# quadram-institute-bioscience/tatajuba

Measured on AMD Instinct MI355X. Metric: reads/s (whole node), 150 bp synthetic FASTQ, homopolymer scan + context histogram, higher is better.
Workload: dtype u8/u64

## Files before the change

### include/tatajuba_amd.h

```cpp
#ifndef TATAJUBA_AMD_H
#define TATAJUBA_AMD_H

#include "tatajuba_hopo.h"

#ifdef __cplusplus
extern "C" {
#endif

#define TJ_META_BASE_SHIFT   0
#define TJ_META_LEN_SHIFT    2
#define TJ_META_COUNT_SHIFT  12
#define TJ_META_MISM_SHIFT   32
#define TJ_META_FLAG_SHIFT   49
#define TJ_META_RAW_CONST    ((1ULL << TJ_META_COUNT_SHIFT) | (0xffeULL << TJ_META_MISM_SHIFT))

typedef struct tjamd_counter tjamd_counter;

typedef struct { uint64_t ctx0, ctx1, meta; } tjamd_record;
typedef struct { uint64_t ctx0, ctx1, meta, pos; } tjamd_located_record;

enum { TJAMD_OK = 0, TJAMD_ERR_NO_DEVICE = 1, TJAMD_ERR_HIP = 2, TJAMD_ERR_ARG = 3, TJAMD_ERR_CAPACITY = 4, TJAMD_ERR_STATE = 5 };

int  tjamd_device_count (void);
const char *tjamd_last_error (void);
const char *tjamd_version (void);
const char *tjamd_source_hash (void);

tjamd_counter *tjamd_counter_create (int device, int kmer_size);
void tjamd_counter_destroy (tjamd_counter *c);
int  tjamd_counter_reset (tjamd_counter *c);
int  tjamd_counter_set_stream (tjamd_counter *c, void *hip_stream);
int  tjamd_counter_device (const tjamd_counter *c);

int  tjamd_scan_device (tjamd_counter *c, const void *d_stream, size_t n_bytes, int min_tract_size);
int  tjamd_scan_host (tjamd_counter *c, const void *h_stream, size_t n_bytes, int min_tract_size);
long tjamd_scan_host_located (tjamd_counter *c, const void *h_stream, size_t n_bytes, int min_tract_size,
                              tjamd_located_record *out, long capacity);

long tjamd_scan_windows (int kmer_size, const char *const *seqs, const int *lens, int n_windows, int min_tract_size,
                         hopo_element *out, int *window_of, long capacity);

long tjamd_read_file_stream (const char *path, unsigned char *out, long capacity, long *n_reads);

long tjamd_read_file_stream_mt (const char *path, unsigned char *out, long capacity, long *n_reads, int n_threads, long window_bytes);

void *tjamd_host_alloc (size_t bytes);
void tjamd_host_free (void *p);
int  tjamd_sync (tjamd_counter *c);

void *tjamd_device_alloc (tjamd_counter *c, size_t bytes);
void tjamd_device_free (tjamd_counter *c, void *p);
int  tjamd_device_download (tjamd_counter *c, void *host, const void *dev, size_t bytes);

int  tjamd_reserve (tjamd_counter *c, size_t stream_bytes, int min_tract_size);

int  tjamd_mark (tjamd_counter *c);
int  tjamd_wait_mark (tjamd_counter *c, int mark);

long tjamd_raw_count (tjamd_counter *c);
long tjamd_download_raw (tjamd_counter *c, tjamd_record *out, long capacity);
long tjamd_undefined_runs (tjamd_counter *c);
int  tjamd_upload_raw (tjamd_counter *c, const hopo_element *elems, long n);

int  tjamd_finalise (tjamd_counter *c, int remove_biased, int min_coverage, int *status);
int  tjamd_finalise_begin (tjamd_counter *c, int remove_biased, int min_coverage);
int  tjamd_counter_set_order_stream (tjamd_counter *c, void *hip_stream);
int  tjamd_finalise_end (tjamd_counter *c, int *status);
long tjamd_kept_count (tjamd_counter *c);
int  tjamd_n_idx (tjamd_counter *c);
int  tjamd_coverage (tjamd_counter *c);
long tjamd_download_kept (tjamd_counter *c, hopo_element *out, long capacity);
long tjamd_download_idx (tjamd_counter *c, int *idx_initial, int *idx_final, long capacity);
const void *tjamd_kept_device_ptr (tjamd_counter *c);

long tjamd_merge_samples (tjamd_counter *c, const void *d_records, const long *counts, int n_samples,
                          void *d_out_keys, void *d_out_counts, long capacity);

long tjamd_gather_histograms (tjamd_counter *dst, tjamd_counter *const *samples, int n_samples, const void **d_records, long *counts);

int tjamd_peer_access_report (char *out, int capacity);

#define TJAMD_COMM_ID_BYTES 128
typedef struct tjamd_comm tjamd_comm;
int  tjamd_comm_unique_id (void *id_bytes);
tjamd_comm *tjamd_comm_create (tjamd_counter *c, const void *id_bytes, int rank, int world);
void tjamd_comm_destroy (tjamd_comm *comm);
int  tjamd_comm_set_stream (tjamd_comm *comm, void *hip_stream);
int  tjamd_comm_rank (const tjamd_comm *comm);
int  tjamd_comm_world (const tjamd_comm *comm);
int  tjamd_comm_count (const tjamd_comm *comm);
int  tjamd_comm_last_exchange (const tjamd_comm *comm, double *ms, long *bytes, long *collectives);
long tjamd_comm_collectives (const tjamd_comm *comm);
long tjamd_allgather_histograms (tjamd_counter *c, tjamd_comm *comm, const void **d_records, long *counts);

long tjamd_tract_ids (tjamd_counter *c, const void *d_keys, long n, int *d_tract_id, int *h_tract_id);

#define TJAMD_N_TRACT_STATS 5
enum { TJAMD_STAT_AVG_LENGTH, TJAMD_STAT_MODAL_FREQ, TJAMD_STAT_PROP_COVERAGE, TJAMD_STAT_COVERAGE_PER_CONTEXT, TJAMD_STAT_ENTROPY };
typedef struct { int first, n_rows, n_present, variable; double reldiff[TJAMD_N_TRACT_STATS]; } tjamd_tract_summary;

long tjamd_tract_stats (tjamd_counter *c, const void *d_keys, const void *d_counts, long n_union, int n_samples,
                        const int *d_tract_id, const int *coverage, const int *d_ref_length,
                        tjamd_tract_summary *d_summary, int *d_var, long capacity, long *n_var);
long tjamd_tract_sample_stats (tjamd_counter *c, const void *d_keys, const void *d_counts, long n_union, int n_samples,
                               const int *coverage, const tjamd_tract_summary *d_summary, long n_tracts, const int *d_list, long n_list,
                               double *d_values, int *d_modal_len, int *d_n_context);

typedef struct { int first, n_rows, n_context, mode, indel, lev_distance; long long integral; } tjamd_union_tract;
typedef struct { int first, n_rows, n_present, variable, selected, lev_distance; double reldiff[TJAMD_N_TRACT_STATS]; } tjamd_union_tract_summary;

long tjamd_union_tracts (tjamd_counter *c, const void *d_keys, const void *d_counts, long n_union, int n_samples,
                         int max_distance_per_flank, int levenshtein_distance,
                         int *d_tract_id, int *d_join_type, tjamd_union_tract *d_tracts, long capacity);
long tjamd_union_tract_stats (tjamd_counter *c, const void *d_keys, const void *d_counts, long n_union, int n_samples,
                              const tjamd_union_tract *d_tracts, long n_tracts, const int *coverage, const int *d_ref_length,
                              tjamd_union_tract_summary *d_summary, int *d_var, long *n_var, int *d_sel, long *n_sel);
long tjamd_union_tract_sample_stats (tjamd_counter *c, const void *d_keys, const void *d_counts, long n_union, int n_samples,
                                     const int *coverage, const tjamd_union_tract_summary *d_summary, long n_tracts,
                                     const int *d_list, long n_list, double *d_values, int *d_modal_len, int *d_n_context, int *d_n_len);

typedef struct { int first, n_elem, n_context, mode; long long integral; } tjamd_group;
long tjamd_group_contexts (tjamd_counter *c, int max_distance_per_flank, int *group_of, tjamd_group *groups, long capacity);

typedef struct { int first, n_elem, n_context, mode, indel, n_len, modal_len, modal_freq; long long integral; } tjamd_context_group;
typedef struct { int length, freq; } tjamd_length_freq;
long tjamd_context_histograms (tjamd_counter *c, int max_distance_per_flank, int levenshtein_distance, int *group_of, int *join_type,
                               tjamd_context_group *groups, tjamd_length_freq *hist, long capacity);

typedef struct tjamd_reference tjamd_reference;
typedef struct { uint64_t ctx0, ctx1; long long flat; int contig, pos, length, base, neg_strand, pad; } tjamd_ref_entry;
tjamd_reference *tjamd_reference_create (tjamd_counter *c, const void *h_stream, size_t n_bytes);
void tjamd_reference_destroy (tjamd_reference *ref);
long tjamd_reference_entries (const tjamd_reference *ref);
long tjamd_reference_contigs (const tjamd_reference *ref);
long tjamd_reference_download (const tjamd_reference *ref, tjamd_ref_entry *out, long capacity);

typedef struct { long long flat; int contig, pos, ref_length, mismatches, neg_strand, n_hits; } tjamd_location;
long tjamd_locate (tjamd_counter *c, const tjamd_reference *ref, const void *d_keys, long n, int max_mismatches, tjamd_location *d_loc);

long tjamd_located_tracts (tjamd_counter *c, const void *d_keys, const void *d_counts, long n_union, int n_samples,
                           const tjamd_union_tract *d_tracts, long n_tracts, const tjamd_location *d_loc,
                           int *d_perm, void *d_out_keys, void *d_out_counts,
                           tjamd_union_tract *d_out_tracts, tjamd_location *d_tract_loc, int *d_ref_length, long capacity);






void tjamd_thread_cleanup (void);

double tjamd_last_scan_ms (tjamd_counter *c);
int    tjamd_counter_uses_log (const tjamd_counter *c);
double tjamd_last_partition_ms (tjamd_counter *c);
double tjamd_last_finalise_ms (tjamd_counter *c);
double tjamd_last_merge_ms (tjamd_counter *c);
double tjamd_last_tract_stats_ms (tjamd_counter *c);
double tjamd_last_union_tracts_ms (tjamd_counter *c);
double tjamd_last_union_tract_stats_ms (tjamd_counter *c);
long   tjamd_last_union_tract_candidates (tjamd_counter *c);
double tjamd_last_reference_ms (tjamd_counter *c);
double tjamd_last_locate_ms (tjamd_counter *c);
double tjamd_last_located_tracts_ms (tjamd_counter *c);
double tjamd_last_tract_variants_ms (tjamd_counter *c);
long   tjamd_last_scan_launches (tjamd_counter *c);
long   tjamd_plan_mismatches (tjamd_counter *c);

long tjamd_synth_stream (uint64_t seed_genome, uint64_t seed_reads, uint64_t variant_seed, long genome_len,
                         long n_reads, int read_len, int read_len_max, unsigned char *out, long capacity, int n_threads);

#ifdef __cplusplus
}
#endif
#endif
```

### tatajuba_amd/capi.py

```python
import ctypes as C
import os

import numpy as np

from .build import build_library, library_path

ELEM_DTYPE = np.dtype([("ctx0", "<u8"), ("ctx1", "<u8"), ("meta", "<u8"), ("read_offset", "<i4"),
                       ("loc_ref_id", "<i4"), ("loc_pos", "<i4"), ("loc_last", "<i4")])
RECORD_DTYPE = np.dtype([("ctx0", "<u8"), ("ctx1", "<u8"), ("meta", "<u8")])
GROUP_DTYPE = np.dtype([("first", "<i4"), ("n_elem", "<i4"), ("n_context", "<i4"), ("mode", "<i4"), ("integral", "<i8")])
CONTEXT_GROUP_DTYPE = np.dtype([("first", "<i4"), ("n_elem", "<i4"), ("n_context", "<i4"), ("mode", "<i4"), ("indel", "<i4"), ("n_len", "<i4"),
                                ("modal_len", "<i4"), ("modal_freq", "<i4"), ("integral", "<i8")])
LENGTH_FREQ_DTYPE = np.dtype([("length", "<i4"), ("freq", "<i4")])
LOCATED_DTYPE = np.dtype([("ctx0", "<u8"), ("ctx1", "<u8"), ("meta", "<u8"), ("pos", "<u8")])
N_TRACT_STATS = 5
TRACT_SUMMARY_DTYPE = np.dtype([("first", "<i4"), ("n_rows", "<i4"), ("n_present", "<i4"), ("variable", "<i4"), ("reldiff", "<f8", (N_TRACT_STATS,))])
assert TRACT_SUMMARY_DTYPE.itemsize == 56
UNION_TRACT_DTYPE = np.dtype([("first", "<i4"), ("n_rows", "<i4"), ("n_context", "<i4"), ("mode", "<i4"), ("indel", "<i4"),
                              ("lev_distance", "<i4"), ("integral", "<i8")])
assert UNION_TRACT_DTYPE.itemsize == 32
UNION_TRACT_SUMMARY_DTYPE = np.dtype([("first", "<i4"), ("n_rows", "<i4"), ("n_present", "<i4"), ("variable", "<i4"), ("selected", "<i4"),
                                      ("lev_distance", "<i4"), ("reldiff", "<f8", (N_TRACT_STATS,))])
assert UNION_TRACT_SUMMARY_DTYPE.itemsize == 64
REF_ENTRY_DTYPE = np.dtype([("ctx0", "<u8"), ("ctx1", "<u8"), ("flat", "<i8"), ("contig", "<i4"), ("pos", "<i4"), ("length", "<i4"),
                            ("base", "<i4"), ("neg_strand", "<i4"), ("pad", "<i4")])
assert REF_ENTRY_DTYPE.itemsize == 48
LOCATION_DTYPE = np.dtype([("flat", "<i8"), ("contig", "<i4"), ("pos", "<i4"), ("ref_length", "<i4"), ("mismatches", "<i4"),
                           ("neg_strand", "<i4"), ("n_hits", "<i4")])
assert LOCATION_DTYPE.itemsize == 32
VARIANT_DTYPE = np.dtype([("flat", "<i8"), ("tract", "<i4"), ("sample", "<i4"), ("contig", "<i4"), ("pos", "<i4"), ("row", "<i4"), ("base", "<i4"),
                          ("ref_length", "<i4"), ("alt_length", "<i4"), ("n_flank", "<i4"), ("pad", "<i4"), ("ref_flank", "<u8"), ("alt_flank", "<u8")])
assert VARIANT_DTYPE.itemsize == 64
FEATURE_DTYPE = np.dtype([("contig", "<i4"), ("start", "<i4"), ("end", "<i4"), ("cls", "<i4"), ("strand", "<i4"), ("line", "<i4"), ("type_off", "<i4"), ("id_off", "<i4")])
assert FEATURE_DTYPE.itemsize == 32
TRACT_FEATURE_DTYPE = np.dtype([("feature", "<i4"), ("max_length", "<i4")])
assert TRACT_FEATURE_DTYPE.itemsize == 8
CDS_DTYPE = np.dtype([("aa_len", "<i4"), ("has_stop", "<i4"), ("n_codons", "<i4"), ("phase", "<i4")])
assert CDS_DTYPE.itemsize == 16
EFFECT_DTYPE = np.dtype([("feature", "<i4"), ("cls", "<i4"), ("cds_pos", "<i4"), ("first_diff", "<i4"), ("ref_aa_len", "<i4"), ("alt_aa_len", "<i4"),
                         ("flags", "<i4"), ("pad", "<i4"), ("ref_aa", "<u8"), ("alt_aa", "<u8")])
assert EFFECT_DTYPE.itemsize == 48
EFFECT_CLASSES = ["NONE", "BOUNDARY", "IDENTICAL", "INFRAME", "FRAMESHIFT"]
SITE_DTYPE = np.dtype([("flat", "<i8"), ("tract", "<i4"), ("contig", "<i4"), ("pos", "<i4"), ("base", "<i4"), ("ref_length", "<i4"), ("min_length", "<i4"),
                       ("n_flank", "<i4"), ("n_alleles", "<i4"), ("first_allele", "<i4"), ("n_called", "<i4"), ("first_record", "<i4"), ("pad", "<i4"),
                       ("ref_flank", "<u8")])
assert SITE_DTYPE.itemsize == 64
ALLELE_DTYPE = np.dtype([("site", "<i4"), ("alt_length", "<i4"), ("n_flank", "<i4"), ("n_samples", "<i4"), ("first_record", "<i4"), ("pad", "<i4"),
                         ("alt_flank", "<u8")])
assert ALLELE_DTYPE.itemsize == 32


class TatajubaAmdError(RuntimeError):
    pass


def _sx(v, bits):
    v = v.astype(np.int64) & ((1 << bits) - 1)
    return np.where(v >= (1 << (bits - 1)), v - (1 << bits), v)


def decode_meta(meta):
    m = np.asarray(meta, dtype=np.uint64)
    sh = lambda s: (m >> np.uint64(s))
    return {"base": _sx(sh(0), 2), "length": _sx(sh(2), 10), "count": _sx(sh(12), 20),
            "mismatches": _sx(sh(32), 12), "multi": _sx(sh(44), 3), "neg_strand": _sx(sh(47), 2),
            "canon_flag": _sx(sh(49), 3)}


class Options(C.Structure):
    _fields_ = [("reference_fasta_filename", C.c_char_p), ("outdir", C.c_char_p),
                ("paired_end", C.c_bool), ("remove_biased", C.c_bool), ("save_vcf", C.c_bool),
                ("gff", C.c_void_p),
                ("max_distance_per_flank", C.c_int), ("kmer_size", C.c_int), ("min_tract_size", C.c_int),
                ("levenshtein_distance", C.c_int), ("min_coverage", C.c_int), ("n_samples", C.c_int),
                ("n_threads", C.c_int)]

    @classmethod
    def defaults(cls, kmer_size=25, min_tract_size=4, min_coverage=5, remove_biased=True, paired_end=False):
        o = cls()
        o.kmer_size, o.min_tract_size, o.min_coverage = kmer_size, min_tract_size, min_coverage
        o.remove_biased, o.paired_end = remove_biased, paired_end
        o.max_distance_per_flank, o.levenshtein_distance, o.n_samples, o.n_threads = 1, 2, 1, 1
        return o


class _HopoCounterStruct(C.Structure):
    _fields_ = [("elem", C.c_void_p), ("name", C.c_char_p),
                ("ref_start", C.c_int), ("n_elem", C.c_int), ("n_alloc", C.c_int), ("kmer_size", C.c_int),
                ("coverage", C.c_int),
                ("idx_initial", C.POINTER(C.c_int)), ("idx_final", C.POINTER(C.c_int)), ("n_idx", C.c_int),
                ("opt", Options), ("ref_counter", C.c_int)]


assert C.sizeof(Options) == 64 and C.sizeof(_HopoCounterStruct) == 136

_LIB = None

EXPORTS = [
    "new_hopo_counter", "del_hopo_counter", "new_or_append_hopo_counter_from_file", "update_hopo_counter_from_seq",
    "update_hopo_counter_from_seq_all_monomers",
    "finalise_hopo_counter", "compare_hopo_element_decreasing", "compare_hopo_context",
    "generate_name_from_flanking_contexts", "generate_tract_as_string", "print_tatajuba_options",
    "distance_between_single_context_kmer", "distance_between_context_kmer_pair", "distance_between_context_kmer_pair_with_edit_shift",
    "leftmost_hopo_name_and_length_from_string", "hopo_counter_histogram_integral",
    "dna_in_2_bits", "bit_2_dna",
    "tjamd_device_count", "tjamd_source_hash", "tjamd_last_error", "tjamd_version", "tjamd_counter_create", "tjamd_counter_destroy",
    "tjamd_counter_reset", "tjamd_counter_set_stream", "tjamd_counter_set_order_stream", "tjamd_counter_device", "tjamd_scan_device", "tjamd_scan_host",
    "tjamd_scan_host_located", "tjamd_read_file_stream_mt", "tjamd_host_alloc", "tjamd_host_free", "tjamd_device_alloc", "tjamd_device_free", "tjamd_device_download", "tjamd_sync", "tjamd_mark", "tjamd_wait_mark", "tjamd_reserve", "tjamd_raw_count",
    "tjamd_download_raw", "tjamd_undefined_runs", "tjamd_upload_raw", "tjamd_finalise", "tjamd_finalise_begin", "tjamd_finalise_end", "tjamd_kept_count",
    "tjamd_n_idx", "tjamd_coverage", "tjamd_download_kept", "tjamd_download_idx", "tjamd_kept_device_ptr",
    "tjamd_merge_samples", "tjamd_gather_histograms", "tjamd_peer_access_report", "tjamd_comm_unique_id", "tjamd_comm_create", "tjamd_comm_destroy",
    "tjamd_comm_set_stream", "tjamd_comm_rank", "tjamd_comm_world", "tjamd_comm_collectives", "tjamd_comm_count", "tjamd_comm_last_exchange", "tjamd_last_merge_ms", "tjamd_allgather_histograms", "tjamd_tract_ids", "tjamd_tract_stats", "tjamd_tract_sample_stats", "tjamd_last_tract_stats_ms", "tjamd_union_tracts", "tjamd_union_tract_stats", "tjamd_union_tract_sample_stats", "tjamd_last_union_tracts_ms", "tjamd_last_union_tract_stats_ms", "tjamd_last_union_tract_candidates",
    "tjamd_reference_create", "tjamd_reference_destroy", "tjamd_reference_entries", "tjamd_reference_contigs",
    "tjamd_reference_download", "tjamd_last_reference_ms", "tjamd_locate", "tjamd_last_locate_ms", "tjamd_located_tracts", "tjamd_last_located_tracts_ms",
    "tjamd_last_tract_variants_ms",
    "tjamd_group_contexts", "tjamd_context_histograms", "tjamd_scan_windows", "tjamd_thread_cleanup", "tjamd_last_scan_ms", "tjamd_last_partition_ms", "tjamd_counter_uses_log", "tjamd_last_finalise_ms", "tjamd_last_scan_launches", "tjamd_plan_mismatches",
    "tjamd_synth_stream", "tjamd_read_file_stream",
    "new_genomic_context_list", "del_genomic_context_list", "del_context_histogram",
    "distance_between_context_histogram_and_hopo_context", "indel_distance_between_context_histogram_and_hopo_context",
]

VARIANT_EXPORTS = ["tjamd_tract_variants", "tjamd_read_file_names"]
FEATURE_EXPORTS = ["tjamd_gff3_read", "tjamd_annotation_create", "tjamd_annotation_destroy", "tjamd_annotation_features", "tjamd_annotation_download",
                   "tjamd_tract_features", "tjamd_last_annotation_ms", "tjamd_last_tract_features_ms"]
LOCATE_EXPORTS = ["tjamd_flank_edit_distance", "tjamd_reference_add_seeds", "tjamd_reference_has_seeds", "tjamd_locate_gapped",
                  "tjamd_last_seed_order_ms", "tjamd_last_locate_gapped_ms"]
EFFECT_EXPORTS = ["tjamd_translate", "tjamd_gff3_read_phase", "tjamd_coding_create", "tjamd_coding_destroy", "tjamd_coding_features", "tjamd_coding_download",
                  "tjamd_variant_effects", "tjamd_last_coding_ms", "tjamd_last_variant_effects_ms"]
SITE_EXPORTS = ["tjamd_merge_variants", "tjamd_site_ref_alt", "tjamd_last_merge_variants_ms"]
MAX_SHIFT = 3


def _share_hip_runtime_with_torch():
    if os.environ.get("TATAJUBA_AMD_HIP_RUNTIME", "") == "system":
        return
    import importlib.util
    import sys
    if "torch" in sys.modules:
        return
    try:
        spec = importlib.util.find_spec("torch")
    except (ImportError, ValueError):
        spec = None
    if spec is None or not spec.submodule_search_locations:
        return
    cand = os.path.join(list(spec.submodule_search_locations)[0], "lib", "libamdhip64.so")
    if os.path.exists(cand):
        try:
            C.CDLL(cand, mode=C.RTLD_GLOBAL)
        except OSError:
            pass


def lib():
    global _LIB
    if _LIB is not None:
        return _LIB
    path = library_path()
    if not os.path.exists(path):
        build_library()
    _share_hip_runtime_with_torch()
    L = C.CDLL(path)
    P = C.POINTER(_HopoCounterStruct)
    L.new_hopo_counter.restype = P; L.new_hopo_counter.argtypes = [C.c_int]
    L.del_hopo_counter.restype = None; L.del_hopo_counter.argtypes = [P]
    L.new_or_append_hopo_counter_from_file.restype = P
    L.new_or_append_hopo_counter_from_file.argtypes = [P, C.c_char_p, Options]
    L.update_hopo_counter_from_seq.restype = None
    L.update_hopo_counter_from_seq.argtypes = [P, C.c_char_p, C.c_int, C.c_int]
    L.update_hopo_counter_from_seq_all_monomers.restype = None
    L.update_hopo_counter_from_seq_all_monomers.argtypes = [P, C.c_char_p, C.c_int]
    L.finalise_hopo_counter.restype = None; L.finalise_hopo_counter.argtypes = [P]
    L.generate_name_from_flanking_contexts.restype = C.c_void_p
    L.generate_name_from_flanking_contexts.argtypes = [C.POINTER(C.c_uint64), C.c_int8, C.c_int, C.c_bool]
    L.generate_tract_as_string.restype = C.c_void_p
    L.generate_tract_as_string.argtypes = [C.POINTER(C.c_uint64), C.c_int8, C.c_int, C.c_int, C.c_bool]
    L.compare_hopo_element_decreasing.restype = C.c_int
    L.compare_hopo_element_decreasing.argtypes = [C.c_void_p, C.c_void_p]

    L.tjamd_device_count.restype = C.c_int
    L.tjamd_last_error.restype = C.c_char_p
    L.tjamd_version.restype = C.c_char_p
    L.tjamd_counter_create.restype = C.c_void_p; L.tjamd_counter_create.argtypes = [C.c_int, C.c_int]
    L.tjamd_counter_destroy.restype = None; L.tjamd_counter_destroy.argtypes = [C.c_void_p]
    L.tjamd_counter_reset.argtypes = [C.c_void_p]
    L.tjamd_counter_set_stream.argtypes = [C.c_void_p, C.c_void_p]
    L.tjamd_counter_device.argtypes = [C.c_void_p]
    L.tjamd_scan_device.argtypes = [C.c_void_p, C.c_void_p, C.c_size_t, C.c_int]
    L.tjamd_scan_host.argtypes = [C.c_void_p, C.c_void_p, C.c_size_t, C.c_int]
    L.tjamd_scan_host_located.restype = C.c_long
    L.tjamd_scan_host_located.argtypes = [C.c_void_p, C.c_void_p, C.c_size_t, C.c_int, C.c_void_p, C.c_long]
    L.tjamd_host_alloc.restype = C.c_void_p; L.tjamd_host_alloc.argtypes = [C.c_size_t]
    L.tjamd_host_free.restype = None; L.tjamd_host_free.argtypes = [C.c_void_p]
    L.tjamd_sync.argtypes = [C.c_void_p]
    L.tjamd_raw_count.restype = C.c_long; L.tjamd_raw_count.argtypes = [C.c_void_p]
    L.tjamd_download_raw.restype = C.c_long; L.tjamd_download_raw.argtypes = [C.c_void_p, C.c_void_p, C.c_long]
    L.tjamd_undefined_runs.restype = C.c_long; L.tjamd_undefined_runs.argtypes = [C.c_void_p]
    L.tjamd_upload_raw.argtypes = [C.c_void_p, C.c_void_p, C.c_long]
    L.tjamd_finalise.argtypes = [C.c_void_p, C.c_int, C.c_int, C.POINTER(C.c_int)]
    L.tjamd_finalise_begin.argtypes = [C.c_void_p, C.c_int, C.c_int]
    L.tjamd_finalise_end.argtypes = [C.c_void_p, C.POINTER(C.c_int)]
    L.tjamd_kept_count.restype = C.c_long; L.tjamd_kept_count.argtypes = [C.c_void_p]
    L.tjamd_n_idx.argtypes = [C.c_void_p]
    L.tjamd_coverage.argtypes = [C.c_void_p]
    L.tjamd_download_kept.restype = C.c_long; L.tjamd_download_kept.argtypes = [C.c_void_p, C.c_void_p, C.c_long]
    L.tjamd_download_idx.restype = C.c_long
    L.tjamd_download_idx.argtypes = [C.c_void_p, C.c_void_p, C.c_void_p, C.c_long]
    L.tjamd_kept_device_ptr.restype = C.c_void_p; L.tjamd_kept_device_ptr.argtypes = [C.c_void_p]
    L.tjamd_merge_samples.restype = C.c_long
    L.tjamd_merge_samples.argtypes = [C.c_void_p, C.c_void_p, C.POINTER(C.c_long), C.c_int, C.c_void_p, C.c_void_p, C.c_long]
    L.tjamd_gather_histograms.restype = C.c_long
    L.tjamd_gather_histograms.argtypes = [C.c_void_p, C.POINTER(C.c_void_p), C.c_int, C.POINTER(C.c_void_p), C.POINTER(C.c_long)]
    L.tjamd_tract_ids.restype = C.c_long; L.tjamd_tract_ids.argtypes = [C.c_void_p, C.c_void_p, C.c_long, C.c_void_p, C.c_void_p]
    L.tjamd_tract_stats.restype = C.c_long
    L.tjamd_tract_stats.argtypes = [C.c_void_p, C.c_void_p, C.c_void_p, C.c_long, C.c_int, C.c_void_p, C.POINTER(C.c_int), C.c_void_p,
                                    C.c_void_p, C.c_void_p, C.c_long, C.POINTER(C.c_long)]
    L.tjamd_tract_sample_stats.restype = C.c_long
    L.tjamd_tract_sample_stats.argtypes = [C.c_void_p, C.c_void_p, C.c_void_p, C.c_long, C.c_int, C.POINTER(C.c_int), C.c_void_p, C.c_long,
                                           C.c_void_p, C.c_long, C.c_void_p, C.c_void_p, C.c_void_p]
    L.tjamd_last_tract_stats_ms.restype = C.c_double; L.tjamd_last_tract_stats_ms.argtypes = [C.c_void_p]
    L.tjamd_union_tracts.restype = C.c_long
    L.tjamd_union_tracts.argtypes = [C.c_void_p, C.c_void_p, C.c_void_p, C.c_long, C.c_int, C.c_int, C.c_int, C.c_void_p, C.c_void_p, C.c_void_p, C.c_long]
    L.tjamd_union_tract_stats.restype = C.c_long
    L.tjamd_union_tract_stats.argtypes = [C.c_void_p, C.c_void_p, C.c_void_p, C.c_long, C.c_int, C.c_void_p, C.c_long, C.POINTER(C.c_int), C.c_void_p,
                                          C.c_void_p, C.c_void_p, C.POINTER(C.c_long), C.c_void_p, C.POINTER(C.c_long)]
    L.tjamd_union_tract_sample_stats.restype = C.c_long
    L.tjamd_union_tract_sample_stats.argtypes = [C.c_void_p, C.c_void_p, C.c_void_p, C.c_long, C.c_int, C.POINTER(C.c_int), C.c_void_p, C.c_long,
                                                 C.c_void_p, C.c_long, C.c_void_p, C.c_void_p, C.c_void_p, C.c_void_p]
    L.tjamd_last_union_tracts_ms.restype = C.c_double; L.tjamd_last_union_tracts_ms.argtypes = [C.c_void_p]
    L.tjamd_last_union_tract_stats_ms.restype = C.c_double; L.tjamd_last_union_tract_stats_ms.argtypes = [C.c_void_p]
    L.tjamd_last_union_tract_candidates.restype = C.c_long; L.tjamd_last_union_tract_candidates.argtypes = [C.c_void_p]
    L.tjamd_reference_create.restype = C.c_void_p; L.tjamd_reference_create.argtypes = [C.c_void_p, C.c_void_p, C.c_size_t]
    L.tjamd_reference_destroy.restype = None; L.tjamd_reference_destroy.argtypes = [C.c_void_p]
    L.tjamd_reference_entries.restype = C.c_long; L.tjamd_reference_entries.argtypes = [C.c_void_p]
    L.tjamd_reference_contigs.restype = C.c_long; L.tjamd_reference_contigs.argtypes = [C.c_void_p]
    L.tjamd_reference_download.restype = C.c_long; L.tjamd_reference_download.argtypes = [C.c_void_p, C.c_void_p, C.c_long]
    L.tjamd_locate.restype = C.c_long; L.tjamd_locate.argtypes = [C.c_void_p, C.c_void_p, C.c_void_p, C.c_long, C.c_int, C.c_void_p]
    L.tjamd_located_tracts.restype = C.c_long
    L.tjamd_located_tracts.argtypes = [C.c_void_p, C.c_void_p, C.c_void_p, C.c_long, C.c_int, C.c_void_p, C.c_long, C.c_void_p,
                                       C.c_void_p, C.c_void_p, C.c_void_p, C.c_void_p, C.c_void_p, C.c_void_p, C.c_long]
    L.tjamd_last_reference_ms.restype = C.c_double; L.tjamd_last_reference_ms.argtypes = [C.c_void_p]
    L.tjamd_last_locate_ms.restype = C.c_double; L.tjamd_last_locate_ms.argtypes = [C.c_void_p]
    L.tjamd_last_located_tracts_ms.restype = C.c_double; L.tjamd_last_located_tracts_ms.argtypes = [C.c_void_p]
    L.tjamd_flank_edit_distance.restype = C.c_int; L.tjamd_flank_edit_distance.argtypes = [C.c_uint64, C.c_uint64, C.c_int, C.c_int, C.c_int]
    L.tjamd_reference_add_seeds.restype = C.c_long; L.tjamd_reference_add_seeds.argtypes = [C.c_void_p, C.c_void_p]
    L.tjamd_reference_has_seeds.restype = C.c_int; L.tjamd_reference_has_seeds.argtypes = [C.c_void_p]
    L.tjamd_locate_gapped.restype = C.c_long
    L.tjamd_locate_gapped.argtypes = [C.c_void_p, C.c_void_p, C.c_void_p, C.c_long, C.c_int, C.c_int, C.c_void_p, C.c_void_p]
    L.tjamd_last_seed_order_ms.restype = C.c_double; L.tjamd_last_seed_order_ms.argtypes = [C.c_void_p]
    L.tjamd_last_locate_gapped_ms.restype = C.c_double; L.tjamd_last_locate_gapped_ms.argtypes = [C.c_void_p]
    L.tjamd_tract_variants.restype = C.c_long
    L.tjamd_tract_variants.argtypes = [C.c_void_p, C.c_void_p, C.c_void_p, C.c_void_p, C.c_long, C.c_int, C.c_void_p, C.c_long, C.c_void_p,
                                       C.c_void_p, C.c_long, C.c_void_p, C.c_long, C.c_void_p]
    L.tjamd_last_tract_variants_ms.restype = C.c_double; L.tjamd_last_tract_variants_ms.argtypes = [C.c_void_p]
    L.tjamd_read_file_names.restype = C.c_long
    L.tjamd_read_file_names.argtypes = [C.c_char_p, C.c_void_p, C.c_long, C.POINTER(C.c_long)]
    L.tjamd_gff3_read.restype = C.c_long
    L.tjamd_gff3_read.argtypes = [C.c_char_p, C.c_char_p, C.c_long, C.c_void_p, C.c_long, C.c_void_p, C.c_long, C.POINTER(C.c_long), C.POINTER(C.c_long)]
    L.tjamd_annotation_create.restype = C.c_void_p; L.tjamd_annotation_create.argtypes = [C.c_void_p, C.c_void_p, C.c_void_p, C.c_long]
    L.tjamd_annotation_destroy.restype = None; L.tjamd_annotation_destroy.argtypes = [C.c_void_p]
    L.tjamd_annotation_features.restype = C.c_long; L.tjamd_annotation_features.argtypes = [C.c_void_p]
    L.tjamd_annotation_download.restype = C.c_long; L.tjamd_annotation_download.argtypes = [C.c_void_p, C.c_void_p, C.c_void_p, C.c_long]
    L.tjamd_tract_features.restype = C.c_long
    L.tjamd_tract_features.argtypes = [C.c_void_p, C.c_void_p, C.c_void_p, C.c_void_p, C.c_long, C.c_int, C.c_void_p, C.c_long, C.c_void_p, C.c_void_p]
    L.tjamd_last_annotation_ms.restype = C.c_double; L.tjamd_last_annotation_ms.argtypes = [C.c_void_p]
    L.tjamd_last_tract_features_ms.restype = C.c_double; L.tjamd_last_tract_features_ms.argtypes = [C.c_void_p]
    L.tjamd_translate.restype = C.c_long; L.tjamd_translate.argtypes = [C.c_char_p, C.c_long, C.c_int, C.c_void_p, C.c_long]
    L.tjamd_gff3_read_phase.restype = C.c_long; L.tjamd_gff3_read_phase.argtypes = [C.c_char_p, C.c_char_p, C.c_long, C.c_void_p, C.c_long]
    L.tjamd_coding_create.restype = C.c_void_p; L.tjamd_coding_create.argtypes = [C.c_void_p, C.c_void_p, C.c_size_t, C.c_void_p, C.c_long, C.c_void_p]
    L.tjamd_coding_destroy.restype = None; L.tjamd_coding_destroy.argtypes = [C.c_void_p]
    L.tjamd_coding_features.restype = C.c_long; L.tjamd_coding_features.argtypes = [C.c_void_p]
    L.tjamd_coding_download.restype = C.c_long; L.tjamd_coding_download.argtypes = [C.c_void_p, C.c_void_p, C.c_long]
    L.tjamd_variant_effects.restype = C.c_long
    L.tjamd_variant_effects.argtypes = [C.c_void_p, C.c_void_p, C.c_void_p, C.c_long, C.c_void_p, C.c_long, C.c_void_p]
    L.tjamd_last_coding_ms.restype = C.c_double; L.tjamd_last_coding_ms.argtypes = [C.c_void_p]
    L.tjamd_last_variant_effects_ms.restype = C.c_double; L.tjamd_last_variant_effects_ms.argtypes = [C.c_void_p]
    L.tjamd_merge_variants.restype = C.c_long
    L.tjamd_merge_variants.argtypes = [C.c_void_p, C.c_int, C.c_void_p, C.c_long, C.c_int, C.c_long, C.c_void_p, C.c_long, C.c_void_p, C.c_long,
                                       C.c_void_p, C.c_void_p, C.c_void_p, C.c_void_p]
    L.tjamd_site_ref_alt.restype = C.c_int; L.tjamd_site_ref_alt.argtypes = [C.c_void_p, C.c_void_p, C.c_int, C.c_void_p, C.c_int]
    L.tjamd_last_merge_variants_ms.restype = C.c_double; L.tjamd_last_merge_variants_ms.argtypes = [C.c_void_p]
    L.tjamd_group_contexts.restype = C.c_long
    L.tjamd_group_contexts.argtypes = [C.c_void_p, C.c_int, C.c_void_p, C.c_void_p, C.c_long]
    L.new_genomic_context_list.restype = C.POINTER(GenomicContextListStruct); L.new_genomic_context_list.argtypes = [P]
    L.del_genomic_context_list.restype = None; L.del_genomic_context_list.argtypes = [C.POINTER(GenomicContextListStruct)]
    L.tjamd_comm_unique_id.argtypes = [C.c_void_p]
    L.tjamd_comm_create.restype = C.c_void_p; L.tjamd_comm_create.argtypes = [C.c_void_p, C.c_void_p, C.c_int, C.c_int]
    L.tjamd_comm_destroy.restype = None; L.tjamd_comm_destroy.argtypes = [C.c_void_p]
    L.tjamd_comm_rank.argtypes = [C.c_void_p]; L.tjamd_comm_world.argtypes = [C.c_void_p]
    L.tjamd_comm_set_stream.argtypes = [C.c_void_p, C.c_void_p]
    L.tjamd_comm_collectives.restype = C.c_long; L.tjamd_comm_collectives.argtypes = [C.c_void_p]
    L.tjamd_allgather_histograms.restype = C.c_long
    L.tjamd_allgather_histograms.argtypes = [C.c_void_p, C.c_void_p, C.POINTER(C.c_void_p), C.POINTER(C.c_long)]
    L.tjamd_peer_access_report.argtypes = [C.c_char_p, C.c_int]
    L.tjamd_context_histograms.restype = C.c_long
    L.tjamd_context_histograms.argtypes = [C.c_void_p, C.c_int, C.c_int, C.c_void_p, C.c_void_p, C.c_void_p, C.c_void_p, C.c_long]
    L.tjamd_device_alloc.restype = C.c_void_p; L.tjamd_device_alloc.argtypes = [C.c_void_p, C.c_size_t]
    L.tjamd_device_free.restype = None; L.tjamd_device_free.argtypes = [C.c_void_p, C.c_void_p]
    L.tjamd_device_download.argtypes = [C.c_void_p, C.c_void_p, C.c_void_p, C.c_size_t]
    L.tjamd_scan_windows.restype = C.c_long
    L.tjamd_scan_windows.argtypes = [C.c_int, C.POINTER(C.c_char_p), C.POINTER(C.c_int), C.c_int, C.c_int, C.c_void_p, C.c_void_p, C.c_long]
    U64P = C.POINTER(C.c_uint64)
    L.distance_between_single_context_kmer.argtypes = [U64P, U64P, C.c_int]
    L.distance_between_context_kmer_pair.argtypes = [U64P, U64P]
    L.distance_between_context_kmer_pair_with_edit_shift.argtypes = [U64P, U64P, C.POINTER(C.c_int)]
    L.leftmost_hopo_name_and_length_from_string.restype = C.c_void_p
    L.leftmost_hopo_name_and_length_from_string.argtypes = [C.c_char_p, C.c_size_t, C.c_int, C.c_int, C.POINTER(C.c_int)]
    L.hopo_counter_histogram_integral.argtypes = [P, C.c_int]
    L.tjamd_last_scan_ms.restype = C.c_double; L.tjamd_last_scan_ms.argtypes = [C.c_void_p]
    L.tjamd_last_finalise_ms.restype = C.c_double; L.tjamd_last_finalise_ms.argtypes = [C.c_void_p]
    L.tjamd_last_partition_ms.restype = C.c_double; L.tjamd_last_partition_ms.argtypes = [C.c_void_p]
    L.tjamd_last_scan_launches.restype = C.c_long; L.tjamd_last_scan_launches.argtypes = [C.c_void_p]
    L.tjamd_synth_stream.restype = C.c_long
    L.tjamd_synth_stream.argtypes = [C.c_uint64, C.c_uint64, C.c_uint64, C.c_long, C.c_long, C.c_int, C.c_int,
                                     C.c_void_p, C.c_long, C.c_int]
    L.tjamd_read_file_stream.restype = C.c_long
    L.tjamd_read_file_stream.argtypes = [C.c_char_p, C.c_void_p, C.c_long, C.POINTER(C.c_long)]
    _LIB = L
    return L


def _err():
    return (lib().tjamd_last_error() or b"").decode(errors="replace")


def device_count():
    return lib().tjamd_device_count()


def synth_stream(n_reads, read_len, genome_len, seed_genome=0x7A7A0001, seed_reads=0x7A7A1000, variant_seed=0,
                 read_len_max=0, n_threads=8, out=None):
    need = -lib().tjamd_synth_stream(seed_genome, seed_reads, variant_seed, genome_len, n_reads, read_len, read_len_max,
                                     None, 0, n_threads)
    if need <= 0:
        raise TatajubaAmdError("bad synthetic-stream parameters")
    if out is None:
        out = np.empty(need, dtype=np.uint8)
    assert out.dtype == np.uint8 and out.size >= need and out.flags["C_CONTIGUOUS"]
    got = lib().tjamd_synth_stream(seed_genome, seed_reads, variant_seed, genome_len, n_reads, read_len, read_len_max,
                                   out.ctypes.data, out.size, n_threads)
    if got != need:
        raise TatajubaAmdError("synthetic stream generation failed")
    return out[:need]


def read_file_stream_mt(path, n_threads=4, window_bytes=0):
    L = lib()
    L.tjamd_read_file_stream_mt.restype = C.c_long
    L.tjamd_read_file_stream_mt.argtypes = [C.c_char_p, C.c_void_p, C.c_long, C.POINTER(C.c_long), C.c_int, C.c_long]
    n = C.c_long(0)
    need = L.tjamd_read_file_stream_mt(os.fsencode(path), None, 0, C.byref(n), n_threads, window_bytes)
    if need < 0:
        raise FileNotFoundError(path)
    out = np.empty(max(need, 1), dtype=np.uint8)
    got = L.tjamd_read_file_stream_mt(os.fsencode(path), out.ctypes.data, need, C.byref(n), n_threads, window_bytes)
    assert got == need
    return out[:need], n.value


def read_file_stream(path):
    n = C.c_long(0)
    need = lib().tjamd_read_file_stream(os.fsencode(path), None, 0, C.byref(n))
    if need < 0:
        raise FileNotFoundError(path)
    out = np.empty(max(need, 1), dtype=np.uint8)
    got = lib().tjamd_read_file_stream(os.fsencode(path), out.ctypes.data, need, C.byref(n))
    assert got == need
    return out[:need], n.value


def read_gff3(path, names):
    blob = b"".join((n if isinstance(n, bytes) else str(n).encode()) + b"\n" for n in names)
    nb, sk = C.c_long(0), C.c_long(0)
    n = lib().tjamd_gff3_read(os.fsencode(path), blob, len(names), None, 0, None, 0, C.byref(nb), C.byref(sk))
    if n < 0:
        raise FileNotFoundError(path)
    out = np.zeros(n, dtype=FEATURE_DTYPE)
    strings = np.zeros(max(nb.value, 1), dtype=np.uint8)
    got = lib().tjamd_gff3_read(os.fsencode(path), blob, len(names), out.ctypes.data, n, strings.ctypes.data, nb.value, C.byref(nb), C.byref(sk))
    assert got == n
    read_gff3.last_skipped = sk.value
    return out, strings[: nb.value].tobytes()


def read_gff3_phase(path, names):
    blob = b"".join((n if isinstance(n, bytes) else str(n).encode()) + b"\n" for n in names)
    n = lib().tjamd_gff3_read_phase(os.fsencode(path), blob, len(names), None, 0)
    if n < 0:
        raise FileNotFoundError(path)
    out = np.zeros(n, dtype=np.int8)
    got = lib().tjamd_gff3_read_phase(os.fsencode(path), blob, len(names), out.ctypes.data if n else None, n)
    assert got == n
    return out


def translate(dna, reverse=False):
    b = dna if isinstance(dna, bytes) else str(dna).encode()
    out = np.zeros(max(len(b) // 3, 1), dtype=np.uint8)
    n = lib().tjamd_translate(b, len(b), 1 if reverse else 0, out.ctypes.data, len(b) // 3)
    if n < 0:
        raise TatajubaAmdError(_err())
    return out[:n].tobytes().decode()


def site_ref_alt(site, allele, k):
    sb = np.asarray(site, SITE_DTYPE).reshape(1).tobytes()
    ab = None if allele is None else np.asarray(allele, ALLELE_DTYPE).reshape(1).tobytes()
    n = lib().tjamd_site_ref_alt(sb, ab, k, None, 0)
    if n < 0:
        raise TatajubaAmdError("tjamd_site_ref_alt: a site or allele that has no text")
    out = C.create_string_buffer(n + 1)
    assert lib().tjamd_site_ref_alt(sb, ab, k, out, n + 1) == n
    return out.value.decode()


def gff3_string(strings, off):
    return strings[off: strings.index(b"\0", off)].decode(errors="replace")


class EmpfreqElement(C.Structure):
    _fields_ = [("freq", C.c_int), ("idx", C.c_int)]


class EmpfreqStruct(C.Structure):
    _fields_ = [("i", C.POINTER(EmpfreqElement)), ("n", C.c_int), ("min", C.c_int), ("max", C.c_int)]


class ContextHistogramStruct(C.Structure):
    _fields_ = [("context", C.POINTER(C.c_uint64)),
                ("base", C.c_int32, 2), ("multi", C.c_int32, 3), ("indel", C.c_int32, 2), ("neg_strand", C.c_int32, 1), ("mismatches", C.c_int32, 12),
                ("name", C.c_char_p), ("n_context", C.c_int), ("integral", C.c_int), ("location", C.c_int), ("loc2d", C.c_int * 3),
                ("coverage", C.c_int), ("n_tracts", C.c_int), ("mode_context_count", C.c_int), ("mode_context_length", C.c_int),
                ("mode_context_id", C.c_int), ("tmp_count", C.POINTER(C.c_int)), ("tmp_length", C.POINTER(C.c_int)), ("index", C.c_int),
                ("h", C.POINTER(EmpfreqStruct)), ("tract_id", C.c_int), ("ref_counter", C.c_int)]


class GenomicContextListStruct(C.Structure):
    _fields_ = [("hist", C.POINTER(C.POINTER(ContextHistogramStruct))), ("name", C.c_char_p), ("opt", Options),
                ("n_hist", C.c_int), ("coverage", C.c_int), ("ref_start", C.c_int)]


class Comm:

    ID_BYTES = 128

    @staticmethod
    def unique_id():
        buf = C.create_string_buffer(Comm.ID_BYTES)
        if lib().tjamd_comm_unique_id(buf) != 0:
            raise TatajubaAmdError(_err())
        return buf.raw

    def __init__(self, counter, ident, rank, world):
        self.world = world
        self._id = C.create_string_buffer(bytes(ident), Comm.ID_BYTES)
        self._h = lib().tjamd_comm_create(counter._h, self._id, rank, world)
        if not self._h:
            raise TatajubaAmdError(_err())

    def set_stream(self, hip_stream):
        if lib().tjamd_comm_set_stream(self._h, C.c_void_p(hip_stream)) != 0:
            raise TatajubaAmdError(_err())

# ... 212 lines not shown
        self._chk(lib().tjamd_finalise(self._h, int(bool(remove_biased)), int(min_coverage), C.byref(st)))
        return st.value

    def finalise_begin(self, remove_biased, min_coverage):
        self._chk(lib().tjamd_finalise_begin(self._h, int(bool(remove_biased)), int(min_coverage)))

    def finalise_end(self):
        st = C.c_int(-1)
        self._chk(lib().tjamd_finalise_end(self._h, C.byref(st)))
        return st.value

    @property
    def n_kept(self):
        return lib().tjamd_kept_count(self._h)

    @property
    def n_idx(self):
        return lib().tjamd_n_idx(self._h)

    @property
    def coverage(self):
        return lib().tjamd_coverage(self._h)

    @property
    def kept_device_ptr(self):
        return lib().tjamd_kept_device_ptr(self._h)

    def download_kept(self):
        n = self.n_kept
        out = np.zeros(n, dtype=ELEM_DTYPE)
        self._chkn(lib().tjamd_download_kept(self._h, out.ctypes.data, n))
        return out

    def download_idx(self):
        n = self.n_idx
        a, b = np.zeros(n, np.int32), np.zeros(n, np.int32)
        self._chkn(lib().tjamd_download_idx(self._h, a.ctypes.data, b.ctypes.data, n))
        return a, b

    def group_contexts(self, max_distance_per_flank):
        n = self.n_kept
        gof = np.zeros(max(n, 1), dtype=np.int32)
        grp = np.zeros(max(n, 1), dtype=GROUP_DTYPE)
        ng = self._chkn(lib().tjamd_group_contexts(self._h, max_distance_per_flank, gof.ctypes.data, grp.ctypes.data, n))
        return gof[:n], grp[:ng]

    def context_histograms(self, max_distance_per_flank, levenshtein_distance):
        n = self.n_kept
        gof, jt = np.zeros(max(n, 1), np.int32), np.zeros(max(n, 1), np.int32)
        grp = np.zeros(max(n, 1), dtype=CONTEXT_GROUP_DTYPE)
        hist = np.zeros(max(n, 1), dtype=LENGTH_FREQ_DTYPE)
        ng = self._chkn(lib().tjamd_context_histograms(self._h, max_distance_per_flank, levenshtein_distance, gof.ctypes.data, jt.ctypes.data,
                                                       grp.ctypes.data, hist.ctypes.data, n))
        return {"group_of": gof[:n], "join_type": jt[:n], "groups": grp[:ng], "hist": hist[:n]}

    def last_scan_launches(self):
        return int(lib().tjamd_last_scan_launches(self._h))

    def plan_mismatches(self):
        lib().tjamd_plan_mismatches.restype = C.c_long
        lib().tjamd_plan_mismatches.argtypes = [C.c_void_p]
        return int(lib().tjamd_plan_mismatches(self._h))

    def last_scan_ms(self):
        return lib().tjamd_last_scan_ms(self._h)

    def last_partition_ms(self):
        return lib().tjamd_last_partition_ms(self._h)

    def bucket_counts(self):
        import numpy as np
        f = lib().tjamd_debug_bucket_counts
        f.restype = C.c_long
        f.argtypes = [C.c_void_p, C.c_void_p, C.c_int]
        b = np.zeros(256, np.uint32)
        if f(self._h, b.ctypes.data, 256) < 0:
            raise TatajubaAmdError(_err())
        return b

    def last_merge_ms(self):
        lib().tjamd_last_merge_ms.restype = C.c_double
        lib().tjamd_last_merge_ms.argtypes = [C.c_void_p]
        return lib().tjamd_last_merge_ms(self._h)

    def last_tract_stats_ms(self):
        return lib().tjamd_last_tract_stats_ms(self._h)

    def last_union_tracts_ms(self):
        return lib().tjamd_last_union_tracts_ms(self._h)

    def last_union_tract_stats_ms(self):
        return lib().tjamd_last_union_tract_stats_ms(self._h)

    def last_union_tract_candidates(self):
        return int(lib().tjamd_last_union_tract_candidates(self._h))

    def last_reference_ms(self):
        return lib().tjamd_last_reference_ms(self._h)

    def last_locate_ms(self):
        return lib().tjamd_last_locate_ms(self._h)

    def last_located_tracts_ms(self):
        return lib().tjamd_last_located_tracts_ms(self._h)

    def locate_gapped(self, ref, d_keys, n, max_edits, max_shift, d_loc, d_how=None):
        got = lib().tjamd_locate_gapped(self._h, ref._h, d_keys, n, max_edits, max_shift, d_loc, d_how)
        if got < 0:
            raise TatajubaAmdError(_err())
        return int(got)

    def last_seed_order_ms(self):
        return lib().tjamd_last_seed_order_ms(self._h)

    def last_locate_gapped_ms(self):
        return lib().tjamd_last_locate_gapped_ms(self._h)

    def last_tract_variants_ms(self):
        return lib().tjamd_last_tract_variants_ms(self._h)

    def last_annotation_ms(self):
        return lib().tjamd_last_annotation_ms(self._h)

    def last_tract_features_ms(self):
        return lib().tjamd_last_tract_features_ms(self._h)

    def variant_effects(self, coding, d_variants, n, d_out, d_tract_feat=None, n_tracts=0):
        return self._chkn(lib().tjamd_variant_effects(self._h, coding._h, d_variants, n, d_tract_feat, n_tracts, d_out))

    def last_coding_ms(self):
        return lib().tjamd_last_coding_ms(self._h)

    def last_variant_effects_ms(self):
        return lib().tjamd_last_variant_effects_ms(self._h)

    def merge_variants(self, kmer_size, d_records, n_records, n_samples, n_tracts, d_sites, site_capacity, d_alleles, allele_capacity,
                       d_genotype=None, d_allele_of=None, d_unique=None):
        n_alleles = C.c_long(-1)
        n_sites = self._chkn(lib().tjamd_merge_variants(self._h, kmer_size, d_records, n_records, n_samples, n_tracts, d_sites, site_capacity,
                                                        d_alleles, allele_capacity, d_genotype, d_allele_of, d_unique, C.byref(n_alleles)))
        return n_sites, n_alleles.value

    def last_merge_variants_ms(self):
        return lib().tjamd_last_merge_variants_ms(self._h)

    def uses_log(self):
        lib().tjamd_counter_uses_log.restype = C.c_int
        lib().tjamd_counter_uses_log.argtypes = [C.c_void_p]
        return bool(lib().tjamd_counter_uses_log(self._h))

    def last_finalise_ms(self):
        return lib().tjamd_last_finalise_ms(self._h)


class HopoCounter:

    def __init__(self, ptr):
        self._p = ptr

    @classmethod
    def new(cls, kmer_size):
        return cls(lib().new_hopo_counter(kmer_size))

    @classmethod
    def new_or_append_from_file(cls, hc, filename, opt):
        p = lib().new_or_append_hopo_counter_from_file(hc._p if hc is not None else None, os.fsencode(filename), opt)
        if hc is not None:
            return hc
        return cls(p)

    def update_from_seq(self, seq, min_tract_size):
        if isinstance(seq, str):
            seq = seq.encode("latin-1")
        lib().update_hopo_counter_from_seq(self._p, seq, len(seq), min_tract_size)

    def update_from_seq_all_monomers(self, seq):
        if isinstance(seq, str):
            seq = seq.encode("latin-1")
        lib().update_hopo_counter_from_seq_all_monomers(self._p, seq, len(seq))

    def finalise(self):
        lib().finalise_hopo_counter(self._p)

    def delete(self):
        if self._p:
            lib().del_hopo_counter(self._p)
            self._p = None

    __del__ = delete

    @property
    def c(self):
        return self._p.contents

    def elems(self, n=None):
        n = self.c.n_elem if n is None else n
        if n == 0:
            return np.zeros(0, dtype=ELEM_DTYPE)
        buf = (C.c_char * (n * 40)).from_address(self.c.elem)
        return np.frombuffer(buf, dtype=ELEM_DTYPE).copy()

    def idx(self):
        n = self.c.n_idx
        if n == 0 or not self.c.idx_initial:
            return np.zeros(0, np.int32), np.zeros(0, np.int32)
        return (np.ctypeslib.as_array(self.c.idx_initial, (n,)).copy(),
                np.ctypeslib.as_array(self.c.idx_final, (n,)).copy())
```

### tatajuba_amd/csrc/hopo_device.hip

```cpp

#include <hip/hip_runtime.h>
#include <rccl/rccl.h>
#include <dlfcn.h>
#include <mutex>
#include <string>
#include <new>
#include <stdint.h>
#include <stdio.h>
#include <stdlib.h>
#include <string.h>
#include <stdarg.h>
#include <limits.h>
#include <float.h>
#include <algorithm>
#include <vector>
#include <memory>

#include "../../include/tatajuba_amd.h"
#include "../../include/tatajuba_variants.h"
#include "../../include/tatajuba_features.h"
#include "../../include/tatajuba_effects.h"
#include "../../include/tatajuba_sites.h"
#include "../../include/tatajuba_locate.h"

// ... 567 lines not shown
  for (u64 i = blockIdx.x * (u64) blockDim.x + threadIdx.x; i < n_fix; i += (u64) gridDim.x * blockDim.x) {
    u64 c0, c1; u32 base, flag;
    if (stale_context (seq, n_bytes, fix[i].pos, k, mprime, c0, c1, base, flag)) {
      u64 idx = atomicAdd (&ctr->n_rec, 1ull);
      if (idx < cap) store_record<4> (out, idx, c0, c1, make_meta (base, fix[i].len, flag), (u64) fix[i].pos);
      else ctr->overflow = 1u;
    }
    else atomicAdd (&ctr->n_undefined, 1ull);
  }
}


template <int W> __device__ __forceinline__ void pack_raw (u64 c0, u64 c1, u32 base, u32 len10, u32 flag, int k, u64 *w);
#define R1_FLAG_SHIFT 59
#define R1_KEY_MASK   (~(3ull << R1_FLAG_SHIFT))
__device__ __forceinline__ u64 pack_rec1 (u32 c0, u32 c1, u32 base, u32 len10, u32 flag)
{
  const u32 lo = c1 | (len10 << 24), hi = c0 | ((len10 >> 8) << 24) | (base << 26) | (flag << 27);
  return ((u64) hi << 32) | lo;
}
template <> __device__ __forceinline__ void pack_raw<1> (u64 c0, u64 c1, u32 base, u32 len10, u32 flag, int k, u64 *w)
{ w[0] = pack_rec1 ((u32) c0, (u32) c1, base, len10, flag); }
template <> __device__ __forceinline__ void pack_raw<2> (u64 c0, u64 c1, u32 base, u32 len10, u32 flag, int k, u64 *w)
{ w[0] = 1ull | ((u64) base << 1) | ((u64) (len10 & 31u) << 2) | (c0 << 7); w[1] = c1 | ((u64) (len10 >> 5) << 56) | ((u64) flag << 61); }
template <> __device__ __forceinline__ void pack_raw<4> (u64 c0, u64 c1, u32 base, u32 len10, u32 flag, int k, u64 *w)
{ w[0] = c0; w[1] = c1; w[2] = (u64) base | ((u64) len10 << 2) | ((u64) flag << 12); w[3] = 0; }
template <int W> __device__ __forceinline__ void pack_null (u64 *w) { pack_raw<W> (0, 0, 0, 0, 3u, 2, w); }

template <int W> __device__ __forceinline__ void unpack_raw (const u64 *w, int k, u64 &c0, u64 &c1, u32 &base, u32 &len10, u32 &flag);
template <> __device__ __forceinline__ void unpack_raw<1> (const u64 *w, int k, u64 &c0, u64 &c1, u32 &base, u32 &len10, u32 &flag)
{
  const u32 lo = (u32) w[0], hi = (u32) (w[0] >> 32);
  c1 = lo & 0xFFFFFFu; c0 = hi & 0xFFFFFFu; len10 = (lo >> 24) | (((hi >> 24) & 3u) << 8); base = (hi >> 26) & 1u; flag = (hi >> 27) & 3u;
}
template <> __device__ __forceinline__ void unpack_raw<2> (const u64 *w, int k, u64 &c0, u64 &c1, u32 &base, u32 &len10, u32 &flag)
{
  const u64 m56 = (1ull << 56) - 1ull;
  c0 = (w[0] >> 7) & m56; c1 = w[1] & m56;
  base = (u32) (w[0] >> 1) & 1u; len10 = ((u32) (w[0] >> 2) & 31u) | (((u32) (w[1] >> 56) & 31u) << 5); flag = (u32) (w[1] >> 61) & 3u;
}
template <> __device__ __forceinline__ void unpack_raw<4> (const u64 *w, int k, u64 &c0, u64 &c1, u32 &base, u32 &len10, u32 &flag)
{ c0 = w[0]; c1 = w[1]; base = (u32) (w[2] & 3ull); len10 = (u32) ((w[2] >> 2) & 0x3FFull); flag = (u32) ((w[2] >> 12) & 3ull); }

__device__ __forceinline__ u64 hash_key (u64 c0, u64 c1, u32 base, u32 len10)
{
  u32 a = (u32) c0 ^ __builtin_amdgcn_alignbit ((u32) (c0 >> 32), (u32) (c0 >> 32), 25) ^ __builtin_amdgcn_alignbit ((u32) c1, (u32) c1, 19)
          ^ __builtin_amdgcn_alignbit ((u32) (c1 >> 32), (u32) (c1 >> 32), 11) ^ ((base | (len10 << 2)) * 0x9E3779B1u);
  u32 h = a * 0x85EBCA6Bu;
  h ^= h >> 15; h *= 0xC2B2AE35u; h ^= h >> 16;
  const u32 tag = (a ^ (a >> 13)) * 0x27D4EB2Fu;
  return ((u64) tag << 32) | h;
}

__device__ __forceinline__ u32 bucket_of_key (u64 c0, u64 c1, u32 base, u32 len10)
{
  u32 h = __builtin_amdgcn_udot4 ((u32) c0, 0x6D2B4F0Bu, base | (len10 << 2), false);
  h = __builtin_amdgcn_udot4 ((u32) (c0 >> 32), 0x1D59A735u, h, false);
  h = __builtin_amdgcn_udot4 ((u32) c1, 0xC5A34D17u, h, false);
  h = __builtin_amdgcn_udot4 ((u32) (c1 >> 32), 0x3B7F9165u, h, false);
  return (h ^ (h >> 8)) & 255u;
}

__device__ __forceinline__ u32 bucket_of_rec1 (u32 lo, u32 hi)
{
  u32 h = __builtin_amdgcn_udot4 (lo, 0x6D2B4F0Bu, 0u, false);
  h = __builtin_amdgcn_udot4 (hi & 0x07FFFFFFu, 0xC5A34D17u, h, false);
  return (h ^ (h >> 8)) & 255u;
}

#define TJ_P        256
#define TJ_PBITS    8
#define TJ_STAGE_WORDS 2048
#define TJ_CH0      1536
#define TJ_EMPTY    0xFFFFFFFFu
#define TJ_CSTRIDE  64

struct Buckets
{
  u64 *pool;
  u32 *table;
  u32 *cursors;
  u32 *pool_next;
  u32 pool_chunks, maxj, ch_shift;
};

#define TJ_NOCHUNK  0xFFFFFFFEu
#define TJ_SPIN_MAX (1u << 20)

__device__ __forceinline__ u32 chunk_of_pos (const Buckets &B, u32 pos) { return (pos / TJ_CH0) >> B.ch_shift; }

__device__ __forceinline__ void bucket_claim_ahead (const Buckets &B, u32 b, u32 p0, u32 n, DevCounters *ctr)
{
  const u32 j = chunk_of_pos (B, p0 + n - 1);
  if (((j * TJ_CH0) << B.ch_shift) < p0) return;
  if (j + 1 >= B.maxj) { ctr->overflow = 1u; return; }
  const u32 mine = atomicAdd (B.pool_next, 1u);
  if (mine >= B.pool_chunks) ctr->overflow = 1u;
  __hip_atomic_store (B.table + (u64) b * B.maxj + j + 1, mine < B.pool_chunks ? mine : TJ_NOCHUNK, __ATOMIC_RELAXED, __HIP_MEMORY_SCOPE_AGENT);
}

__device__ __forceinline__ void bucket_claim_ahead_range (const Buckets &B, u32 b, u32 p0, u32 n, DevCounters *ctr)
{
  const u32 ch = (u32) TJ_CH0 << B.ch_shift;
  for (u32 j = (p0 + ch - 1u) / ch; (u64) j * ch < (u64) p0 + n; j++) {
    if (j + 1 >= B.maxj) { ctr->overflow = 1u; return; }
    const u32 mine = atomicAdd (B.pool_next, 1u);
    if (mine >= B.pool_chunks) ctr->overflow = 1u;
    __hip_atomic_store (B.table + (u64) b * B.maxj + j + 1, mine < B.pool_chunks ? mine : TJ_NOCHUNK, __ATOMIC_RELAXED, __HIP_MEMORY_SCOPE_AGENT);
  }
}

__device__ __forceinline__ u32 bucket_chunk_id (const Buckets &B, u32 b, u32 j, bool wait, DevCounters *ctr)
{
  if (j >= B.maxj) return TJ_NOCHUNK;
  u32 *e = B.table + (u64) b * B.maxj + j;
  u32 ch = __hip_atomic_load (e, __ATOMIC_RELAXED, __HIP_MEMORY_SCOPE_AGENT);
  if (wait) {
    for (u32 spins = 0; ch == TJ_EMPTY && spins < TJ_SPIN_MAX; spins++) {
      __builtin_amdgcn_s_sleep (4);
      ch = __hip_atomic_load (e, __ATOMIC_RELAXED, __HIP_MEMORY_SCOPE_AGENT);
    }
    if (ch == TJ_EMPTY && ctr) ctr->overflow = 2u;
  }
  return ch >= TJ_NOCHUNK ? TJ_NOCHUNK : ch;
}

__device__ __forceinline__ u64 bucket_slot (const Buckets &B, u32 b, u32 pos, bool wait, DevCounters *ctr)
{
  const u32 j = chunk_of_pos (B, pos);
  const u32 ch = bucket_chunk_id (B, b, j, wait, ctr);
  if (ch == TJ_NOCHUNK) return ~0ull;
  return (((u64) ch * TJ_CH0) << B.ch_shift) + (pos - ((j * TJ_CH0) << B.ch_shift));
}

template <int W>
__device__ __forceinline__ void bucket_insert_slow (u64 c0, u64 c1, u32 base, u32 len10, u32 flag, int k, const Buckets &B, DevCounters *ctr)
{
  u64 w[W];
  pack_raw<W> (c0, c1, base, len10, flag, k, w);
  const u32 b = (W == 1) ? bucket_of_rec1 ((u32) w[0], (u32) (w[0] >> 32)) : bucket_of_key (c0, c1, base, len10);
  const u32 pos = atomicAdd (&B.cursors[b * TJ_CSTRIDE], 1u);
  bucket_claim_ahead (B, b, pos, 1u, ctr);
  const u64 at = bucket_slot (B, b, pos, true, ctr);
  if (at != ~0ull) { u64 *q = B.pool + at * W; for (int j = 0; j < W; j++) q[j] = w[j]; }
}


template <int W, int BIG = 0>
struct StageLds
{
  static constexpr int WS = (W == 4) ? 3 : W;
  static constexpr int WORDS = BIG == 2 ? 8192 : BIG ? TJ_STAGE_WORDS * 2 : (W == 1) ? TJ_STAGE_WORDS : 2688;
  static constexpr int S = WORDS / WS;
  static constexpr int SPARE = BIG ? 64 : 0;
  u64 rec[WORDS + SPARE * WS];
  alignas (16) u64 gbase[TJ_P];
  u64 gbase2[TJ_P];
  alignas (16) u32 hist[TJ_P + SPARE];
  alignas (16) u32 offs[TJ_P + SPARE];
  u32 split[BIG == 2 ? 1 : TJ_P];
  u32 wsum[TJ_P / 64];
  u32 n;
  unsigned char bin[S + SPARE];
};

typedef StageLds<1, true> StageLdsFast1;
static_assert (offsetof (StageLdsFast1, gbase2) == offsetof (StageLdsFast1, gbase) + sizeof (u64) * TJ_P, "gbase and gbase2 back to back");

template <int W, int BLOCK, int BIG = 0>
struct StageSink
{
  static constexpr bool K32 = (W == 1);
  static constexpr int S = StageLds<W, BIG>::S;
  static constexpr int WS = StageLds<W, BIG>::WS;
  static constexpr int R = (S + BLOCK - 1) / BLOCK;
  static constexpr int PS = (BIG && S > BLOCK && (S - BLOCK) % BLOCK == 0) ? S - BLOCK : 0;
  StageLds<W, BIG> &L;
  Buckets B; DevCounters *ctr; int k;
  u32 bound;
  u32 cur_j, cur_chunk;

  __device__ __forceinline__ void start ()
  {
    if (threadIdx.x == 0) L.n = 0;
    if (BIG && threadIdx.x < TJ_P) L.hist[threadIdx.x] = 0;
    bound = 0; cur_j = TJ_EMPTY; cur_chunk = TJ_NOCHUNK;
    lds_barrier ();
  }

  __device__ __forceinline__ void tick () {}

  __device__ __forceinline__ void put (bool have, u64 c0, u64 c1, u32 base, u32 len10, u32 flag, u64 pos, u32 round_max)
  {
    if (bound + round_max > (u32) S) bound = partition ();
    bound += round_max;
    if (have) {
      const u32 at = atomicAdd (&L.n, 1u);
      u64 w[W];
      pack_raw<W> (c0, c1, base, len10, flag, k, w);
#pragma unroll
      for (int j = 0; j < WS; j++) L.rec[at * WS + j] = w[j];
      L.bin[at] = (unsigned char) (W == 1 ? bucket_of_rec1 ((u32) w[0], (u32) (w[0] >> 32)) : bucket_of_key (c0, c1, base, len10));
    }
  }

  __device__ __forceinline__ void put1 (bool have, u32 lo, u32 hi, u32 round_max)
  {
    if (bound + round_max > (u32) S) bound = partition ();
    bound += round_max;
    if (have) {
      const u32 at = atomicAdd (&L.n, 1u);
      L.rec[at * WS] = ((u64) hi << 32) | lo;
      L.bin[at] = (unsigned char) bucket_of_rec1 (lo, hi);
    }
  }

  __device__ __forceinline__ void reserve1 (u32 round_max)
  {
    if (bound + round_max > (u32) S) bound = partition ();
    bound += round_max;
  }
  __device__ __forceinline__ u32 count_addr () const { return (u32) (size_t) (lptr_t) &L.n; }
  __device__ __forceinline__ void store1 (u32 at, u32 lo, u32 hi)
  {
    L.rec[at * WS] = ((u64) hi << 32) | lo;
    L.bin[at] = (unsigned char) bucket_of_rec1 (lo, hi);
  }
  __device__ __forceinline__ void store1v (u32 at, u32 lo, u32 hi, u32 h0, u32 h1, u32 m27)
  {
    L.rec[at * WS] = ((u64) hi << 32) | lo;
    u32 h = __builtin_amdgcn_udot4 (lo, h0, 0u, false);
    h = __builtin_amdgcn_udot4 (hi & m27, h1, h, false);
    L.bin[at] = (unsigned char) (h ^ (h >> 8));
  }
  __device__ __forceinline__ void store_fields (u32 at, u64 c0, u64 c1, u32 base, u32 len10, u32 flag)
  {
    u64 w[W];
    pack_raw<W> (c0, c1, base, len10, flag, k, w);
#pragma unroll
    for (int j = 0; j < WS; j++) L.rec[at * WS + j] = w[j];
    L.bin[at] = (unsigned char) (W == 1 ? bucket_of_rec1 ((u32) w[0], (u32) (w[0] >> 32)) : bucket_of_key (c0, c1, base, len10));
  }

  __device__ __forceinline__ u32 partition_big (const bool final_pass = false)
  {
    lds_barrier ();
    const u32 n = (u32) __builtin_amdgcn_readfirstlane ((int) L.n);
    if constexpr (PS > 0) {
      if (n >= (u32) PS || final_pass) return final_pass ? partition_pass<false> (n) : partition_pass<true> (n);
      lds_barrier ();
      return n;
    }
    else return partition_pass<false> (n);
  }

  template <bool FULL>
  __device__ __forceinline__ u32 partition_pass (const u32 n)
  {
    static_assert (!BIG || BLOCK == 2 * TJ_P, "two threads per bucket");
    constexpr int RR = FULL ? PS / BLOCK : R;
    constexpr int H = (RR < 4) ? RR : 4;
    const int tid = threadIdx.x, lane = tid & 63;
    const int wave = __builtin_amdgcn_readfirstlane (tid >> 6);
    u64 w[RR][WS], wrem[WS];
    u32 rk[RR], bb[RR], brem = 0;
#pragma unroll
    for (int r = 0; r < RR; r++)
      if (FULL || (u32) r * BLOCK < n) {
        const u32 i = (u32) tid + (u32) r * BLOCK;
        bb[r] = L.bin[i];
#pragma unroll
        for (int j = 0; j < WS; j++) w[r][j] = L.rec[i * WS + j];
      }
    if constexpr (FULL) {
      brem = L.bin[(u32) PS + (u32) tid];
#pragma unroll
      for (int j = 0; j < WS; j++) wrem[j] = L.rec[((u32) PS + (u32) tid) * WS + j];
    }
#pragma unroll
    for (int r = 0; r < RR; r++)
      if (FULL || (u32) r * BLOCK < n) {
        const u32 i = (u32) tid + (u32) r * BLOCK;
        if constexpr (!FULL) bb[r] = (i < n) ? bb[r] : (u32) (TJ_P + lane);
        rk[r] = atomicAdd (&L.hist[bb[r]], 1u);
      }
    lds_barrier ();
    if (tid == 0) L.n = FULL ? n - (u32) PS : 0u;
    u32 cnt = 0, p0 = 0, off = 0;
    if (wave < TJ_P / 64) {
      const uint4 h4 = *reinterpret_cast<const uint4 *> (&L.hist[4 * lane]);
      const u32 tot = h4.x + h4.y + h4.z + h4.w;
      const u32 e0 = wave_inclusive_scan (tot) - tot;
      if ((lane >> 4) == wave) *reinterpret_cast<uint4 *> (&L.offs[4 * lane]) = make_uint4 (e0, e0 + h4.x, e0 + h4.x + h4.y, e0 + h4.x + h4.y + h4.z);
      cnt = L.hist[tid];
      off = L.offs[tid];
      if (cnt) p0 = atomicAdd (&B.cursors[tid * TJ_CSTRIDE], cnt);
    }
    else if (!FULL && wave == TJ_P / 64) L.offs[tid] = (u32) S + (u32) lane;
    lds_barrier ();
    if (tid < TJ_P) L.hist[tid] = 0;
    {
      u32 dst[RR];
#pragma unroll
      for (int r = 0; r < RR; r++) if (FULL || (u32) r * BLOCK < n) dst[r] = L.offs[bb[r]];
#pragma unroll
      for (int r = 0; r < RR; r++)
        if (FULL || (u32) r * BLOCK < n) {
// ... 1594 lines not shown
}


__device__ __forceinline__ u32 key_digit (u64 c0, u64 c1, u64 meta, int pass, int k)
{
  const int o = 8 * pass;
  const u32 v12 = (u32) ((((meta >> TJ_META_LEN_SHIFT) & 0x3FFull) ^ 0x200ull) << 2) | (u32) ((meta >> TJ_META_FLAG_SHIFT) & 3ull);
  const u64 base = meta & 1ull;
  u32 d = 0;
  int lo;
  lo = o;                      if (lo < 12)                       d |= (u32) (v12 >> lo);
  lo = o - 12;                 if (lo < 2 * k && lo > -8)         d |= (u32) (lo >= 0 ? (c1 >> lo) : (c1 << -lo));
  lo = o - 12 - 2 * k;         if (lo < 2 * k && lo > -8)         d |= (u32) (lo >= 0 ? (c0 >> lo) : (c0 << -lo));
  lo = o - 12 - 4 * k;         if (lo < 1 && lo > -8)             d |= (u32) (base << -lo);
  return (~d) & 0xFFu;
}

__host__ int key_passes (int k) { return (13 + 4 * k + 7) / 8; }

#define RS_ITEMS      1024
#define RS_WAVE_ITEMS 256

__device__ __forceinline__ u64 match_digit (u32 d, bool active)
{
  u64 peers = __ballot (active);
#pragma unroll
  for (int b = 0; b < 8; b++) {
    u64 bal = __ballot ((d >> b) & 1u);
    peers &= ((d >> b) & 1u) ? bal : ~bal;
  }
  return active ? peers : 0ull;
}

__global__ __launch_bounds__ (256)
void radix_count_kernel (const u64 *__restrict__ in, long n, int pass, int k, u32 *__restrict__ hist, int nblk)
{
  __shared__ u32 h[256];
  const int tid = threadIdx.x, lane = tid & 63;
  const u64 lt = (1ull << lane) - 1ull;
  h[tid] = 0;
  __syncthreads ();
  const long base = (long) blockIdx.x * RS_ITEMS;
  for (int i = tid; i < RS_ITEMS; i += 256) {
    long r = base + i;
    bool active = r < n;
    u32 d = 0;
    if (active) { const u64 *p = in + 3 * r; d = key_digit (p[0], p[1], p[2], pass, k); }
    u64 peers = match_digit (d, active);
    if (active && (peers & lt) == 0ull) atomicAdd (&h[d], (u32) __popcll (peers));
  }
  __syncthreads ();
  hist[(long) tid * nblk + blockIdx.x] = h[tid];
}

__global__ __launch_bounds__ (256)
void radix_scatter_kernel (const u64 *__restrict__ in, u64 *__restrict__ out, long n, int pass, int k,
                           const u32 *__restrict__ offs, int nblk)
{
  __shared__ u32 wcnt[4][256];
  const int tid = threadIdx.x, wave = tid >> 6, lane = tid & 63;
  for (int i = tid; i < 1024; i += 256) (&wcnt[0][0])[i] = 0;
  __syncthreads ();
  const long wbase = (long) blockIdx.x * RS_ITEMS + (long) wave * RS_WAVE_ITEMS;
  const u64 lt = (1ull << lane) - 1ull;

  for (int r = 0; r < RS_WAVE_ITEMS / 64; r++) {
    long idx = wbase + r * 64 + lane;
    bool active = idx < n;
    u32 d = 0;
    if (active) { const u64 *p = in + 3 * idx; d = key_digit (p[0], p[1], p[2], pass, k); }
    u64 peers = match_digit (d, active);
    if (active && (peers & lt) == 0ull) atomicAdd (&wcnt[wave][d], (u32) __popcll (peers));
  }
  __syncthreads ();
  {
    u32 run = offs[(long) tid * nblk + blockIdx.x];
    for (int w = 0; w < 4; w++) { u32 c = wcnt[w][tid]; wcnt[w][tid] = run; run += c; }
  }
  __syncthreads ();
  for (int r = 0; r < RS_WAVE_ITEMS / 64; r++) {
    long idx = wbase + r * 64 + lane;
    bool active = idx < n;
    u32 d = 0;
    u64 a = 0, b = 0, m = 0;
    if (active) { const u64 *p = in + 3 * idx; a = p[0]; b = p[1]; m = p[2]; d = key_digit (a, b, m, pass, k); }
    u64 peers = match_digit (d, active);
    int leader = active ? (__ffsll ((long long) peers) - 1) : 0;
    u32 old = 0;
    if (active && lane == leader) old = atomicAdd (&wcnt[wave][d], (u32) __popcll (peers));
    old = __shfl (old, leader);
    if (active) {
      u64 *q = out + 3 * ((u64) old + (u64) __popcll (peers & lt));
      q[0] = a; q[1] = b; q[2] = m;
    }
  }
}


#define BS_RANK_MAX  256

__device__ __forceinline__ u32 bin_of_record (u64 c0, u64 c1, u64 meta, int k, int nbits)
{
  const int kb = nbits - 1;
  const u64 v = (2 * k >= kb) ? (c0 >> (2 * k - kb)) : ((c0 << (kb - 2 * k)) | (c1 >> (4 * k - kb)));
  const u32 x = ((u32) (meta & 1ull) << kb) | (u32) v;
  return ((1u << nbits) - 1u) - x;
}

__device__ __forceinline__ bool record_before (u64 a0, u64 a1, u64 am, u32 ai, u64 b0, u64 b1, u64 bm, u32 bi)
{
  const u32 ab = (u32) am & 1u, bb = (u32) bm & 1u;
  if (ab != bb) return ab > bb;
  if (a0 != b0) return a0 > b0;
  if (a1 != b1) return a1 > b1;
  const u32 al = ((u32) (am >> TJ_META_LEN_SHIFT) & 0x3FFu) ^ 0x200u, bl = ((u32) (bm >> TJ_META_LEN_SHIFT) & 0x3FFu) ^ 0x200u;
  if (al != bl) return al > bl;
  return ai < bi;
}

__device__ __forceinline__ u32 bin_reserve (u32 *__restrict__ cursors, u32 bin, bool active, int grouped)
{
  if (!grouped) return active ? atomicAdd (&cursors[bin], 1u) : 0u;
  const int lane = threadIdx.x & 63;
  u64 todo = __ballot (active);
  u32 pos = 0;
  while (todo) {
    const int leader = __ffsll ((long long) todo) - 1;
    const u32 lb = (u32) __builtin_amdgcn_readlane ((int) bin, leader);
    const u64 grp = __ballot (active && bin == lb) & todo;
    u32 base = 0;
    if (lane == leader) base = atomicAdd (&cursors[lb], (u32) __popcll (grp));
    base = (u32) __builtin_amdgcn_readlane ((int) base, leader);
    if ((grp >> lane) & 1ull) pos = base + (u32) __popcll (grp & ((1ull << lane) - 1ull));
    todo &= ~grp;
  }
  return pos;
}

__global__ __launch_bounds__ (256)
void bin_count_kernel (const u64 *__restrict__ in, long n, int k, int nbits, u32 *__restrict__ bins, uint4 *__restrict__ cov, long cov_vec, int grouped,
                       const FinPlan *__restrict__ plan = nullptr)
{
  if (plan) { if (!plan->ok) return; n = plan->n1; nbits = plan->nbits; cov_vec = plan->t / 2; }
  for (long i = (long) blockIdx.x * 256 + threadIdx.x; i < cov_vec; i += (long) gridDim.x * 256) cov[i] = make_uint4 (0, 0, 0, 0);
  for (long i0 = (long) blockIdx.x * 256; i0 < n; i0 += (long) gridDim.x * 256) {
    const long i = i0 + threadIdx.x;
    u32 bin = 0;
    if (i < n) { const u64 *p = in + 3 * i; bin = bin_of_record (p[0], p[1], p[2], k, nbits); }
    (void) bin_reserve (bins, bin, i < n, grouped);
  }
}

#define BS_MAXBINS (1 << BS_MAXBITS)
#define WGS_CHUNK  16384

#define WGS_PAD(i) ((i) + ((i) >> 5))
struct WgScanLds { u32 a[WGS_CHUNK + WGS_CHUNK / 32 + 1]; u32 wsum[16]; u32 vmax; };

__device__ __forceinline__ u32 wg_exclusive_scan (const u32 *__restrict__ in, int n_all, u32 *__restrict__ out, u32 *__restrict__ out2, WgScanLds &L, u32 &vmax)
{
  const int tid = threadIdx.x, lane = tid & 63, wave = tid >> 6;
  if (tid == 0) L.vmax = 0;
  u32 carry = 0;
  for (int base = 0; base < n_all; base += WGS_CHUNK) {
    const int n = min (WGS_CHUNK, n_all - base);
    const int per = (n + 1023) / 1024;
    for (int i = tid; i < n; i += 1024) L.a[WGS_PAD (i)] = in[base + i];
    __syncthreads ();
    u32 sum = 0, mx = 0;
    for (int j = 0; j < per; j++) { const int b = tid * per + j; if (b < n) { const u32 v = L.a[WGS_PAD (b)]; sum += v; mx = max (mx, v); } }
    const u32 incl = wave_inclusive_scan (sum);
    if (lane == 63) L.wsum[wave] = incl;
    for (int o = 32; o > 0; o >>= 1) mx = max (mx, (u32) __shfl_down ((int) mx, o));
    if (lane == 0 && mx) atomicMax (&L.vmax, mx);
    __syncthreads ();
    u32 run = carry + incl - sum, total = 0;
    for (int w = 0; w < 16; w++) { const u32 x = L.wsum[w]; if (w < wave) run += x; total += x; }
    for (int j = 0; j < per; j++) { const int b = tid * per + j; if (b < n) { const u32 v = L.a[WGS_PAD (b)]; L.a[WGS_PAD (b)] = run; run += v; } }
    __syncthreads ();
    for (int i = tid; i < n; i += 1024) { const u32 v = L.a[WGS_PAD (i)]; out[base + i] = v; if (out2) out2[base + i] = v; }
    carry += total;
    __syncthreads ();
  }
  vmax = L.vmax;
  return carry;
}

__global__ __launch_bounds__ (1024)
void bin_scan_kernel (u32 *__restrict__ bins, int nbins, u32 *__restrict__ binstart, u32 rank_max, FinCounts *fin, const FinPlan *__restrict__ plan = nullptr)
{
  __shared__ WgScanLds L;
  u32 vmax;
  if (plan) { if (!plan->ok) return; nbins = plan->nbins; }
  const u32 total = wg_exclusive_scan (bins, nbins, binstart, bins, L, vmax);
  if (threadIdx.x == 0) { binstart[nbins] = total; fin->sort_fallback = vmax > rank_max ? 1u : 0u; }
}

__global__ __launch_bounds__ (256)
void bin_scatter_kernel (const u64 *__restrict__ in, u64 *__restrict__ out, long n, int k, int nbits, u32 *__restrict__ cursors,
                         const FinPlan *__restrict__ plan = nullptr, uint4 *__restrict__ cov = nullptr)
{
  if (plan) { if (!plan->ok) return; n = plan->n1; nbits = plan->nbits; }
  if (cov) for (long i = (long) blockIdx.x * 256 + threadIdx.x; i < plan->t / 2; i += (long) gridDim.x * 256) cov[i] = make_uint4 (0, 0, 0, 0);
  for (long i = (long) blockIdx.x * 256 + threadIdx.x; i < n; i += (long) gridDim.x * 256) {
    const u64 *p = in + 3 * i;
    const u64 a = p[0], b = p[1], m = p[2];
    u64 *q = out + 3 * (u64) atomicAdd (&cursors[bin_of_record (a, b, m, k, nbits)], 1u);
    q[0] = a; q[1] = b; q[2] = m;
  }
}


#define SC_ITEMS 4096

__device__ __forceinline__ u32 block_exclusive_scan_256 (u32 v, u32 *s_tmp, u32 &total)
{
  const int tid = threadIdx.x, lane = tid & 63, wave = tid >> 6;
  u32 x = v;
#pragma unroll
  for (int o = 1; o < 64; o <<= 1) { u32 y = __shfl_up (x, o); if (lane >= o) x += y; }
  if (lane == 63) s_tmp[wave] = x;
  __syncthreads ();
  u32 wbase = 0;
  for (int w = 0; w < wave; w++) wbase += s_tmp[w];
  total = s_tmp[0] + s_tmp[1] + s_tmp[2] + s_tmp[3];
  __syncthreads ();
  return wbase + x - v;
}

__global__ __launch_bounds__ (256)
void scan_reduce_kernel (const u32 *__restrict__ in, long n, u32 *__restrict__ bsum)
{
  __shared__ u32 s_tmp[4];
  const long base = (long) blockIdx.x * SC_ITEMS + (long) threadIdx.x * 16;
  u32 s = 0;
  for (int i = 0; i < 16; i++) if (base + i < n) s += in[base + i];
  u32 total;
  block_exclusive_scan_256 (s, s_tmp, total);
  if (threadIdx.x == 0) bsum[blockIdx.x] = total;
}

__global__ __launch_bounds__ (256)
void scan_apply_kernel (const u32 *__restrict__ in, u32 *__restrict__ out, long n, const u32 *__restrict__ boff, u32 *total_out)
{
  __shared__ u32 s_tmp[4];
  const long base = (long) blockIdx.x * SC_ITEMS + (long) threadIdx.x * 16;
  u32 v[16], s = 0;
  for (int i = 0; i < 16; i++) { v[i] = (base + i < n) ? in[base + i] : 0u; s += v[i]; }
  u32 total;
  u32 ex = block_exclusive_scan_256 (s, s_tmp, total) + (boff ? boff[blockIdx.x] : 0u);
  for (int i = 0; i < 16; i++) { if (base + i < n) out[base + i] = ex; ex += v[i]; }
  if (total_out && base <= n - 1 && n - 1 < base + 16) *total_out = ex;
}


__device__ __forceinline__ bool same_key (const u64 *a, const u64 *b)
{
  const u64 km = (3ull << TJ_META_BASE_SHIFT) | (0x3FFull << TJ_META_LEN_SHIFT);
  return a[0] == b[0] && a[1] == b[1] && ((a[2] ^ b[2]) & km) == 0ull;
}

__device__ __forceinline__ bool same_context (const u64 *a, const u64 *b)
{
  return a[0] == b[0] && a[1] == b[1] && ((a[2] ^ b[2]) & 3ull) == 0ull;
}

__device__ __forceinline__ int meta_count (u64 meta)
{
  int c = (int) ((meta >> TJ_META_COUNT_SHIFT) & 0xFFFFFull);
  return (c & 0x80000) ? c - 0x100000 : c;
}

__device__ __forceinline__ int meta_len (u64 meta)
{
  int l = (int) ((meta >> TJ_META_LEN_SHIFT) & 0x3FFull);
  return (l & 0x200) ? l - 0x400 : l;
}

__device__ __forceinline__ bool same_context_rows (const u64 *rec, long i, long j) { return same_context (rec + 3 * i, rec + 3 * j); }

__global__ void seg_heads_kernel (const u64 *__restrict__ rec, long n, u32 *__restrict__ flags, int context_only)
{
  for (long i = blockIdx.x * (long) blockDim.x + threadIdx.x; i < n; i += (long) gridDim.x * blockDim.x) {
    bool head = (i == 0);
    if (!head) head = context_only ? !same_context (rec + 3 * i, rec + 3 * (i - 1)) : !same_key (rec + 3 * i, rec + 3 * (i - 1));
    flags[i] = head ? 1u : 0u;
  }
}

__global__ void seg_headpos_kernel (const u32 *__restrict__ flags, const u32 *__restrict__ segid, long n, u32 *__restrict__ headpos)
{
  for (long i = blockIdx.x * (long) blockDim.x + threadIdx.x; i < n; i += (long) gridDim.x * blockDim.x)
    if (flags[i]) headpos[segid[i]] = (u32) i;
}

__global__ void ctx_decide_kernel (const u64 *__restrict__ kept, long n1, const u32 *__restrict__ ctxpos, const u32 *n_ctx_p,
                                   int min_coverage, u32 *__restrict__ keep)
{
  const u32 n_ctx = *n_ctx_p;
  for (u32 j = blockIdx.x * blockDim.x + threadIdx.x; j < n_ctx; j += gridDim.x * blockDim.x) {
    const long s = ctxpos[j], e = (j + 1 < n_ctx) ? (long) ctxpos[j + 1] : n1;
    int depth = 0;
    for (long i = s; i < e; i++) depth += meta_count (kept[3 * i + 2]);
    keep[j] = depth >= min_coverage;
  }
}

__global__ void ctx_write_kernel (long n1, const u32 *__restrict__ ctxpos, const u32 *n_ctx_p, const u32 *__restrict__ keep,
                                  const u32 *__restrict__ outpos, int *__restrict__ idx_initial, int *__restrict__ idx_final)
{
  const u32 n_ctx = *n_ctx_p;
  for (u32 j = blockIdx.x * blockDim.x + threadIdx.x; j < n_ctx; j += gridDim.x * blockDim.x)
    if (keep[j]) {
      idx_initial[outpos[j]] = (int) ctxpos[j];
      idx_final[outpos[j]] = (j + 1 < n_ctx) ? (int) ctxpos[j + 1] : (int) n1;
    }
}

__device__ __forceinline__ u64 cov_word (u32 key31, int w) { return ((u64) (key31 + 1u) << 32) | (u64) (u32) w; }

__device__ __forceinline__ void cov_direct_add (u32 key31, int w, u64 *__restrict__ tab)
{
  atomicAdd ((unsigned long long *) &tab[key31], (unsigned long long) (long long) w + (1ull << 33));
}

__device__ __forceinline__ void cov_add_from (u32 key31, u32 slot, int w, u64 *__restrict__ tab, int log2t)
{
  const u32 tmask = (1u << log2t) - 1u;
  for (u32 probe = 0; probe <= tmask; probe++) {
    const u64 old = atomicCAS ((unsigned long long *) &tab[slot], 0ull, (unsigned long long) cov_word (key31, w));
    if (old == 0ull) break;
    if ((u32) (old >> 32) == key31 + 1u) { atomicAdd (reinterpret_cast<u32 *> (&tab[slot]), (u32) w); break; }
    slot = (slot + 1u) & tmask;
  }
}

__device__ __forceinline__ void cov_add (u32 key31, int w, u64 *__restrict__ tab, int log2t)
{
  cov_add_from (key31, (key31 * 2654435761u) >> (32 - log2t), w, tab, log2t);
}

__device__ __forceinline__ void cov_add2 (u32 ka, u32 kb, int w, u64 *__restrict__ tab, int log2t)
// ... 78 lines not shown
  else if constexpr (J == 16) { const auto r = __builtin_amdgcn_permlane16_swap (v, v, false, false); return (lane & 16) ? r[0] : r[1]; }
  else { const auto r = __builtin_amdgcn_permlane32_swap (v, v, false, false); return (lane & 32) ? r[0] : r[1]; }
}

__global__ __launch_bounds__ (64 * BSI_WAVES)
void bin_sort_index_kernel (const u64 *__restrict__ in, u64 *__restrict__ out, const u32 *__restrict__ binstart, int nbins, const FinCounts *fin,
                            int min_coverage, u64 *__restrict__ cov_tab, int log2t,
                            u32 *__restrict__ binctx, u32 *__restrict__ tstart, u32 *__restrict__ tend, const FinPlan *__restrict__ plan = nullptr,
                            int cov_direct = 0)
{
  __shared__ alignas (16) u32 hd[BSI_WAVES][BS_RANK_MAX];
  __shared__ u32 sz[BSI_WAVES][BS_RANK_MAX];
  const int lane = threadIdx.x & 63, wave = threadIdx.x >> 6;
  const int bin0 = (int) blockIdx.x * BSI_WAVES + wave;
  u32 st0 = 0, en0 = 0;
  if (bin0 < nbins) { st0 = binstart[bin0]; en0 = binstart[bin0 + 1]; }
  if (plan) { if (!plan->ok) return; nbins = plan->nbins; log2t = plan->log2t; cov_direct = (int) plan->cov_direct; }
  if (fin->sort_fallback) return;
  u32 *H = hd[wave], *E = sz[wave];
  for (int bin = bin0; bin < nbins; bin += gridDim.x * BSI_WAVES) {
    const u32 st = (bin == bin0) ? st0 : binstart[bin], s = ((bin == bin0) ? en0 : binstart[bin + 1]) - st;
    if (s == 0) { if (lane == 0) binctx[bin] = 0; continue; }
    const u64 *R = in + 3 * (u64) st;
    u32 nkeep = 0;
    if (s <= 64u) {
      const bool valid = (u32) lane < s;
      u64 a0 = 0, a1 = 0, am = 0;
      if (valid) { a0 = R[3 * lane]; a1 = R[3 * lane + 1]; am = R[3 * lane + 2]; }
      const int w = meta_count (am);
      u64 cas_a = 0, cas_b = 0;
      if (!cov_direct && valid) cov_add2_issue ((u32) (a0 & 0x7FFFFFFFull), (u32) (a1 & 0x7FFFFFFFull), w, cov_tab, log2t, cas_a, cas_b);
      u32 kh = valid ? 2u | ((u32) am & 1u) : 0u;
      u32 kl = ((((u32) (am >> TJ_META_LEN_SHIFT) & 0x3FFu) ^ 0x200u) << 6) | (63u - (u32) lane);
      u32 x0 = (u32) a0, x1 = (u32) (a0 >> 32), y0 = (u32) a1, y1 = (u32) (a1 >> 32), m0 = (u32) am, m1 = (u32) (am >> 32);
      auto step = [&] (auto jc, int kk) {
        constexpr int J = decltype (jc)::value;
        const u32 ox0 = lane_xor<J> (x0, lane), ox1 = lane_xor<J> (x1, lane), oy0 = lane_xor<J> (y0, lane), oy1 = lane_xor<J> (y1, lane);
        const u32 om0 = lane_xor<J> (m0, lane), om1 = lane_xor<J> (m1, lane), okh = lane_xor<J> (kh, lane), okl = lane_xor<J> (kl, lane);
        const u64 mx = ((u64) x1 << 32) | x0, my = ((u64) y1 << 32) | y0, ox = ((u64) ox1 << 32) | ox0, oy = ((u64) oy1 << 32) | oy0;
        const bool mine_first = (kh > okh) | ((kh == okh) & ((mx > ox) | ((mx == ox) & ((my > oy) | ((my == oy) & (kl > okl))))));
        const bool want_first = ((lane & kk) == 0) == ((lane & J) == 0);
        const bool take = mine_first != want_first;
        x0 = take ? ox0 : x0; x1 = take ? ox1 : x1; y0 = take ? oy0 : y0; y1 = take ? oy1 : y1;
        m0 = take ? om0 : m0; m1 = take ? om1 : m1; kh = take ? okh : kh; kl = take ? okl : kl;
      };
#pragma unroll
      for (int kk = 2; kk <= 64; kk <<= 1) {
        if (kk >= 64) step (std::integral_constant<int, 32> (), kk);
        if (kk >= 32) step (std::integral_constant<int, 16> (), kk);
        if (kk >= 16) step (std::integral_constant<int, 8> (), kk);
        if (kk >= 8) step (std::integral_constant<int, 4> (), kk);
        if (kk >= 4) step (std::integral_constant<int, 2> (), kk);
        step (std::integral_constant<int, 1> (), kk);
      }
      const bool have = kh >= 2u;
      const u64 b0 = ((u64) x1 << 32) | x0, b1 = ((u64) y1 << 32) | y0, bm = ((u64) m1 << 32) | m0;
      if (have) { u64 *q = out + 3 * ((u64) st + (u32) lane); q[0] = b0; q[1] = b1; q[2] = bm; }
      const u32 px0 = (u32) __builtin_amdgcn_update_dpp (0, (int) x0, 0x138, 0xF, 0xF, false), px1 = (u32) __builtin_amdgcn_update_dpp (0, (int) x1, 0x138, 0xF, 0xF, false);
      const u32 py0 = (u32) __builtin_amdgcn_update_dpp (0, (int) y0, 0x138, 0xF, 0xF, false), py1 = (u32) __builtin_amdgcn_update_dpp (0, (int) y1, 0x138, 0xF, 0xF, false);
      const u32 pkh = (u32) __builtin_amdgcn_update_dpp (0, (int) kh, 0x138, 0xF, 0xF, false);
      const bool head = have & ((lane == 0) | (px0 != x0) | (px1 != x1) | (py0 != y0) | (py1 != y1) | (pkh != kh));
      const u64 heads = __ballot (head);
      const int cnt = have ? meta_count (bm) : 0;
      const u32 incl = wave_inclusive_scan ((u32) cnt);
      const u64 above = (lane == 63) ? 0ull : (heads >> (lane + 1));
      const u32 next_head = above ? (u32) lane + (u32) __ffsll ((long long) above) : s;
      const u32 last_incl = (u32) __builtin_amdgcn_ds_bpermute ((int) ((next_head - 1u) << 2), (int) incl);
      const int depth = (int) (last_incl - (incl - (u32) cnt));
      const bool keep = head & (depth >= min_coverage);
      const u64 keeps = __ballot (keep);
      if (keep) {
        const u32 o = (u32) __popcll (keeps & ((1ull << lane) - 1ull));
        tstart[st + o] = st + (u32) lane;
        tend[st + o] = st + next_head;
      }
      nkeep = (u32) __popcll (keeps);
      if (cov_direct) {
        if (head) { cov_direct_add ((u32) (b0 & 0x7FFFFFFFull), depth, cov_tab); cov_direct_add ((u32) (b1 & 0x7FFFFFFFull), depth, cov_tab); }
      }
      else if (valid) {
        asm volatile ("" : "+v"(cas_a), "+v"(cas_b));
        cov_add2_finish ((u32) (a0 & 0x7FFFFFFFull), (u32) (a1 & 0x7FFFFFFFull), w, cov_tab, log2t, cas_a, cas_b);
      }
      if (lane == 0) binctx[bin] = nkeep;
      asm volatile ("s_waitcnt lgkmcnt(0)" ::: "memory");
      __builtin_amdgcn_wave_barrier ();
      continue;
    }
    for (u32 t0 = 0; t0 < s; t0 += 64) {
      const u32 t = t0 + lane;
      bool keep = false;
      if (t < s) {
        const u64 a0 = R[3 * t], a1 = R[3 * t + 1], am = R[3 * t + 2];
        u32 rank = 0, ctx_before = 0, ctx_size = 0;
        int depth = 0;
        const u32 abase = (u32) am & 1u, alen = ((u32) (am >> TJ_META_LEN_SHIFT) & 0x3FFu) ^ 0x200u;
        for (u32 j0 = 0; j0 < s; j0 += 4) {
          u64 b0[4], b1[4], bm[4];
#pragma unroll
          for (int i = 0; i < 4; i++) {
            const u32 jj = (j0 + (u32) i < s) ? j0 + (u32) i : s - 1u;
            b0[i] = R[3 * jj]; b1[i] = R[3 * jj + 1]; bm[i] = R[3 * jj + 2];
          }
#pragma unroll
          for (int i = 0; i < 4; i++) {
            const u32 j = j0 + (u32) i;
            const bool live = j < s;
            const u32 bbase = (u32) bm[i] & 1u, blen = ((u32) (bm[i] >> TJ_META_LEN_SHIFT) & 0x3FFu) ^ 0x200u;
            const bool e0 = b0[i] == a0, e1 = b1[i] == a1, eb = bbase == abase;
            const bool before = live & ((bbase > abase) | (eb & ((b0[i] > a0) | (e0 & ((b1[i] > a1) | (e1 & ((blen > alen) | ((blen == alen) & (j < t)))))))));
            const bool same = live & e0 & e1 & (((u32) (bm[i] ^ am) & 3u) == 0u);
            rank += before ? 1u : 0u;
            ctx_size += same ? 1u : 0u;
            depth += same ? meta_count (bm[i]) : 0;
            ctx_before += (same & before) ? 1u : 0u;
          }
        }
        u64 *q = out + 3 * ((u64) st + rank);
        q[0] = a0; q[1] = a1; q[2] = am;
        keep = (ctx_before == 0u) && depth >= min_coverage;
        H[t] = rank | (keep ? 0x80000000u : 0u);
        E[t] = ctx_size;
        if (ctx_before == 0u) {
          if (cov_direct) { cov_direct_add ((u32) (a0 & 0x7FFFFFFFull), depth, cov_tab); cov_direct_add ((u32) (a1 & 0x7FFFFFFFull), depth, cov_tab); }
          else cov_add2 ((u32) (a0 & 0x7FFFFFFFull), (u32) (a1 & 0x7FFFFFFFull), depth, cov_tab, log2t);
        }
      }
      nkeep += (u32) __popcll (__ballot (keep));
    }
    asm volatile ("s_waitcnt lgkmcnt(0)" ::: "memory");
    __builtin_amdgcn_wave_barrier ();
    for (u32 t = lane; t < s; t += 64) {
      const u32 h = H[t];
      if (h & 0x80000000u) {
        const u32 rank = h & 0x7FFFFFFFu;
        u32 o = 0;
        for (u32 j = 0; j < s; j += 4) {
          const uint4 g = *reinterpret_cast<const uint4 *> (&H[j]);
          o += ((g.x & 0x80000000u) && (g.x & 0x7FFFFFFFu) < rank) ? 1u : 0u;
          o += (j + 1u < s && (g.y & 0x80000000u) && (g.y & 0x7FFFFFFFu) < rank) ? 1u : 0u;
          o += (j + 2u < s && (g.z & 0x80000000u) && (g.z & 0x7FFFFFFFu) < rank) ? 1u : 0u;
          o += (j + 3u < s && (g.w & 0x80000000u) && (g.w & 0x7FFFFFFFu) < rank) ? 1u : 0u;
        }
        tstart[st + o] = st + rank;
        tend[st + o] = st + rank + E[t];
      }
    }
    if (lane == 0) binctx[bin] = nkeep;
    asm volatile ("s_waitcnt lgkmcnt(0)" ::: "memory");
    __builtin_amdgcn_wave_barrier ();
  }
}

__global__ __launch_bounds__ (1024)
void bin_ctx_scan_kernel (const u32 *__restrict__ binctx, int nbins, u32 *__restrict__ binout, FinCounts *fin, const FinPlan *__restrict__ plan = nullptr)
{
  __shared__ WgScanLds L;
  u32 vmax;
  if (plan) { if (!plan->ok) return; nbins = plan->nbins; }
  const u32 total = wg_exclusive_scan (binctx, nbins, binout, nullptr, L, vmax);
  if (threadIdx.x == 0 && !fin->sort_fallback) { fin->n_idx = total; fin->coverage = INT_MIN; }
}

__global__ __launch_bounds__ (256)
void bin_ctx_write_kernel (const u32 *__restrict__ binstart, const u32 *__restrict__ binctx, const u32 *__restrict__ binout, int nbins,
                           const u32 *__restrict__ tstart, const u32 *__restrict__ tend, int *__restrict__ idx_initial, int *__restrict__ idx_final,
                           const u64 *__restrict__ cov_tab, long t, FinCounts *fin, const FinPlan *__restrict__ plan = nullptr)
{
  __shared__ int s_best[4];
  if (plan) { if (!plan->ok) return; nbins = plan->nbins; t = plan->t; }
  if (fin->sort_fallback) return;
  const int lane = threadIdx.x & 63, wave = threadIdx.x >> 6;
  for (int bin = blockIdx.x * 4 + wave; bin < nbins; bin += gridDim.x * 4) {
    const u32 cnt = binctx[bin], st = binstart[bin], o0 = binout[bin];
    for (u32 o = lane; o < cnt; o += 64) { idx_initial[o0 + o] = (int) tstart[st + o]; idx_final[o0 + o] = (int) tend[st + o]; }
  }
  cov_max_part (cov_tab, t, &fin->coverage, s_best);
}

#define MG_RANK_MAX 256
#define TJ_META_SAMPLE_SHIFT 52

__global__ __launch_bounds__ (256)
void merge_scatter_kernel (const u64 *__restrict__ in, u64 *__restrict__ out, long n, int k, int nbits, u32 *__restrict__ cursors,
                           const long *__restrict__ starts, int n_samples)
{
  for (long i0 = (long) blockIdx.x * 256; i0 < n; i0 += (long) gridDim.x * 256) {
    const long i = i0 + threadIdx.x;
    const bool active = i < n;
    u64 a = 0, b = 0, m = 0;
    int lo = 0;
    if (active) {
      int hi = n_samples;
      while (hi - lo > 1) { const int mid = (lo + hi) >> 1; if (starts[mid] <= i) lo = mid; else hi = mid; }
      const u64 *p = in + 3 * i;
      a = p[0]; b = p[1]; m = p[2];
    }
    const u32 pos = bin_reserve (cursors, active ? bin_of_record (a, b, m, k, nbits) : 0u, active, 1);
    if (active) {
      u64 *q = out + 3 * (u64) pos;
      q[0] = a; q[1] = b; q[2] = (m & ((1ull << TJ_META_SAMPLE_SHIFT) - 1ull)) | ((u64) lo << TJ_META_SAMPLE_SHIFT);
    }
  }
}

__device__ __forceinline__ bool merge_same_key (u64 a0, u64 a1, u64 am, u64 b0, u64 b1, u64 bm)
{
  const u64 km = (3ull << TJ_META_BASE_SHIFT) | (0x3FFull << TJ_META_LEN_SHIFT);
  return a0 == b0 && a1 == b1 && ((am ^ bm) & km) == 0ull;
}

__global__ __launch_bounds__ (64)
void bin_merge_kernel (const u64 *__restrict__ rec, const u32 *__restrict__ binstart, int nbins, const FinCounts *fin,
                       u32 *__restrict__ binctx, u32 *__restrict__ tpos, u32 *__restrict__ ttot)
{
  __shared__ u64 R[3 * MG_RANK_MAX];
  __shared__ alignas (16) u32 H[MG_RANK_MAX];
  if (fin->sort_fallback) return;
  const int lane = threadIdx.x;
  for (int bin = blockIdx.x; bin < nbins; bin += gridDim.x) {
    const u32 st = binstart[bin], s = binstart[bin + 1] - st;
    if (s == 0) { if (lane == 0) binctx[bin] = 0; continue; }
    for (u32 t = lane; t < s; t += 64) {
      const u64 *p = rec + 3 * (u64) (st + t);
      const u64 v0 = p[0], v1 = p[1], v2 = p[2];
      R[3 * t] = v0; R[3 * t + 1] = v1;
      R[3 * t + 2] = (v2 & ~(0x3FFull << TJ_META_LEN_SHIFT)) | ((((v2 >> TJ_META_LEN_SHIFT) & 0x3FFull) ^ 0x200ull) << TJ_META_LEN_SHIFT);
    }
    asm volatile ("s_waitcnt vmcnt(0) lgkmcnt(0)" ::: "memory");
    __builtin_amdgcn_wave_barrier ();
    const u64 lmask = 0x3FFull << TJ_META_LEN_SHIFT;
    u32 nrep = 0;
    for (u32 t0 = 0; t0 < s; t0 += 64) {
      const u32 t = t0 + lane;
      bool rep = false;
      if (t < s) {
        const u64 a0 = R[3 * t], a1 = R[3 * t + 1], al = R[3 * t + 2] & lmask;
        rep = true;
        u32 tot = 0, r = 0, fl = 0;
        for (u32 j0 = 0; j0 < s; j0 += 4) {
          u64 b0[4], b1[4], bm[4];
#pragma unroll
          for (int i = 0; i < 4; i++) {
            const u32 jj = (j0 + (u32) i < s) ? j0 + (u32) i : s - 1u;
            b0[i] = R[3 * jj]; b1[i] = R[3 * jj + 1]; bm[i] = R[3 * jj + 2];
          }
#pragma unroll
          for (int i = 0; i < 4; i++) {
            const u32 j = j0 + (u32) i;
            const bool live = j < s;
            const u64 bl = bm[i] & lmask;
            const bool same = live & (b0[i] == a0) & (b1[i] == a1) & (bl == al);
            const bool before = live & ((b0[i] > a0) | ((b0[i] == a0) & ((b1[i] > a1) | ((b1[i] == a1) & (bl > al)))));
            r += before ? 1u : 0u;
            rep = rep & !(same & (j < t));
            tot += same ? (u32) meta_count (bm[i]) : 0u;
            fl |= same ? (u32) (bm[i] >> TJ_META_FLAG_SHIFT) & 7u : 0u;
          }
        }
        H[t] = r | (rep ? 0x80000000u : 0u);
        ttot[st + t] = rep ? ((tot & 0xFFFFFu) | (fl << 28)) : 0xFFFFFFFFu;
      }
      nrep += (u32) __popcll (__ballot (rep));
    }
    asm volatile ("s_waitcnt lgkmcnt(0)" ::: "memory");
    __builtin_amdgcn_wave_barrier ();
    for (u32 t = lane; t < s; t += 64) {
      const u32 r = H[t] & 0x7FFFFFFFu;
      u32 d = 0;
      for (u32 j = 0; j < s; j += 4) {
        const uint4 h = *reinterpret_cast<const uint4 *> (&H[j]);
        d += ((h.x & 0x80000000u) && (h.x & 0x7FFFFFFFu) < r) ? 1u : 0u;
        d += (j + 1u < s && (h.y & 0x80000000u) && (h.y & 0x7FFFFFFFu) < r) ? 1u : 0u;
        d += (j + 2u < s && (h.z & 0x80000000u) && (h.z & 0x7FFFFFFFu) < r) ? 1u : 0u;
        d += (j + 3u < s && (h.w & 0x80000000u) && (h.w & 0x7FFFFFFFu) < r) ? 1u : 0u;
      }
      tpos[st + t] = d;
    }
    if (lane == 0) binctx[bin] = nrep;
    asm volatile ("s_waitcnt lgkmcnt(0)" ::: "memory");
    __builtin_amdgcn_wave_barrier ();
  }
}

__global__ __launch_bounds__ (256)
void bin_merge_write_kernel (const u64 *__restrict__ rec, const u32 *__restrict__ binstart, const u32 *__restrict__ binout, int nbins, const FinCounts *fin,
                             const u32 *__restrict__ tpos, const u32 *__restrict__ ttot, int n_samples,
                             u64 *__restrict__ keys, int *__restrict__ counts, long cap)
{
  if (fin->sort_fallback) return;
  const int lane = threadIdx.x & 63, wave = threadIdx.x >> 6;
  for (int bin = blockIdx.x * 4 + wave; bin < nbins; bin += gridDim.x * 4) {
    const u32 st = binstart[bin], s = binstart[bin + 1] - st, o0 = binout[bin];
    for (u32 t0 = 0; t0 < s; t0 += 64) {
      const u32 t = t0 + lane;
      if (t < s) {
        const long u = (long) o0 + tpos[st + t];
        if (u < cap) {
          const u64 a0 = rec[3 * (u64) (st + t)], a1 = rec[3 * (u64) (st + t) + 1], am = rec[3 * (u64) (st + t) + 2];
          const u32 tot = ttot[st + t];
          if (tot != 0xFFFFFFFFu) {
            for (int q = 0; q < n_samples; q++) counts[u * n_samples + q] = 0;
            u64 m = am & ((1ull << TJ_META_SAMPLE_SHIFT) - 1ull);
            m = (m & ~(0xFFFFFull << TJ_META_COUNT_SHIFT)) | (((u64) tot & 0xFFFFFull) << TJ_META_COUNT_SHIFT);
            m = (m & ~(7ull << TJ_META_FLAG_SHIFT)) | ((u64) ((tot >> 28) & 7u) << TJ_META_FLAG_SHIFT);
            keys[3 * u] = a0; keys[3 * u + 1] = a1; keys[3 * u + 2] = m;
          }
        }
      }
      __builtin_amdgcn_wave_barrier ();
      asm volatile ("s_waitcnt vmcnt(0)" ::: "memory");
      if (t < s) {
        const long u = (long) o0 + tpos[st + t];
        if (u < cap) {
          const u64 am = rec[3 * (u64) (st + t) + 2];
          counts[u * n_samples + (int) (am >> TJ_META_SAMPLE_SHIFT)] = meta_count (am);
        }
      }
    }
  }
}

__global__ void set_int_kernel (int *p, int v) { *p = v; }


__global__ void merge_tag_kernel (const u64 *__restrict__ in, u64 *__restrict__ out, long n, const long *__restrict__ starts, int n_samples)
{
  for (long i = blockIdx.x * (long) blockDim.x + threadIdx.x; i < n; i += (long) gridDim.x * blockDim.x) {
    int lo = 0, hi = n_samples;
    while (hi - lo > 1) { const int mid = (lo + hi) >> 1; if (starts[mid] <= i) lo = mid; else hi = mid; }
    out[3 * i] = in[3 * i]; out[3 * i + 1] = in[3 * i + 1];
    out[3 * i + 2] = (in[3 * i + 2] & ((1ull << TJ_META_SAMPLE_SHIFT) - 1ull)) | ((u64) lo << TJ_META_SAMPLE_SHIFT);
  }
}

__global__ void merge_write_kernel (const u64 *__restrict__ rec, long n, const u32 *__restrict__ flags, const u32 *__restrict__ segid,
                                    int n_samples, u64 *__restrict__ keys, int *__restrict__ counts, u32 *__restrict__ totals, u32 *__restrict__ orflags, long cap)
{
  for (long i = blockIdx.x * (long) blockDim.x + threadIdx.x; i < n; i += (long) gridDim.x * blockDim.x) {
    const u32 seg = segid[i] + flags[i] - 1u;
    if ((long) seg >= cap) continue;
    const u64 meta = rec[3 * i + 2];
    const int sample = (int) (meta >> TJ_META_SAMPLE_SHIFT);
    const int cnt = meta_count (meta);
    counts[(long) seg * n_samples + sample] = cnt;
    atomicAdd (&totals[seg], (u32) cnt);
    atomicOr (&orflags[seg], (u32) (meta >> TJ_META_FLAG_SHIFT) & 7u);
    if (flags[i]) { keys[3 * (long) seg] = rec[3 * i]; keys[3 * (long) seg + 1] = rec[3 * i + 1]; keys[3 * (long) seg + 2] = meta; }
  }
}

__global__ void merge_totals_kernel (u64 *__restrict__ keys, const u32 *__restrict__ totals, const u32 *__restrict__ orflags, const u32 *n_seg_p, long cap)
{
  const long n_seg = min ((long) *n_seg_p, cap);
  for (long j = blockIdx.x * (long) blockDim.x + threadIdx.x; j < n_seg; j += (long) gridDim.x * blockDim.x) {
    u64 m = keys[3 * j + 2] & ((1ull << TJ_META_SAMPLE_SHIFT) - 1ull);
    m = (m & ~(0xFFFFFull << TJ_META_COUNT_SHIFT)) | (((u64) totals[j] & 0xFFFFFull) << TJ_META_COUNT_SHIFT);
    m = (m & ~(7ull << TJ_META_FLAG_SHIFT)) | ((u64) (orflags[j] & 7u) << TJ_META_FLAG_SHIFT);
    keys[3 * j + 2] = m;
  }
}



struct DevBuf
{
  void *p = nullptr;
  size_t cap = 0;
};

#define TJ_SCAN_PIECE_TARGET (1ull << 30)

struct DevState { alignas (256) DevCounters ctr; alignas (256) FinCounts fin; alignas (256) u32 cursors[TJ_P + 1]; alignas (256) FinPlan plan;
                  alignas (256) DevCounters snap_ctr; alignas (256) u32 snap_cursors[TJ_P + 1]; alignas (256) u32 pad[4]; };

struct StageTimer
{
  hipEvent_t e0 = nullptr, e1 = nullptr;
  bool timed = false;
  hipError_t create () { const hipError_t e = hipEventCreate (&e0); return e != hipSuccess ? e : hipEventCreate (&e1); }
  void destroy () { if (e0) (void) hipEventDestroy (e0); if (e1) (void) hipEventDestroy (e1); }
  hipError_t begin (hipStream_t stream) { return hipEventRecord (e0, stream); }
  hipError_t end (hipStream_t stream) { return hipEventRecord (e1, stream); }
  bool elapsed (int device, float &ms) const
  { return timed && hipSetDevice (device) == hipSuccess && hipEventSynchronize (e1) == hipSuccess && hipEventElapsedTime (&ms, e0, e1) == hipSuccess; }
  double ms (int device) const { float f = 0.f; return elapsed (device, f) ? (double) f : -1.0; }
};
enum { T_SCAN, T_FIN, T_MERGE, T_TRACT, T_UNION, T_UNION_STATS, T_REF, T_LOCATE, T_LOCATED_TRACTS, T_VARIANTS, T_ANNOTATION, T_TRACT_FEATURES, T_SEED_ORDER, T_LOCATE_GAPPED, T_CODING, T_VARIANT_EFFECTS, T_MERGE_VARIANTS, TJ_N_TIMERS };

struct tjamd_counter
{
  int device = 0, k = 0, W = 4, n_cu = 256;
  hipStream_t own_stream = nullptr, stream = nullptr;
  DevCounters *d_ctr = nullptr, *h_ctr = nullptr;
  DevCounters *d_lctr = nullptr;
  u32 *d_cursors = nullptr, *h_cursors = nullptr;
  DevBuf pool, table, stage, fix, loc, prefix, rawlist, slow;
  DevBuf log, logmeta;
  int log_mode = 1;
  bool log_next_clean[2] = {false, false};
  hipEvent_t ev_p1 = nullptr;
#define TJ_PIECE_EVENTS 64
  hipEvent_t ev_pa[TJ_PIECE_EVENTS] = {}, ev_pb[TJ_PIECE_EVENTS] = {};
  int n_piece_ev = 0;
  StageTimer timer[TJ_N_TIMERS];
  DevBuf ts_cov, ts_aux;
  long union_cand = -1;
  DevBuf ut_tot, ut_lev, ut_fb, ut_slots;
  DevBuf lc_work;
  bool part_timed = false;
  int fast_mode = 1;
  u32 pool_chunks = 0, maxj = 0;
  int ch_shift = -1;
  u64 bucket_bound = 0;
  u64 chunk_bound = 0;
  long n_raw_known = 0;
  u64 raw_bound = 0;
  long n_undefined = 0;
  double slack = 1.0;
  DevBuf alt, hist, flags, segid, headpos, keep, outpos, scan_tmp, kept, idx_i, idx_f, cov, bins, binstart, binctx, ovf, grp_jt, grp_hist, fine;
  u32 bin_rank_max = BS_RANK_MAX;
  FinCounts *d_fin = nullptr, *h_fin = nullptr;
  struct DevState *d_state = nullptr, *h_state = nullptr;
  void *h_kept = nullptr; size_t h_kept_cap = 0;
  bool bins_zeroed = false;
  bool fine_dirty = false;
  bool bins_counted = false;
  long n_kept = 0; int n_idx = 0, coverage = 0, status = -1;
  hipEvent_t ev_done = nullptr;
  hipEvent_t ev_agg = nullptr;
  hipStream_t order_stream = nullptr;
  int fin_pending = 0;
  int fin_rb = 0, fin_mc = 0; bool fin_speculative = false, fin_plan_ahead = false; u64 fin_kept_cap = 0;
  hipEvent_t marks[8] = {nullptr, nullptr, nullptr, nullptr, nullptr, nullptr, nullptr, nullptr};
  unsigned mark_seq = 0;
  long last_scan_launches = 0;
  unsigned scan_seq = 0;
  size_t piece_target = TJ_SCAN_PIECE_TARGET;
  int scan_grid_cap = 0;
  bool buckets_clean = false;
  long plan_mismatches = 0;
  bool ctr_clean = false;
};

static int ensure (DevBuf &b, size_t bytes, hipStream_t stream, size_t keep_bytes = 0)
{
  if (bytes <= b.cap) return TJAMD_OK;
  size_t want = std::max (bytes, b.cap + b.cap / 2);
  void *np = nullptr;
  hipError_t e = hipMalloc (&np, want);
  if (e != hipSuccess && want > bytes) { want = bytes; e = hipMalloc (&np, want); }
  if (e != hipSuccess) return set_err (TJAMD_ERR_HIP, "hipMalloc of %zu bytes failed: %s", want, hipGetErrorString (e));
  if (b.p) {
    if (keep_bytes) HIPCHK (hipMemcpyAsync (np, b.p, keep_bytes, hipMemcpyDeviceToDevice, stream));
    HIPCHK (hipStreamSynchronize (stream));
    HIPCHK (hipFree (b.p));
  }
  b.p = np; b.cap = want;
  return TJAMD_OK;
}

static void release (DevBuf &b) { if (b.p) (void) hipFree (b.p); b.p = nullptr; b.cap = 0; }

struct Stage
{
  tjamd_counter *c; StageTimer *t;
  Stage (tjamd_counter *c_, int slot) : c (c_), t (c_ && tjamd_device_count () > 0 ? &c_->timer[slot] : nullptr) { if (t) t->timed = false; }
  void begin () { (void) t->begin (c->stream); }
  void end () { (void) t->end (c->stream); }
  void done () { t->timed = true; }
};

struct ScratchCut
{
  struct Piece { void *at; size_t offset; void (*put) (void *at, char *p); } piece[16];
  int n = 0; size_t used = 0;
  template <class T> void take (T *&p, size_t count)
  {
    p = nullptr;
    if (n < 16) piece[n] = Piece {&p, used, [] (void *at, char *q) { *(T **) at = (T *) q; }};
    n++; used += (count * sizeof (T) + 255) & ~(size_t) 255;
  }
  int commit (tjamd_counter *c)
  {
    if (n > 16) return set_err (TJAMD_ERR_STATE, "a scratch cut of %d pieces (16 at most)", n);
    const int rc = ensure (c->lc_work, used, c->stream);
    for (int i = 0; i < n && !rc; i++) piece[i].put (piece[i].at, (char *) c->lc_work.p + piece[i].offset);
    return rc;
  }
};

static int read_back (tjamd_counter *c, const char *fn, const void *d, void *h, size_t words)
{
  hipError_t e = hipGetLastError ();
  if (e == hipSuccess && words) e = hipMemcpyAsync (h, d, words * 4, hipMemcpyDeviceToHost, c->stream);
  if (e == hipSuccess) e = hipStreamSynchronize (c->stream);
  return e == hipSuccess ? TJAMD_OK : set_err (TJAMD_ERR_HIP, "%s: failed: %s", fn, hipGetErrorString (e));
}

extern "C" tjamd_counter *tjamd_counter_create (int device, int kmer_size)
{
  int n = tjamd_device_count ();
  if (n <= 0) { set_err (TJAMD_ERR_NO_DEVICE, "no HIP device visible: the homopolymer-tract engine needs an MI355X (no CPU fallback)"); return NULL; }
  if (device < 0 || device >= n) { set_err (TJAMD_ERR_ARG, "device %d out of range [0,%d)", device, n); return NULL; }
  if (kmer_size < 2 || kmer_size > 32) { set_err (TJAMD_ERR_ARG, "kmer_size %d outside [2,32] (reference clamp: src/main.c:184-185)", kmer_size); return NULL; }
  HIPCHK_NULL (hipSetDevice (device));
  tjamd_counter *c = new tjamd_counter ();
  c->device = device; c->k = kmer_size;
  c->W = (kmer_size <= 12) ? 1 : (kmer_size <= 28) ? 2 : 4;
  hipDeviceProp_t prop;
  HIPCHK_NULL (hipGetDeviceProperties (&prop, device));
  c->n_cu = prop.multiProcessorCount > 0 ? prop.multiProcessorCount : 256;
  const char *bm = getenv ("TATAJUBA_AMD_BIN_MAX");
  if (bm && atoi (bm) >= 1 && atoi (bm) <= BS_RANK_MAX) c->bin_rank_max = (u32) atoi (bm);
  const char *pc = getenv ("TATAJUBA_AMD_SCAN_PIECE");
  if (pc && atol (pc) >= 4096) c->piece_target = (size_t) atol (pc);
  const char *sk = getenv ("TATAJUBA_AMD_SINK");
  if (sk && !strcmp (sk, "fused")) c->log_mode = 0;
  if (sk && !strcmp (sk, "log")) c->log_mode = 2;
  const char *fm = getenv ("TATAJUBA_AMD_FAST");
  if (fm && atoi (fm) >= 0 && atoi (fm) <= 2) c->fast_mode = atoi (fm);
  const char *sg = getenv ("TATAJUBA_AMD_SCAN_GRID");
  if (sg && atoi (sg) >= 1) c->scan_grid_cap = atoi (sg);
  const char *sl = getenv ("TATAJUBA_AMD_BUCKET_SLACK");
  if (sl && atof (sl) >= 1.0) c->slack = atof (sl);
  HIPCHK_NULL (hipStreamCreateWithFlags (&c->own_stream, hipStreamNonBlocking));
  c->stream = c->own_stream;
  HIPCHK_NULL (hipMalloc ((void **) &c->d_state, sizeof (DevState)));
  HIPCHK_NULL (hipMalloc ((void **) &c->d_lctr, sizeof (DevCounters)));
  HIPCHK_NULL (hipHostMalloc ((void **) &c->h_state, sizeof (DevState), hipHostMallocDefault));
  c->d_ctr = &c->d_state->ctr; c->d_fin = &c->d_state->fin;
  HIPCHK_NULL (hipMalloc ((void **) &c->d_cursors, (size_t) (TJ_P + 1) * TJ_CSTRIDE * 4));
  HIPCHK_NULL (hipMemsetAsync (c->d_cursors, 0, (size_t) (TJ_P + 1) * TJ_CSTRIDE * 4, c->stream));
  c->h_ctr = &c->h_state->ctr; c->h_fin = &c->h_state->fin; c->h_cursors = c->h_state->cursors;
  memset (c->h_state, 0, sizeof (DevState));
  HIPCHK_NULL (hipMemsetAsync (c->d_state, 0, sizeof (DevState), c->stream));
  HIPCHK_NULL (hipMemsetAsync (c->d_lctr, 0, sizeof (DevCounters), c->stream));
  for (StageTimer &t : c->timer) HIPCHK_NULL (t.create ());
  HIPCHK_NULL (hipEventCreate (&c->ev_p1));
  HIPCHK_NULL (hipEventCreateWithFlags (&c->ev_done, hipEventDisableTiming));
  HIPCHK_NULL (hipEventCreateWithFlags (&c->ev_agg, hipEventDisableTiming));
  HIPCHK_NULL (hipStreamSynchronize (c->stream));
  return c;
}

extern "C" void tjamd_counter_destroy (tjamd_counter *c)
{
  if (!c) return;
  (void) hipSetDevice (c->device);
  (void) hipStreamSynchronize (c->stream);
  DevBuf *all[] = {&c->log, &c->logmeta, &c->pool, &c->table, &c->stage, &c->fix, &c->loc, &c->prefix, &c->rawlist, &c->slow, &c->alt, &c->hist, &c->flags, &c->segid, &c->headpos,
                   &c->keep, &c->outpos, &c->scan_tmp, &c->kept, &c->idx_i, &c->idx_f, &c->cov, &c->bins, &c->binstart, &c->binctx, &c->ovf, &c->grp_jt, &c->grp_hist, &c->fine,
                   &c->ts_cov, &c->ts_aux, &c->ut_tot, &c->ut_lev, &c->ut_fb, &c->ut_slots, &c->lc_work};
  for (DevBuf *b : all) release (*b);
  for (hipEvent_t ev : c->marks) if (ev) (void) hipEventDestroy (ev);
  if (c->d_state) (void) hipFree (c->d_state);
  if (c->d_lctr) (void) hipFree (c->d_lctr);
  if (c->d_cursors) (void) hipFree (c->d_cursors);
  if (c->h_state) (void) hipHostFree (c->h_state);
  if (c->h_kept) (void) hipHostFree (c->h_kept);
  for (StageTimer &t : c->timer) t.destroy ();
  if (c->ev_p1) (void) hipEventDestroy (c->ev_p1);
  for (int i = 0; i < TJ_PIECE_EVENTS; i++) { if (c->ev_pa[i]) (void) hipEventDestroy (c->ev_pa[i]); if (c->ev_pb[i]) (void) hipEventDestroy (c->ev_pb[i]); }
  if (c->ev_done) (void) hipEventDestroy (c->ev_done);
  if (c->ev_agg) (void) hipEventDestroy (c->ev_agg);
  if (c->own_stream) (void) hipStreamDestroy (c->own_stream);
  delete c;
}

extern "C" int tjamd_counter_device (const tjamd_counter *c) { return c ? c->device : -1; }

extern "C" int tjamd_counter_set_stream (tjamd_counter *c, void *hip_stream)
{
  if (!c) return set_err (TJAMD_ERR_ARG, "null counter");
  HIPCHK (hipSetDevice (c->device));
  HIPCHK (hipStreamSynchronize (c->stream));
  c->stream = hip_stream ? (hipStream_t) hip_stream : c->own_stream;
  return TJAMD_OK;
}

extern "C" int tjamd_counter_set_order_stream (tjamd_counter *c, void *hip_stream)
{
  if (!c) return set_err (TJAMD_ERR_ARG, "null counter");
  HIPCHK (hipSetDevice (c->device));
  HIPCHK (hipStreamSynchronize (c->stream));
  if (c->order_stream) HIPCHK (hipStreamSynchronize (c->order_stream));
  c->order_stream = (hipStream_t) hip_stream;
  return TJAMD_OK;
}

static Buckets make_buckets (const tjamd_counter *c)
{
  Buckets B;
  B.pool = (u64 *) c->pool.p; B.table = (u32 *) c->table.p; B.cursors = c->d_cursors; B.pool_next = c->d_cursors + TJ_P * TJ_CSTRIDE;
  B.pool_chunks = c->pool_chunks; B.maxj = c->maxj; B.ch_shift = (u32) std::max (c->ch_shift, 0);
  return B;
}

static int clear_buckets (tjamd_counter *c, bool snapshot = false)
{
  if (!c->buckets_clean || snapshot) {
    const bool fused = snapshot && c->fine_dirty && c->bins.p != nullptr;
    hipLaunchKernelGGL (clear_buckets_kernel, dim3 (TJ_P), dim3 (256), 0, c->stream, c->d_cursors, c->d_ctr,
                        (u32 *) (c->maxj ? c->table.p : nullptr), c->maxj, c->ch_shift, c->d_fin, (u32 *) c->bins.p, c->bins.p ? BS_MAXBINS : 0,
                        snapshot ? &c->d_state->snap_ctr : (DevCounters *) nullptr, snapshot ? c->d_state->snap_cursors : (u32 *) nullptr,
                        snapshot ? &c->d_state->plan : (FinPlan *) nullptr, fused ? (u32 *) c->fine.p : (u32 *) nullptr, fine_bin_bits (c->k));
    HIPCHK (hipGetLastError ());
    c->buckets_clean = true;
    c->ctr_clean = true;
    c->bins_zeroed = c->bins.p != nullptr && !fused;
    if (fused) { c->fine_dirty = false; c->bins_counted = true; }
  }
  c->n_raw_known = 0; c->raw_bound = 0; c->bucket_bound = 0; c->chunk_bound = TJ_P; c->ch_shift = -1;
  return TJAMD_OK;
}

extern "C" int tjamd_counter_reset (tjamd_counter *c)
{
  if (!c) return set_err (TJAMD_ERR_ARG, "null counter");
  HIPCHK (hipSetDevice (c->device));
  if (!(c->ctr_clean && c->fin_pending == 0 && c->n_undefined == 0)) HIPCHK (hipMemsetAsync (c->d_ctr, 0, sizeof (DevCounters), c->stream));
  int rc = clear_buckets (c);
  c->ctr_clean = true;
  if (rc) return rc;
  c->n_undefined = 0;
  c->n_kept = 0; c->n_idx = 0; c->coverage = 0; c->status = -1;
  return TJAMD_OK;
}

extern "C" void *tjamd_host_alloc (size_t bytes)
{
  void *p = nullptr;
  if (hipHostMalloc (&p, bytes, hipHostMallocPortable) != hipSuccess) { set_err (TJAMD_ERR_HIP, "hipHostMalloc of %zu bytes failed", bytes); return NULL; }
  return p;
}

extern "C" void tjamd_host_free (void *p) { if (p) (void) hipHostFree (p); }

extern "C" void *tjamd_device_alloc (tjamd_counter *c, size_t bytes)
{
  void *p = nullptr;
  if (!c || hipSetDevice (c->device) != hipSuccess || hipMalloc (&p, bytes ? bytes : 1) != hipSuccess) { set_err (TJAMD_ERR_HIP, "hipMalloc of %zu bytes failed", bytes); return NULL; }
  return p;
}
extern "C" void tjamd_device_free (tjamd_counter *c, void *p) { if (c && p && hipSetDevice (c->device) == hipSuccess) (void) hipFree (p); }
extern "C" int tjamd_device_download (tjamd_counter *c, void *host, const void *dev, size_t bytes)
{
  if (!c || (bytes && (!host || !dev))) return set_err (TJAMD_ERR_ARG, "bad arguments");
  HIPCHK (hipSetDevice (c->device));
  HIPCHK (hipStreamSynchronize (c->stream));
  if (bytes) HIPCHK (hipMemcpy (host, dev, bytes, hipMemcpyDeviceToHost));
  return TJAMD_OK;
}

extern "C" int tjamd_sync (tjamd_counter *c)
{
  if (!c) return set_err (TJAMD_ERR_ARG, "null counter");
  HIPCHK (hipSetDevice (c->device));
  HIPCHK (hipStreamSynchronize (c->stream));
  return TJAMD_OK;
}

extern "C" int tjamd_mark (tjamd_counter *c)
{
  if (!c) return -set_err (TJAMD_ERR_ARG, "null counter");
  if (hipSetDevice (c->device) != hipSuccess) return -set_err (TJAMD_ERR_HIP, "hipSetDevice failed");
  const int slot = (int) (c->mark_seq++ & 7u);
  if (!c->marks[slot] && hipEventCreateWithFlags (&c->marks[slot], hipEventDisableTiming) != hipSuccess) return -set_err (TJAMD_ERR_HIP, "hipEventCreate failed");
  if (hipEventRecord (c->marks[slot], c->stream) != hipSuccess) return -set_err (TJAMD_ERR_HIP, "hipEventRecord failed");
  return slot;
}

extern "C" int tjamd_wait_mark (tjamd_counter *c, int mark)
{
  if (!c || mark < 0 || mark > 7 || !c->marks[mark]) return set_err (TJAMD_ERR_ARG, "bad mark");
  HIPCHK (hipSetDevice (c->device));
  HIPCHK (hipEventSynchronize (c->marks[mark]));
  return TJAMD_OK;
}

__global__ void pack_cursors_kernel (const u32 *__restrict__ cursors, u32 *__restrict__ packed)
{
  if (threadIdx.x <= TJ_P) packed[threadIdx.x] = cursors[threadIdx.x * TJ_CSTRIDE];
}

static int queue_counter_copies (tjamd_counter *c)
{
  hipLaunchKernelGGL (pack_cursors_kernel, dim3 (1), dim3 (320), 0, c->stream, (const u32 *) c->d_cursors, c->d_state->cursors);
  HIPCHK (hipGetLastError ());
  HIPCHK (hipMemcpyAsync (c->h_state, c->d_state, sizeof (DevState), hipMemcpyDeviceToHost, c->stream));
  return TJAMD_OK;
}

static int apply_counter_copies (tjamd_counter *c, bool from_snapshot = false)
{
  long total = 0;
  u64 mx = 0;
  struct View { const DevCounters *h_ctr; const u32 *h_cursors; } v = {c->h_ctr, c->h_cursors};
  if (from_snapshot) { v.h_ctr = &c->h_state->snap_ctr; v.h_cursors = c->h_state->snap_cursors; }
  for (int b = 0; b < TJ_P; b++) { total += v.h_cursors[b]; mx = std::max<u64> (mx, v.h_cursors[b]); }
  if (v.h_ctr->overflow == 2u)
    return set_err (TJAMD_ERR_HIP, "a chunk of raw record storage was claimed but its id was never published (waited %u polls): "
                    "the claiming workgroup did not make progress -- please report; scanning again usually succeeds", (unsigned) TJ_SPIN_MAX);
  if (v.h_ctr->overflow)
    return set_err (TJAMD_ERR_CAPACITY, "raw record storage exhausted (%u of %u chunks handed out, fullest bucket %llu records): "
                    "raise TATAJUBA_AMD_BUCKET_SLACK (now %.1f) and scan again", v.h_cursors[TJ_P], c->pool_chunks, (unsigned long long) mx, c->slack);
  if (v.h_ctr->fix_overflow) return set_err (TJAMD_ERR_CAPACITY, "too many non-ACGTU tract candidates in one batch (%llu)",
                                             (unsigned long long) std::max (v.h_ctr->lc[0].n_fix, v.h_ctr->lc[1].n_fix));
  c->n_raw_known = total - (long) v.h_ctr->n_null;
  c->raw_bound = (u64) c->n_raw_known;
  c->bucket_bound = mx;
  c->chunk_bound = v.h_cursors[TJ_P];
  c->n_undefined = (long) v.h_ctr->n_undefined;
  return TJAMD_OK;
}

static int sync_counters (tjamd_counter *c)
{
  int rc = queue_counter_copies (c);
  if (rc) return rc;
  HIPCHK (hipStreamSynchronize (c->stream));
  return apply_counter_copies (c);
}

static void choose_chunk_size (tjamd_counter *c, u64 records)
{
  if (c->ch_shift >= 0) return;
  const u64 units = records / (16384ull * TJ_CH0);
  int sft = 3;
  static_assert ((TJ_CH0 << 3) > (int) TJ_LOGB, "a run of one log block crosses at most one chunk boundary");
  while ((1ull << sft) < units) sft++;
  c->ch_shift = sft;
}

static int ensure_table (tjamd_counter *c, u64 need_maxj)
{
  if (need_maxj > c->maxj) {
    const u32 nmaxj = (u32) std::max<u64> (need_maxj, (u64) c->maxj + c->maxj / 2);
    void *np = nullptr;
// ... 277 lines not shown
extern "C" long tjamd_undefined_runs (tjamd_counter *c)
{
  if (tjamd_raw_count (c) < 0) return -1;
  return c->n_undefined;
}

extern "C" long tjamd_download_raw (tjamd_counter *c, tjamd_record *out, long capacity)
{
  long n = tjamd_raw_count (c);
  if (n < 0) return n;
  if (n > capacity) return -set_err (TJAMD_ERR_CAPACITY, "%ld raw records, caller capacity %ld", n, capacity);
  if (n == 0) return 0;
  int rc = ensure (c->prefix, 64, c->stream);
  if (!rc) rc = ensure (c->rawlist, (size_t) n * 24, c->stream);
  if (rc) return -rc;
  if (hipMemsetAsync (c->prefix.p, 0, 8, c->stream) != hipSuccess) return -set_err (TJAMD_ERR_HIP, "memset failed");
  const Buckets BK = make_buckets (c);
  switch (c->W) {
    case 1: hipLaunchKernelGGL (unpack_buckets_kernel<1>, dim3 (TJ_P), dim3 (256), 0, c->stream, BK, c->k, (u64 *) c->rawlist.p, (u64) n, (u64 *) c->prefix.p); break;
    case 2: hipLaunchKernelGGL (unpack_buckets_kernel<2>, dim3 (TJ_P), dim3 (256), 0, c->stream, BK, c->k, (u64 *) c->rawlist.p, (u64) n, (u64 *) c->prefix.p); break;
    default: hipLaunchKernelGGL (unpack_buckets_kernel<4>, dim3 (TJ_P), dim3 (256), 0, c->stream, BK, c->k, (u64 *) c->rawlist.p, (u64) n, (u64 *) c->prefix.p); break;
  }
  u64 n_out = 0;
  if (hipGetLastError () != hipSuccess || hipStreamSynchronize (c->stream) != hipSuccess ||
      hipMemcpy (&n_out, c->prefix.p, 8, hipMemcpyDeviceToHost) != hipSuccess ||
      hipMemcpy (out, c->rawlist.p, (size_t) n * 24, hipMemcpyDeviceToHost) != hipSuccess) return -set_err (TJAMD_ERR_HIP, "raw download failed");
  if ((long) n_out != n) return -set_err (TJAMD_ERR_STATE, "raw download found %llu records, cursors say %ld", (unsigned long long) n_out, n);
  return n;
}

extern "C" int tjamd_upload_raw (tjamd_counter *c, const hopo_element *elems, long n)
{
  if (!c || (n && !elems) || n < 0) return set_err (TJAMD_ERR_ARG, "bad arguments");
  if (n == 0) return TJAMD_OK;
  HIPCHK (hipSetDevice (c->device));
  int rc = sync_counters (c);
  if (!rc) rc = ensure_buckets (c, (u64) n, 0);
  c->raw_bound += (u64) n;
  if (!rc) rc = ensure (c->stage, (size_t) n * 40, c->stream);
  if (rc) return rc;
  HIPCHK (hipMemcpyAsync (c->stage.p, elems, (size_t) n * 40, hipMemcpyHostToDevice, c->stream));
  const unsigned grid = (unsigned) std::min<long> ((n + 255) / 256, 2048);
  const Buckets BK = make_buckets (c);
  switch (c->W) {
    case 1: hipLaunchKernelGGL (bin_elems_kernel<1>, dim3 (grid), dim3 (256), 0, c->stream, (const u64 *) c->stage.p, n, c->k, BK, c->d_ctr); break;
    case 2: hipLaunchKernelGGL (bin_elems_kernel<2>, dim3 (grid), dim3 (256), 0, c->stream, (const u64 *) c->stage.p, n, c->k, BK, c->d_ctr); break;
    default: hipLaunchKernelGGL (bin_elems_kernel<4>, dim3 (grid), dim3 (256), 0, c->stream, (const u64 *) c->stage.p, n, c->k, BK, c->d_ctr); break;
  }
  HIPCHK (hipGetLastError ());
  c->status = -1;
  return sync_counters (c);
}


static int exclusive_scan (tjamd_counter *c, const u32 *in, u32 *out, long n, u32 *total_out, u32 *tmp, size_t tmp_words)
{
  if (n <= 0) return TJAMD_OK;
  long nblk = (n + SC_ITEMS - 1) / SC_ITEMS;
  if (nblk == 1) {
    hipLaunchKernelGGL (scan_apply_kernel, dim3 (1), dim3 (256), 0, c->stream, in, out, n, (const u32 *) nullptr, total_out);
    HIPCHK (hipGetLastError ());
    return TJAMD_OK;
  }
  if ((size_t) nblk > tmp_words) return set_err (TJAMD_ERR_STATE, "scan scratch too small");
  hipLaunchKernelGGL (scan_reduce_kernel, dim3 ((unsigned) nblk), dim3 (256), 0, c->stream, in, n, tmp);
  HIPCHK (hipGetLastError ());
  int rc = exclusive_scan (c, tmp, tmp, nblk, nullptr, tmp + nblk, tmp_words - (size_t) nblk);
  if (rc) return rc;
  hipLaunchKernelGGL (scan_apply_kernel, dim3 ((unsigned) nblk), dim3 (256), 0, c->stream, in, out, n, (const u32 *) tmp, total_out);
  HIPCHK (hipGetLastError ());
  return TJAMD_OK;
}

static size_t scan_tmp_words (long n)
{
  size_t w = 8;
  while (n > SC_ITEMS) { n = (n + SC_ITEMS - 1) / SC_ITEMS; w += (size_t) n; }
  return w;
}

static int radix_sort_records (tjamd_counter *c, u64 *&a, u64 *&b, long n)
{
  const int passes = key_passes (c->k);
  const int nblk = (int) ((n + RS_ITEMS - 1) / RS_ITEMS);
  const long nh = 256l * nblk;
  int rc = ensure (c->hist, (size_t) nh * 4, c->stream);
  if (!rc) rc = ensure (c->scan_tmp, std::max (scan_tmp_words (nh), scan_tmp_words (n)) * 4, c->stream);
  if (rc) return rc;
  for (int p = 0; p < passes; p++) {
    hipLaunchKernelGGL (radix_count_kernel, dim3 (nblk), dim3 (256), 0, c->stream, (const u64 *) a, n, p, c->k, (u32 *) c->hist.p, nblk);
    HIPCHK (hipGetLastError ());
    rc = exclusive_scan (c, (const u32 *) c->hist.p, (u32 *) c->hist.p, nh, nullptr, (u32 *) c->scan_tmp.p, c->scan_tmp.cap / 4);
    if (rc) return rc;
    hipLaunchKernelGGL (radix_scatter_kernel, dim3 (nblk), dim3 (256), 0, c->stream, (const u64 *) a, b, n, p, c->k, (const u32 *) c->hist.p, nblk);
    HIPCHK (hipGetLastError ());
    std::swap (a, b);
  }
  return TJAMD_OK;
}

static unsigned grid_for (long n) { return (unsigned) std::max<long> (1, std::min<long> ((n + 255) / 256, 4096)); }



static int finalise_radix (tjamd_counter *c, long n1, int min_coverage)
{
  int rc = ensure (c->alt, (size_t) n1 * 24, c->stream);
  if (!rc) rc = ensure (c->flags, (size_t) n1 * 4, c->stream);
  if (!rc) rc = ensure (c->segid, (size_t) n1 * 4, c->stream);
  if (!rc) rc = ensure (c->headpos, (size_t) n1 * 4, c->stream);
  if (!rc) rc = ensure (c->keep, (size_t) n1 * 4, c->stream);
  if (!rc) rc = ensure (c->outpos, (size_t) n1 * 4, c->stream);
  if (!rc) rc = ensure (c->scan_tmp, scan_tmp_words (n1) * 4, c->stream);
  if (rc) return rc;
  u64 *a = (u64 *) c->kept.p, *b = (u64 *) c->alt.p;
  rc = radix_sort_records (c, a, b, n1);
  if (rc) return rc;
  if (a != (u64 *) c->kept.p) std::swap (c->kept, c->alt);

  const u64 *kept = (const u64 *) c->kept.p;
  u32 *flags = (u32 *) c->flags.p, *segid = (u32 *) c->segid.p, *headpos = (u32 *) c->headpos.p;
  u32 *keep = (u32 *) c->keep.p, *outpos = (u32 *) c->outpos.p;
  hipLaunchKernelGGL (seg_heads_kernel, dim3 (grid_for (n1)), dim3 (256), 0, c->stream, kept, n1, flags, 1);
  HIPCHK (hipGetLastError ());
  rc = exclusive_scan (c, flags, segid, n1, &c->d_fin->n_ctx, (u32 *) c->scan_tmp.p, c->scan_tmp.cap / 4);
  if (rc) return rc;
  hipLaunchKernelGGL (seg_headpos_kernel, dim3 (grid_for (n1)), dim3 (256), 0, c->stream, (const u32 *) flags, (const u32 *) segid, n1, headpos);
  HIPCHK (hipGetLastError ());
  hipLaunchKernelGGL (ctx_decide_kernel, dim3 (grid_for (n1)), dim3 (256), 0, c->stream, kept, n1, (const u32 *) headpos,
                      (const u32 *) &c->d_fin->n_ctx, min_coverage, keep);
  HIPCHK (hipGetLastError ());
  HIPCHK (hipMemcpyAsync (c->h_fin, c->d_fin, sizeof (FinCounts), hipMemcpyDeviceToHost, c->stream));
  HIPCHK (hipStreamSynchronize (c->stream));
  const long n_ctx = c->h_fin->n_ctx;
  rc = exclusive_scan (c, keep, outpos, n_ctx, &c->d_fin->n_idx, (u32 *) c->scan_tmp.p, c->scan_tmp.cap / 4);
  if (!rc) rc = ensure (c->idx_i, (size_t) n_ctx * 4, c->stream);
  if (!rc) rc = ensure (c->idx_f, (size_t) n_ctx * 4, c->stream);
  if (rc) return rc;
  hipLaunchKernelGGL (ctx_write_kernel, dim3 (grid_for (n_ctx)), dim3 (256), 0, c->stream, n1, (const u32 *) headpos, (const u32 *) &c->d_fin->n_ctx,
                      (const u32 *) keep, (const u32 *) outpos, (int *) c->idx_i.p, (int *) c->idx_f.p);
  HIPCHK (hipGetLastError ());

  const int log2t = cov_table_bits (n1);
  const long t = 1l << log2t;
  rc = ensure (c->cov, (size_t) t * 8, c->stream);
  if (rc) return rc;
  u64 *ctab = (u64 *) c->cov.p;
  HIPCHK (hipMemsetAsync (c->cov.p, 0, (size_t) t * 8, c->stream));
  hipLaunchKernelGGL (set_int_kernel, dim3 (1), dim3 (1), 0, c->stream, &c->d_fin->coverage, INT_MIN);
  hipLaunchKernelGGL (cov_insert_kernel, dim3 (grid_for (2 * n1)), dim3 (256), 0, c->stream, kept, n1, ctab, log2t);
  HIPCHK (hipGetLastError ());
  hipLaunchKernelGGL (cov_max_kernel, dim3 (std::min<unsigned> (grid_for (t), 256u)), dim3 (256), 0, c->stream, (const u64 *) ctab, t, &c->d_fin->coverage);
  HIPCHK (hipGetLastError ());
  HIPCHK (c->timer[T_FIN].end (c->stream));
  c->timer[T_FIN].timed = true;
  HIPCHK (hipMemcpyAsync (c->h_fin, c->d_fin, sizeof (FinCounts), hipMemcpyDeviceToHost, c->stream));
  HIPCHK (hipStreamSynchronize (c->stream));
  return TJAMD_OK;
}

static int finalise_binned (tjamd_counter *c, long n1, int min_coverage, long cap = 0, bool wait = true)
{
  const bool planned = n1 == 0;
  const bool aside = planned && !wait && c->order_stream != nullptr && c->order_stream != c->stream;
  const hipStream_t st = aside ? c->order_stream : c->stream;
  const FinPlan *plan = planned ? &c->d_state->plan : nullptr;
  if (planned) n1 = cap;
  const int nbits = bin_bits_for (n1, c->k);
  const int nbins = planned ? BS_MAXBINS : 1 << nbits;
  int cov_direct = 0;
  const int log2t = planned ? cov_table_bits (n1) : cov_plan_bits (n1, c->k, &cov_direct);
  const long t = 1l << log2t;
  const bool fused = planned && c->bins_counted;
  c->bins_counted = false;
  int rc = ensure (c->alt, (size_t) n1 * 24, c->stream);
  if (!rc && !c->bins.p) { rc = ensure (c->bins, (size_t) (BS_MAXBINS + 1) * 4, c->stream); c->bins_zeroed = false; }
  if (!rc) rc = ensure (c->binstart, (size_t) (nbins + 1) * 4, c->stream);
  if (!rc) rc = ensure (c->binctx, (size_t) nbins * 8, c->stream);
  if (!rc) rc = ensure (c->headpos, (size_t) n1 * 4, c->stream);
  if (!rc) rc = ensure (c->outpos, (size_t) n1 * 4, c->stream);
  if (!rc) rc = ensure (c->idx_i, (size_t) n1 * 4, c->stream);
  if (!rc) rc = ensure (c->idx_f, (size_t) n1 * 4, c->stream);
  if (!rc) rc = ensure (c->cov, (size_t) t * 8, c->stream);
  if (rc) return rc;
  u32 *bins = (u32 *) c->bins.p, *binstart = (u32 *) c->binstart.p, *binctx = (u32 *) c->binctx.p, *binout = binctx + nbins;
  u32 *tstart = (u32 *) c->headpos.p, *tend = (u32 *) c->outpos.p;
  u64 *ctab = (u64 *) c->cov.p;
  if (!fused && !c->bins_zeroed) HIPCHK (hipMemsetAsync (bins, 0, (size_t) BS_MAXBINS * 4, c->stream));
  c->bins_zeroed = false;
  if (aside) { HIPCHK (hipEventRecord (c->ev_agg, c->stream)); HIPCHK (hipStreamWaitEvent (st, c->ev_agg, 0)); }
  const unsigned g1 = planned ? std::min<unsigned> (grid_for (n1), 2048u) : grid_for (n1);
  if (!fused) hipLaunchKernelGGL (bin_count_kernel, dim3 (g1), dim3 (256), 0, st, (const u64 *) c->kept.p, n1, c->k, nbits, bins,
                                  (uint4 *) c->cov.p, (long) (t / 2), 0, plan);
  hipLaunchKernelGGL (bin_scan_kernel, dim3 (1), dim3 (1024), 0, st, bins, nbins, binstart, c->bin_rank_max, c->d_fin, plan);
  hipLaunchKernelGGL (bin_scatter_kernel, dim3 (g1), dim3 (256), 0, st, (const u64 *) c->kept.p, (u64 *) c->alt.p, n1, c->k, nbits, bins, plan,
                      fused ? (uint4 *) c->cov.p : (uint4 *) nullptr);
  hipLaunchKernelGGL (bin_sort_index_kernel, dim3 ((unsigned) std::min (nbins / BSI_WAVES + 1, 16384)), dim3 (64 * BSI_WAVES), 0, st,
                      (const u64 *) c->alt.p, (u64 *) c->kept.p, (const u32 *) binstart, nbins, (const FinCounts *) c->d_fin, min_coverage,
                      ctab, log2t, binctx, tstart, tend, plan, cov_direct);
  hipLaunchKernelGGL (bin_ctx_scan_kernel, dim3 (1), dim3 (1024), 0, st, (const u32 *) binctx, nbins, binout, c->d_fin, plan);
  hipLaunchKernelGGL (bin_ctx_write_kernel, dim3 (256), dim3 (256), 0, st, (const u32 *) binstart, (const u32 *) binctx, (const u32 *) binout, nbins,
                      (const u32 *) tstart, (const u32 *) tend, (int *) c->idx_i.p, (int *) c->idx_f.p, (const u64 *) ctab, t, c->d_fin, plan);
  HIPCHK (hipGetLastError ());
  HIPCHK (c->timer[T_FIN].end (st));
  c->timer[T_FIN].timed = true;
  if (planned) HIPCHK (hipMemcpyAsync (c->h_state, c->d_state, sizeof (DevState), hipMemcpyDeviceToHost, st));
  else HIPCHK (hipMemcpyAsync (c->h_fin, c->d_fin, sizeof (FinCounts), hipMemcpyDeviceToHost, c->stream));
  if (wait) HIPCHK (hipStreamSynchronize (c->stream));
  else HIPCHK (hipEventRecord (c->ev_done, st));
  return TJAMD_OK;
}

static int finalise_impl (tjamd_counter *c, int remove_biased, int min_coverage, int *status, int phase);

extern "C" int tjamd_finalise (tjamd_counter *c, int remove_biased, int min_coverage, int *status)
{
  int rc = finalise_impl (c, remove_biased, min_coverage, status, 0);
  return rc;
}
extern "C" int tjamd_finalise_begin (tjamd_counter *c, int remove_biased, int min_coverage)
{
  const int rc = finalise_impl (c, remove_biased, min_coverage, nullptr, 1);
  if (!rc && c->fin_pending == 0) c->fin_pending = 3;
  return rc;
}
extern "C" int tjamd_finalise_end (tjamd_counter *c, int *status)
{
  if (!c) return set_err (TJAMD_ERR_ARG, "null counter");
  if (!c->fin_pending) return set_err (TJAMD_ERR_STATE, "tjamd_finalise_end without tjamd_finalise_begin");
  if (c->fin_pending == 3) { c->fin_pending = 0; if (status) *status = c->status; return TJAMD_OK; }
  return finalise_impl (c, c->fin_rb, c->fin_mc, status, 2);
}

static int finalise_impl (tjamd_counter *c, int remove_biased, int min_coverage, int *status, int phase)
{
  if (!c) return set_err (TJAMD_ERR_ARG, "null counter");
  HIPCHK (hipSetDevice (c->device));
  bool speculative = c->fin_speculative, plan_ahead = c->fin_plan_ahead;
  u64 kept_cap = c->fin_kept_cap;
  int rc = TJAMD_OK;
  if (phase == 2) goto second_half;
  c->fin_pending = 0;
  {
  c->n_kept = 0; c->n_idx = 0; c->coverage = 0; c->timer[T_FIN].timed = false;
  speculative = (c->raw_bound / 2 + 1) * 24 <= (8ull << 30);
  kept_cap = c->raw_bound / 2 + 1;
  if (!speculative) {
    rc = sync_counters (c);
    if (rc) return rc;
    if (c->n_raw_known == 0) { c->status = 1; if (status) *status = 1; return TJAMD_OK; }
    if (c->n_raw_known >= (1l << 31)) return set_err (TJAMD_ERR_CAPACITY, "%ld raw records exceed the reference's int n_elem", c->n_raw_known);
    kept_cap = (u64) c->n_raw_known / 2 + 1;
  }

  rc = ensure (c->kept, (size_t) kept_cap * 24, c->stream);
  if (!rc) rc = ensure (c->ovf, c->pool.cap, c->stream);
  if (rc) return rc;
  HIPCHK (c->timer[T_FIN].begin (c->stream));
  const Buckets BK = make_buckets (c);
  long plan_cap = (long) std::min<u64> (kept_cap, std::max<u64> (kept_cap / 8, 1u << 16));
  if (const char *pc = getenv ("TATAJUBA_AMD_PLAN_CAP")) plan_cap = std::max (1l, std::min (plan_cap, atol (pc)));
  plan_ahead = speculative && getenv ("TATAJUBA_AMD_NO_PLAN") == nullptr;
  FinPlan *const d_plan = plan_ahead ? &c->d_state->plan : nullptr;
  u32 *fine = nullptr;
  if (plan_ahead && getenv ("TATAJUBA_AMD_NO_FUSED_BINS") == nullptr) {
    const bool fresh = c->fine.p == nullptr;
    rc = ensure (c->fine, (size_t) BS_MAXBINS * 4, c->stream);
    if (rc) return rc;
    if (fresh || c->fine_dirty) HIPCHK (hipMemsetAsync (c->fine.p, 0, (size_t) BS_MAXBINS * 4, c->stream));
    if (!c->bins.p) { rc = ensure (c->bins, (size_t) (BS_MAXBINS + 1) * 4, c->stream); c->bins_zeroed = false; if (rc) return rc; }
    fine = (u32 *) c->fine.p;
    c->fine_dirty = true;
  }
  const int fbits = fine_bin_bits (c->k);
  switch (c->W) {
    case 1: hipLaunchKernelGGL (aggregate1_kernel, dim3 (TJ_P), dim3 (AG_BLOCK), 0, c->stream, BK, (u64 *) c->ovf.p, c->k, remove_biased, (u64 *) c->kept.p, kept_cap, c->d_fin, plan_cap, d_plan, fine, fbits); break;
    case 2: hipLaunchKernelGGL (aggregate2_kernel, dim3 (TJ_P), dim3 (AG_BLOCK), 0, c->stream, BK, (u64 *) c->ovf.p, c->k, remove_biased, (u64 *) c->kept.p, kept_cap, c->d_fin, plan_cap, d_plan, fine, fbits); break;
    default: hipLaunchKernelGGL (aggregate4_kernel, dim3 (TJ_P), dim3 (AG_BLOCK), 0, c->stream, BK, (u64 *) c->ovf.p, c->k, remove_biased, (u64 *) c->kept.p, kept_cap, c->d_fin, plan_cap, d_plan, fine, fbits); break;
  }
  HIPCHK (hipGetLastError ());
  rc = plan_ahead ? TJAMD_OK : queue_counter_copies (c);
  if (!rc) rc = clear_buckets (c, plan_ahead);
  if (rc) return rc;
  c->fin_rb = remove_biased; c->fin_mc = min_coverage; c->fin_speculative = speculative; c->fin_plan_ahead = plan_ahead; c->fin_kept_cap = kept_cap;
  if (plan_ahead) { rc = finalise_binned (c, 0, min_coverage, plan_cap, phase != 1); if (rc) return rc; }
  else HIPCHK (hipStreamSynchronize (c->stream));
  }
  if (phase == 1) { c->fin_pending = plan_ahead ? 1 : 2; return TJAMD_OK; }
second_half:
  if (phase == 2) {
    if (c->fin_pending == 1) HIPCHK (hipEventSynchronize (c->ev_done));
    c->fin_pending = 0;
  }
  if (speculative) {
    rc = apply_counter_copies (c, plan_ahead);
    const long n = c->n_raw_known;
    c->n_raw_known = 0; c->raw_bound = 0; c->bucket_bound = 0; c->chunk_bound = TJ_P;
    if (rc) return rc;
    if (n == 0) { c->status = 1; if (status) *status = 1; return TJAMD_OK; }
    if (n >= (1l << 31)) return set_err (TJAMD_ERR_CAPACITY, "%ld raw records exceed the reference's int n_elem", n);
  }
  if (plan_ahead) {
    FinPlan &pl = c->h_state->plan;
    if (pl.n1 != pl.n1_exact || pl.kept_overflow != pl.ovf_exact) {
      c->plan_mismatches++;
      pl.n1 = pl.n1_exact; pl.kept_overflow = pl.ovf_exact; pl.ok = 0;
    }
  }
  if (plan_ahead ? c->h_state->plan.kept_overflow : c->h_fin->overflow) return set_err (TJAMD_ERR_CAPACITY, "kept list overflow");
  const long n1 = plan_ahead ? c->h_state->plan.n1 : (long) c->h_fin->n_kept;
  if (n1 == 0) {
    HIPCHK (c->timer[T_FIN].end (c->stream)); c->timer[T_FIN].timed = true;
    c->status = 2; if (status) *status = 2; return TJAMD_OK;
  }

  c->n_kept = n1;
  if (!(plan_ahead && c->h_state->plan.ok)) rc = finalise_binned (c, n1, min_coverage);
  if (!rc && c->h_fin->sort_fallback) rc = finalise_radix (c, n1, min_coverage);
  if (rc) return rc;
  c->n_idx = (int) c->h_fin->n_idx;
  if (c->n_idx == 0) { c->status = 3; if (status) *status = 3; return TJAMD_OK; }
  c->coverage = c->h_fin->coverage;
  c->status = 0;
  if (status) *status = 0;
  return TJAMD_OK;
}

extern "C" long tjamd_kept_count (tjamd_counter *c) { return c ? c->n_kept : -1; }
extern "C" int tjamd_n_idx (tjamd_counter *c) { return c ? c->n_idx : -1; }
extern "C" int tjamd_coverage (tjamd_counter *c) { return c ? c->coverage : -1; }
extern "C" const void *tjamd_kept_device_ptr (tjamd_counter *c) { return c ? c->kept.p : NULL; }

extern "C" long tjamd_download_kept (tjamd_counter *c, hopo_element *out, long capacity)
{
  if (!c) return -set_err (TJAMD_ERR_ARG, "null counter");
  if (c->status < 0) return -set_err (TJAMD_ERR_STATE, "counter not finalised");
  const long n1 = c->n_kept;
  if (n1 > capacity) return -set_err (TJAMD_ERR_CAPACITY, "%ld kept records, caller capacity %ld", n1, capacity);
  if (n1 == 0) return 0;
  if (hipSetDevice (c->device) != hipSuccess) return -set_err (TJAMD_ERR_HIP, "hipSetDevice failed");
  if ((size_t) n1 * 24 > c->h_kept_cap) {
    if (c->h_kept) (void) hipHostFree (c->h_kept);
    c->h_kept = nullptr; c->h_kept_cap = 0;
    const size_t want = (size_t) n1 * 24 + ((size_t) n1 * 24 >> 2) + 4096;
    if (hipHostMalloc (&c->h_kept, want, hipHostMallocDefault) != hipSuccess) { c->h_kept = nullptr; return -set_err (TJAMD_ERR_HIP, "hipHostMalloc of %zu bytes failed", want); }
    c->h_kept_cap = want;
  }
  const tjamd_record *tmp = (const tjamd_record *) c->h_kept;
  if (hipMemcpyAsync (c->h_kept, c->kept.p, (size_t) n1 * 24, hipMemcpyDeviceToHost, c->stream) != hipSuccess ||
      hipStreamSynchronize (c->stream) != hipSuccess) return -set_err (TJAMD_ERR_HIP, "download failed");
  for (long i = 0; i < n1; i++) {
    out[i].context[0] = tmp[i].ctx0; out[i].context[1] = tmp[i].ctx1;
    memcpy ((char *) &out[i] + 16, &tmp[i].meta, 8);
    out[i].read_offset = -1;
    out[i].loc_ref_id = out[i].loc_pos = out[i].loc_last = -1;
  }
  return n1;
}

extern "C" long tjamd_download_idx (tjamd_counter *c, int *idx_initial, int *idx_final, long capacity)
{
  if (!c) return -set_err (TJAMD_ERR_ARG, "null counter");
  if (c->status < 0) return -set_err (TJAMD_ERR_STATE, "counter not finalised");
  const long n = c->n_idx;
  if (n > capacity) return -set_err (TJAMD_ERR_CAPACITY, "%ld index ranges, caller capacity %ld", n, capacity);
  if (n == 0) return 0;
  if (hipSetDevice (c->device) != hipSuccess) return -set_err (TJAMD_ERR_HIP, "hipSetDevice failed");
  if (hipMemcpy (idx_initial, c->idx_i.p, (size_t) n * 4, hipMemcpyDeviceToHost) != hipSuccess ||
      hipMemcpy (idx_final, c->idx_f.p, (size_t) n * 4, hipMemcpyDeviceToHost) != hipSuccess) return -set_err (TJAMD_ERR_HIP, "download failed");
  return n;
}

extern "C" double tjamd_last_scan_ms (tjamd_counter *c)
{
  float ms = 0.f;
  if (!c || !c->timer[T_SCAN].elapsed (c->device, ms)) return -1.0;
  for (int i = 0; i < c->n_piece_ev; i++) { float p = 0.f; if (hipEventElapsedTime (&p, c->ev_pa[i], c->ev_pb[i]) == hipSuccess) ms -= p; }
  return (double) ms;
}

extern "C" double tjamd_last_merge_ms (tjamd_counter *c) { return c ? c->timer[T_MERGE].ms (c->device) : -1.0; }

extern "C" int tjamd_counter_uses_log (const tjamd_counter *c) { return (c && c->W <= c->log_mode && c->fast_mode) ? 1 : 0; }

extern "C" double tjamd_last_partition_ms (tjamd_counter *c)
{
  if (!c || !c->timer[T_SCAN].timed) return -1.0;
  if (!c->part_timed) return 0.0;
  float ms = 0.f;
  if (hipSetDevice (c->device) != hipSuccess || hipEventSynchronize (c->ev_p1) != hipSuccess || hipEventElapsedTime (&ms, c->timer[T_SCAN].e1, c->ev_p1) != hipSuccess) return -1.0;
  for (int i = 0; i < c->n_piece_ev; i++) { float p = 0.f; if (hipEventElapsedTime (&p, c->ev_pa[i], c->ev_pb[i]) == hipSuccess) ms += p; }
  return (double) ms;
}

extern "C" double tjamd_last_finalise_ms (tjamd_counter *c) { return c ? c->timer[T_FIN].ms (c->device) : -1.0; }

extern "C" long tjamd_last_scan_launches (tjamd_counter *c) { return c ? c->last_scan_launches : -1; }
extern "C" long tjamd_plan_mismatches (tjamd_counter *c) { return c ? c->plan_mismatches : -1; }

static long merge_samples_radix (tjamd_counter *c, const void *d_records, long n, int n_samples, void *d_out_keys, void *d_out_counts, long capacity);


__device__ __forceinline__ int flank_hamming (u64 a, u64 b)
{
  const u64 d = a ^ b;
  return __popcll ((d | (d >> 1)) & 0x5555555555555555ull);
}

__global__ void group_back_kernel (const u64 *__restrict__ kept, long n, int maxd, int *__restrict__ back)
{
  for (long i = blockIdx.x * (long) blockDim.x + threadIdx.x; i < n; i += (long) gridDim.x * blockDim.x) {
    const u64 c0 = kept[3 * i], c1 = kept[3 * i + 1], base = kept[3 * i + 2] & 3ull;
    long j = i - 1;
    while (j >= 0 && (kept[3 * j + 2] & 3ull) == base && flank_hamming (kept[3 * j], c0) + flank_hamming (kept[3 * j + 1], c1) < maxd) j--;
    back[i] = (int) j;
  }
}

__global__ void group_resolve_kernel (const int *__restrict__ back, long n, u32 *__restrict__ head)
{
  for (long i = blockIdx.x * (long) blockDim.x + threadIdx.x; i < n; i += (long) gridDim.x * blockDim.x) {
    if (back[i] != (int) i - 1) continue;
    head[i] = 1u;
    long start = i;
    for (long j = i + 1; j < n && back[j] != (int) j - 1; j++) {
      if (start > (long) back[j]) head[j] = 0u;
      else { head[j] = 1u; start = j; }
    }
  }
}

struct GroupOut { int first, n_elem, n_context, mode; long long integral; };

__global__ void group_summary_kernel (const u64 *__restrict__ kept, long n, const u32 *__restrict__ head, const u32 *__restrict__ gid_excl,
                                      int *__restrict__ group_of, GroupOut *__restrict__ groups)
{
  for (long i = blockIdx.x * (long) blockDim.x + threadIdx.x; i < n; i += (long) gridDim.x * blockDim.x) {
    if (!head[i]) continue;
    const int g = (int) gid_excl[i];
    GroupOut o = {(int) i, 0, 0, (int) i, 0};
    int mode_count = 0;
    for (long j = i; j < n && (j == i || !head[j]); j++) {
      const u64 m = kept[3 * j + 2];
      const int cnt = meta_count (m);
      if (j == i || kept[3 * j] != kept[3 * (j - 1)] || kept[3 * j + 1] != kept[3 * (j - 1) + 1]) o.n_context++;
      if (j == i || mode_count < cnt) { mode_count = cnt; o.mode = (int) j; }
      o.integral += cnt; o.n_elem++;
      group_of[j] = g;
    }
    groups[g] = o;
  }
}


__device__ __forceinline__ u32 name_symbol (u64 c0, u64 c1, u32 base, int k, int t)
{
  if (t < k) return (u32) (c0 >> (2 * t)) & 3u;
  if (t == k + 1) return base;
  if (t < k + 3) return 4u;
  return (u32) (c1 >> (2 * (t - k - 3))) & 3u;
}

__device__ int name_edit_distance (const u64 *__restrict__ kept, long a, long b, int k, int free_end)
{
  const u64 a0 = kept[3 * a], a1 = kept[3 * a + 1], b0 = kept[3 * b], b1 = kept[3 * b + 1];
  const u32 ab = (u32) (kept[3 * a + 2] & 3ull), bb = (u32) (kept[3 * b + 2] & 3ull);
  const int n = 2 * k + 3;
  unsigned char row[2 * 32 + 4];
  for (int y = 0; y <= n; y++) row[y] = (unsigned char) y;
  int early = n;
  for (int x = 1; x <= n; x++) {
    const u32 sb = name_symbol (b0, b1, bb, k, x - 1);
    int diag = row[0];
    row[0] = (unsigned char) x;
    for (int y = 1; y <= n; y++) {
      const int up = row[y];
      int best = diag + (name_symbol (a0, a1, ab, k, y - 1) == sb ? 0 : 1);
      best = min (best, min ((int) row[y - 1], up) + 1);
      diag = up; row[y] = (unsigned char) best;
    }
    early = min (early, (int) row[n]);
  }
  int result = row[n];
  if (free_end) {
    result = min (result, early);
    for (int y = 0; y <= n; y++) result = min (result, (int) row[y]);
  }
  return result;
}

#define GJ_ADDS_CONTEXT(t) ((t) != 1)

struct MetaCount { __device__ __forceinline__ int operator() (const u64 *__restrict__ kept, long i) const { return meta_count (kept[3 * i + 2]); } };
struct TotalCount
{
  const long long *__restrict__ total;
  __device__ __forceinline__ long long operator() (const u64 *__restrict__, long i) const { return total[i]; }
};

template <class CountOf>
__global__ void group_speculate_kernel (const u64 *__restrict__ kept, long n, int k, int lev, int free_end, const u32 *__restrict__ head,
                                        u32 *__restrict__ cand, int *__restrict__ jt, u32 *__restrict__ n_cand, CountOf count_of)
{
  for (long i = blockIdx.x * (long) blockDim.x + threadIdx.x; i < n; i += (long) gridDim.x * blockDim.x) {
    u32 c = 0;
    jt[i] = head[i] ? 0 : ((kept[3 * i] == kept[3 * (i - 1)] && kept[3 * i + 1] == kept[3 * (i - 1) + 1]) ? 1 : 5);
    if (head[i] && i > 0 && ((kept[3 * i + 2] ^ kept[3 * (i - 1) + 2]) & 3ull) == 0ull) {
      long ph = i - 1;
      while (!head[ph]) ph--;
      long mode = ph;
      auto mc = count_of (kept, ph);
      for (long j = ph + 1; j < i; j++) { const auto cj = count_of (kept, j); if (cj > mc) { mc = cj; mode = j; } }
      if (name_edit_distance (kept, mode, i, k, free_end) < lev) { c = 1u; atomicAdd (n_cand, 1u); }
    }
    cand[i] = c;
  }
}

#define GR_CHUNK 4096
template <class CountOf>
__global__ __launch_bounds__ (256)
void group_repair_kernel (const u64 *__restrict__ kept, long n, int k, int maxd, int lev, int free_end,
                          u32 *__restrict__ head, const u32 *__restrict__ cand, int *__restrict__ jt, CountOf count_of, int *__restrict__ lev_of)
{
  __shared__ long s_pos, s_min;
  if (threadIdx.x == 0) s_pos = 0;
  __syncthreads ();
  for (;;) {
    const long start = s_pos;
    if (start >= n) break;
    if (threadIdx.x == 0) s_min = n;
    __syncthreads ();
    const long end = min (n, start + (long) GR_CHUNK);
    for (long i = start + threadIdx.x; i < end; i += blockDim.x)
      if (cand[i]) { atomicMin ((unsigned long long *) &s_min, (unsigned long long) i); break; }
    __syncthreads ();
    const long h = s_min;
    if (threadIdx.x == 0) {
      if (h >= n) s_pos = end;
      else {
        long hd = h - 1;
        while (!head[hd]) hd--;
        long mode = hd;
        auto mc = count_of (kept, hd);
        for (long j = hd + 1; j < h; j++) { const auto cj = count_of (kept, j); if (cj > mc) { mc = cj; mode = j; } }
        long i = h;
        while (i < n) {
          if ((kept[3 * i + 2] ^ kept[3 * hd + 2]) & 3ull) break;
// ... 780 lines not shown
  rc = exclusive_scan (c, vf, (u32 *) c->outpos.p, nt, total, (u32 *) c->scan_tmp.p, c->scan_tmp.cap / 4);
  if (!rc) rc = exclusive_scan (c, sf, (u32 *) c->headpos.p, nt, total + 1, (u32 *) c->scan_tmp.p, c->scan_tmp.cap / 4);
  if (rc) return -rc;
  if (d_var) hipLaunchKernelGGL (tract_var_scatter_kernel, dim3 (grid_for (nt)), dim3 (256), 0, c->stream, (const u32 *) vf, (const u32 *) c->outpos.p, nt, d_var);
  if (d_sel) hipLaunchKernelGGL (tract_var_scatter_kernel, dim3 (grid_for (nt)), dim3 (256), 0, c->stream, (const u32 *) sf, (const u32 *) c->headpos.p, nt, d_sel);
  if (hipGetLastError () != hipSuccess) return -set_err (TJAMD_ERR_HIP, "%s: list launch failed", fn);
  st.end ();
  int h_err = 0;
  u32 h_tot[2] = {0, 0};
  if (hipMemcpyAsync (&h_err, err, 4, hipMemcpyDeviceToHost, c->stream) != hipSuccess || hipMemcpyAsync (h_tot, total, 8, hipMemcpyDeviceToHost, c->stream) != hipSuccess ||
      hipStreamSynchronize (c->stream) != hipSuccess) return -set_err (TJAMD_ERR_HIP, "%s: failed: %s", fn, hipGetErrorString (hipGetLastError ()));
  if (h_err) return -set_err (TJAMD_ERR_ARG, "%s: the tracts must tile the union (first 0, each starting where the one before ends, the last ending at row %ld)", fn, n_union);
  st.done ();
  if (n_var) *n_var = (long) h_tot[0];
  if (n_sel) *n_sel = (long) h_tot[1];
  return nt;
}

extern "C" long tjamd_union_tract_sample_stats (tjamd_counter *c, const void *d_keys, const void *d_counts, long n_union, int n_samples,
                                                const int *coverage, const tjamd_union_tract_summary *d_summary, long n_tracts,
                                                const int *d_list, long n_list, double *d_values, int *d_modal_len, int *d_n_context, int *d_n_len)
{
  static const char *fn = "tjamd_union_tract_sample_stats";
  int rc = tract_args (fn, d_keys, d_counts, n_union, n_samples, coverage);
  if (rc) return -rc;
  if (n_list < 0 || n_tracts < 0 || n_tracts > n_union) return -set_err (TJAMD_ERR_ARG, "%s: n_list %ld, n_tracts %ld (union of %ld rows)", fn, n_list, n_tracts, n_union);
  if (n_list > 0 && (!d_summary || !d_list || !d_values)) return -set_err (TJAMD_ERR_ARG, "%s: null summary, list or values buffer", fn);
  if (!c) return -set_err (TJAMD_ERR_ARG, "%s: null counter", fn);
  if (hipSetDevice (c->device) != hipSuccess) return -set_err (TJAMD_ERR_HIP, "hipSetDevice failed");
  if (n_list == 0) return 0;
  long long *g_cnt = nullptr;
  int *g_len = nullptr;
  rc = ensure_union_fallback (c, n_list, g_cnt, g_len);
  if (!rc) rc = upload_coverage (c, coverage, n_samples);
  if (rc) return -rc;
  const int S = tract_segment (n_samples);
  int *err = (int *) c->ts_aux.p, h_err = 0;
  auto launch = [&] (auto kernel, unsigned grid) {
    hipLaunchKernelGGL (kernel, dim3 (grid), dim3 (256), 0, c->stream, (const u64 *) d_keys, (const int *) d_counts, n_union, n_samples, S, (const int *) c->ts_cov.p,
                        (const UnionSummary *) d_summary, n_tracts, d_list, n_list, d_values, d_modal_len, d_n_context, d_n_len, (u32 *) c->ut_fb.p, g_cnt, g_len, err);
  };
  launch (union_tract_sample_stats_kernel<false>, tract_grid (n_list, S));
  launch (union_tract_sample_stats_kernel<true>, (unsigned) UT_FULL_BLOCKS);
  rc = read_back (c, fn, err, &h_err, 1);
  if (rc) return -rc;
  if (h_err) return -set_err (TJAMD_ERR_ARG, "%s: a listed tract id is outside [0, %ld) or its rows outside the union", fn, n_tracts);
  return n_list;
}

extern "C" double tjamd_last_union_tracts_ms (tjamd_counter *c) { return c ? c->timer[T_UNION].ms (c->device) : -1.0; }

extern "C" long tjamd_last_union_tract_candidates (tjamd_counter *c) { return c ? c->union_cand : -1; }

extern "C" double tjamd_last_union_tract_stats_ms (tjamd_counter *c) { return c ? c->timer[T_UNION_STATS].ms (c->device) : -1.0; }

static std::mutex g_peer_mutex;
static signed char g_peer[64][64];
static int peer_access (int dst_dev, int src_dev)
{
  if (dst_dev == src_dev) return 1;
  if (dst_dev < 0 || src_dev < 0 || dst_dev >= 64 || src_dev >= 64) return 0;
  std::lock_guard<std::mutex> lock (g_peer_mutex);
  if (g_peer[dst_dev][src_dev]) return g_peer[dst_dev][src_dev] > 0;
  int can = 0, prev = -1;
  (void) hipGetDevice (&prev);
  if (hipDeviceCanAccessPeer (&can, dst_dev, src_dev) == hipSuccess && can && hipSetDevice (dst_dev) == hipSuccess) {
    const hipError_t e = hipDeviceEnablePeerAccess (src_dev, 0);
    can = (e == hipSuccess || e == hipErrorPeerAccessAlreadyEnabled);
    (void) hipGetLastError ();
  }
  else can = 0;
  if (prev >= 0) (void) hipSetDevice (prev);
  g_peer[dst_dev][src_dev] = can ? 1 : -1;
  return can;
}

extern "C" int tjamd_peer_access_report (char *out, int capacity)
{
  int staged = 0, at = 0;
  std::lock_guard<std::mutex> lock (g_peer_mutex);
  if (out && capacity > 0) out[0] = 0;
  for (int d = 0; d < 64; d++)
    for (int sdev = 0; sdev < 64; sdev++)
      if (g_peer[d][sdev]) {
        if (g_peer[d][sdev] < 0) staged++;
        if (out && at < capacity - 24) at += snprintf (out + at, (size_t) (capacity - at), "%d<-%d:%s ", d, sdev, g_peer[d][sdev] > 0 ? "direct" : "staged");
      }
  return staged;
}

extern "C" long tjamd_gather_histograms (tjamd_counter *dst, tjamd_counter *const *samples, int n_samples, const void **d_records, long *counts)
{
  if (!dst || !samples || n_samples < 1 || !d_records || !counts) return -set_err (TJAMD_ERR_ARG, "bad arguments");
  long n = 0;
  for (int i = 0; i < n_samples; i++) {
    if (!samples[i] || samples[i]->status < 0) return -set_err (TJAMD_ERR_STATE, "sample %d is not finalised", i);
    counts[i] = samples[i]->n_kept; n += counts[i];
  }
  if (hipSetDevice (dst->device) != hipSuccess) return -set_err (TJAMD_ERR_HIP, "hipSetDevice failed");
  int rc = ensure (dst->rawlist, (size_t) std::max<long> (n, 1) * 24, dst->stream);
  if (rc) return -rc;
  size_t off = 0;
  for (int i = 0; i < n_samples; i++) {
    const size_t bytes = (size_t) counts[i] * 24;
    if (!bytes) continue;
    tjamd_counter *s = samples[i];
    if (s->device != dst->device) peer_access (dst->device, s->device);
    hipError_t e = (s->device == dst->device)
      ? hipMemcpyAsync ((char *) dst->rawlist.p + off, s->kept.p, bytes, hipMemcpyDeviceToDevice, dst->stream)
      : hipMemcpyPeerAsync ((char *) dst->rawlist.p + off, dst->device, s->kept.p, s->device, bytes, dst->stream);
    if (e != hipSuccess) return -set_err (TJAMD_ERR_HIP, "gather copy of sample %d failed: %s", i, hipGetErrorString (e));
    off += bytes;
  }
  if (hipStreamSynchronize (dst->stream) != hipSuccess) return -set_err (TJAMD_ERR_HIP, "gather failed");
  *d_records = dst->rawlist.p;
  return n;
}


extern "C" long tjamd_merge_samples (tjamd_counter *c, const void *d_records, const long *counts, int n_samples,
                                      void *d_out_keys, void *d_out_counts, long capacity)
{
  if (!c || !counts || n_samples < 1 || n_samples > 4096 || !d_out_keys || !d_out_counts) return -set_err (TJAMD_ERR_ARG, "bad arguments");
  if (hipSetDevice (c->device) != hipSuccess) return -set_err (TJAMD_ERR_HIP, "hipSetDevice failed");
  std::vector<long> starts ((size_t) n_samples + 1);
  long n = 0;
  for (int i = 0; i < n_samples; i++) { if (counts[i] < 0) return -set_err (TJAMD_ERR_ARG, "negative count"); starts[i] = n; n += counts[i]; }
  starts[n_samples] = n;
  if (n == 0) return 0;
  if (!d_records) return -set_err (TJAMD_ERR_ARG, "null records");
  if (n >= (1l << 31)) return -set_err (TJAMD_ERR_CAPACITY, "%ld records to merge", n);

  int nbits = 6;
  while (nbits < BS_MAXBITS && nbits < 1 + 4 * c->k && (24l << nbits) < n) nbits++;
  nbits = std::min (nbits, 1 + 4 * c->k);
  const int nbins = 1 << nbits;
  int rc = ensure (c->prefix, (size_t) (n_samples + 1) * 8, c->stream);
  if (!rc) rc = ensure (c->alt, (size_t) n * 24, c->stream);
  if (!rc && !c->bins.p) { rc = ensure (c->bins, (size_t) (BS_MAXBINS + 1) * 4, c->stream); c->bins_zeroed = false; }
  if (!rc) rc = ensure (c->binstart, (size_t) (BS_MAXBINS + 1) * 4, c->stream);
  if (!rc) rc = ensure (c->binctx, (size_t) BS_MAXBINS * 8, c->stream);
  if (!rc) rc = ensure (c->headpos, (size_t) n * 4, c->stream);
  if (!rc) rc = ensure (c->outpos, (size_t) n * 4, c->stream);
  if (rc) return -rc;
  if (hipMemcpyAsync (c->prefix.p, starts.data (), (size_t) (n_samples + 1) * 8, hipMemcpyHostToDevice, c->stream) != hipSuccess ||
      hipStreamSynchronize (c->stream) != hipSuccess) return -set_err (TJAMD_ERR_HIP, "copy failed");
  u32 *bins = (u32 *) c->bins.p, *binstart = (u32 *) c->binstart.p, *binctx = (u32 *) c->binctx.p, *binout = binctx + nbins;
  u32 *tpos = (u32 *) c->headpos.p, *ttot = (u32 *) c->outpos.p;
  if (!c->bins_zeroed && hipMemsetAsync (bins, 0, (size_t) BS_MAXBINS * 4, c->stream) != hipSuccess) return -set_err (TJAMD_ERR_HIP, "memset failed");
  c->bins_zeroed = false;
  Stage st (c, T_MERGE);
  st.begin ();
  hipLaunchKernelGGL (bin_count_kernel, dim3 (grid_for (n)), dim3 (256), 0, c->stream, (const u64 *) d_records, n, c->k, nbits, bins, (uint4 *) nullptr, 0l, 1);
  hipLaunchKernelGGL (bin_scan_kernel, dim3 (1), dim3 (1024), 0, c->stream, bins, nbins, binstart,
                      c->bin_rank_max < (u32) BS_RANK_MAX ? c->bin_rank_max : (u32) MG_RANK_MAX, c->d_fin);
  hipLaunchKernelGGL (merge_scatter_kernel, dim3 (grid_for (n)), dim3 (256), 0, c->stream, (const u64 *) d_records, (u64 *) c->alt.p, n, c->k, nbits, bins,
                      (const long *) c->prefix.p, n_samples);
  hipLaunchKernelGGL (bin_merge_kernel, dim3 ((unsigned) std::min (nbins, 16384)), dim3 (64), 0, c->stream, (const u64 *) c->alt.p, (const u32 *) binstart, nbins,
                      (const FinCounts *) c->d_fin, binctx, tpos, ttot);
  hipLaunchKernelGGL (bin_ctx_scan_kernel, dim3 (1), dim3 (1024), 0, c->stream, (const u32 *) binctx, nbins, binout, c->d_fin);
  hipLaunchKernelGGL (bin_merge_write_kernel, dim3 ((unsigned) std::min (nbins / 4 + 1, 4096)), dim3 (256), 0, c->stream, (const u64 *) c->alt.p, (const u32 *) binstart,
                      (const u32 *) binout, nbins, (const FinCounts *) c->d_fin, (const u32 *) tpos, (const u32 *) ttot, n_samples,
                      (u64 *) d_out_keys, (int *) d_out_counts, capacity);
  if (hipGetLastError () != hipSuccess) return -set_err (TJAMD_ERR_HIP, "merge launch failed");
  st.end ();
  st.done ();
  if (hipMemcpyAsync (c->h_fin, c->d_fin, sizeof (FinCounts), hipMemcpyDeviceToHost, c->stream) != hipSuccess ||
      hipStreamSynchronize (c->stream) != hipSuccess) return -set_err (TJAMD_ERR_HIP, "merge failed: %s", hipGetErrorString (hipGetLastError ()));
  if (c->h_fin->sort_fallback) return merge_samples_radix (c, d_records, n, n_samples, d_out_keys, d_out_counts, capacity);
  const long n_union = c->h_fin->n_idx;
  if (n_union > capacity) return -set_err (TJAMD_ERR_CAPACITY, "%ld union keys, caller capacity %ld", n_union, capacity);
  return n_union;
}

static long merge_samples_radix (tjamd_counter *c, const void *d_records, long n, int n_samples, void *d_out_keys, void *d_out_counts, long capacity)
{
  int rc = ensure (c->rawlist, (size_t) n * 24, c->stream);
  if (!rc) rc = ensure (c->alt, (size_t) n * 24, c->stream);
  if (!rc) rc = ensure (c->flags, (size_t) n * 4, c->stream);
  if (!rc) rc = ensure (c->segid, (size_t) n * 4, c->stream);
  if (!rc) rc = ensure (c->keep, (size_t) n * 8, c->stream);
  if (!rc) rc = ensure (c->scan_tmp, scan_tmp_words (n) * 4, c->stream);
  if (rc) return -rc;
  hipLaunchKernelGGL (merge_tag_kernel, dim3 (grid_for (n)), dim3 (256), 0, c->stream, (const u64 *) d_records, (u64 *) c->rawlist.p, n, (const long *) c->prefix.p, n_samples);
  u64 *a = (u64 *) c->rawlist.p, *b = (u64 *) c->alt.p;
  rc = radix_sort_records (c, a, b, n);
  if (rc) return -rc;
  if (a != (u64 *) c->rawlist.p) std::swap (c->rawlist, c->alt);
  u32 *flags = (u32 *) c->flags.p, *segid = (u32 *) c->segid.p;
  hipLaunchKernelGGL (seg_heads_kernel, dim3 (grid_for (n)), dim3 (256), 0, c->stream, (const u64 *) a, n, flags, 0);
  rc = exclusive_scan (c, flags, segid, n, &c->d_fin->n_seg, (u32 *) c->scan_tmp.p, c->scan_tmp.cap / 4);
  if (rc) return -rc;
  if (hipMemcpyAsync (c->h_fin, c->d_fin, sizeof (FinCounts), hipMemcpyDeviceToHost, c->stream) != hipSuccess ||
      hipStreamSynchronize (c->stream) != hipSuccess) return -set_err (TJAMD_ERR_HIP, "merge failed: %s", hipGetErrorString (hipGetLastError ()));
  const long n_union = c->h_fin->n_seg;
  if (n_union > capacity) return -set_err (TJAMD_ERR_CAPACITY, "%ld union keys, caller capacity %ld", n_union, capacity);
  if (hipMemsetAsync (d_out_counts, 0, (size_t) n_union * n_samples * 4, c->stream) != hipSuccess ||
      hipMemsetAsync (c->keep.p, 0, (size_t) n * 8, c->stream) != hipSuccess) return -set_err (TJAMD_ERR_HIP, "memset failed");
  hipLaunchKernelGGL (merge_write_kernel, dim3 (grid_for (n)), dim3 (256), 0, c->stream, (const u64 *) a, n, (const u32 *) flags, (const u32 *) segid,
                      n_samples, (u64 *) d_out_keys, (int *) d_out_counts, (u32 *) c->keep.p, (u32 *) c->keep.p + n, capacity);
  hipLaunchKernelGGL (merge_totals_kernel, dim3 (grid_for (n_union)), dim3 (256), 0, c->stream, (u64 *) d_out_keys, (const u32 *) c->keep.p,
                      (const u32 *) c->keep.p + n, (const u32 *) &c->d_fin->n_seg, capacity);
  if (hipGetLastError () != hipSuccess || hipStreamSynchronize (c->stream) != hipSuccess) return -set_err (TJAMD_ERR_HIP, "merge kernels failed");
  return n_union;
}



struct tjamd_comm
{
  ncclComm_t comm = nullptr;
  int rank = 0, world = 1, device = 0;
  long cap = 0;
  hipStream_t stream = nullptr;
  DevBuf send, recv, out, dcounts;
  long *h_counts = nullptr;
  long exchanges = 0, collectives = 0;
  hipEvent_t ev0 = nullptr, ev1 = nullptr;
  double last_ms = -1.0; long last_bytes = 0, last_collectives = 0;
};

struct RcclApi
{
  const char *(*GetErrorString) (ncclResult_t);
  ncclResult_t (*GetUniqueId) (ncclUniqueId *);
  ncclResult_t (*CommInitRank) (ncclComm_t *, int, ncclUniqueId, int);
  ncclResult_t (*CommDestroy) (ncclComm_t);
  ncclResult_t (*CommCount) (const ncclComm_t, int *);
  ncclResult_t (*CommAbort) (ncclComm_t);
  ncclResult_t (*AllGather) (const void *, void *, size_t, ncclDataType_t, ncclComm_t, hipStream_t);
};

static const RcclApi *rccl_api ()
{
  static RcclApi api;
  static bool ok = false;
  static char why[512] = "";
  static std::once_flag once;
  std::call_once (once, [] () {
    void *h = nullptr;
    std::string tried;
    std::vector<std::string> names;
    if (const char *e = getenv ("TATAJUBA_AMD_RCCL")) names.push_back (e);
    else {
      names.push_back ("librccl.so.1"); names.push_back ("librccl.so");
      const char *rp = getenv ("ROCM_PATH");
      const std::string root = (rp && *rp) ? rp : "/opt/rocm";
      names.push_back (root + "/lib/librccl.so.1"); names.push_back (root + "/lib/librccl.so");
    }
    for (const std::string &nm : names) {
      h = dlopen (nm.c_str (), RTLD_NOW | RTLD_LOCAL);
      if (h) break;
      tried += (tried.empty () ? "" : ", ") + nm;
    }
    if (!h) { snprintf (why, sizeof why, "RCCL not found (tried %s): the exchange between processes needs it", tried.c_str ()); return; }
    struct { const char *name; void **to; } syms[] = {
      {"ncclGetErrorString", (void **) &api.GetErrorString}, {"ncclGetUniqueId", (void **) &api.GetUniqueId},
      {"ncclCommInitRank", (void **) &api.CommInitRank}, {"ncclCommDestroy", (void **) &api.CommDestroy},
      {"ncclCommCount", (void **) &api.CommCount}, {"ncclCommAbort", (void **) &api.CommAbort}, {"ncclAllGather", (void **) &api.AllGather}};
    for (auto &sy : syms) {
      *sy.to = dlsym (h, sy.name);
      if (!*sy.to) { snprintf (why, sizeof why, "RCCL: %s not found in the library that was loaded", sy.name); return; }
    }
    ok = true;
  });
  if (!ok) { set_err (TJAMD_ERR_HIP, "%s", why); return nullptr; }
  return &api;
}

#define NCCLCHK(name, call, ret) do { ncclResult_t r_ = (call); if (r_ != ncclSuccess) { \
  set_err (TJAMD_ERR_HIP, "%s failed: %s", name, NC->GetErrorString (r_)); return ret; } } while (0)

extern "C" int tjamd_comm_unique_id (void *id_bytes)
{
  static_assert (TJAMD_COMM_ID_BYTES == NCCL_UNIQUE_ID_BYTES, "id size");
  if (!id_bytes) return set_err (TJAMD_ERR_ARG, "tjamd_comm_unique_id: null buffer");
  const RcclApi *NC = rccl_api ();
  if (!NC) return TJAMD_ERR_HIP;
  ncclUniqueId id;
  NCCLCHK ("ncclGetUniqueId", NC->GetUniqueId (&id), TJAMD_ERR_HIP);
  memcpy (id_bytes, &id, sizeof id);
  return TJAMD_OK;
}

extern "C" tjamd_comm *tjamd_comm_create (tjamd_counter *c, const void *id_bytes, int rank, int world)
{
  if (!c || !id_bytes || world < 1 || world > 4096 || rank < 0 || rank >= world) { set_err (TJAMD_ERR_ARG, "tjamd_comm_create: bad arguments"); return NULL; }
  const RcclApi *NC = rccl_api ();
  if (!NC) return NULL;
  HIPCHK_NULL (hipSetDevice (c->device));
  tjamd_comm *m = new (std::nothrow) tjamd_comm;
  if (!m) { set_err (TJAMD_ERR_HIP, "out of memory"); return NULL; }
  m->rank = rank; m->world = world; m->device = c->device;
  ncclUniqueId id;
  memcpy (&id, id_bytes, sizeof id);
  ncclResult_t r = NC->CommInitRank (&m->comm, world, id, rank);
  if (r != ncclSuccess) { set_err (TJAMD_ERR_HIP, "ncclCommInitRank failed: %s", NC->GetErrorString (r)); delete m; return NULL; }
  if (hipHostMalloc ((void **) &m->h_counts, (size_t) world * sizeof (long), hipHostMallocDefault) != hipSuccess ||
      hipEventCreate (&m->ev0) != hipSuccess || hipEventCreate (&m->ev1) != hipSuccess) {
    set_err (TJAMD_ERR_HIP, "hipHostMalloc / hipEventCreate failed"); (void) NC->CommDestroy (m->comm); delete m; return NULL;
  }
  return m;
}

extern "C" void tjamd_comm_destroy (tjamd_comm *m)
{
  if (!m) return;
  (void) hipSetDevice (m->device);
  if (m->comm) if (const RcclApi *NC = rccl_api ()) (void) NC->CommDestroy (m->comm);
  release (m->send); release (m->recv); release (m->out); release (m->dcounts);
  if (m->h_counts) (void) hipHostFree (m->h_counts);
  if (m->ev0) (void) hipEventDestroy (m->ev0);
  if (m->ev1) (void) hipEventDestroy (m->ev1);
// ... 1914 lines not shown
```

Baseline: 11.30 billion.

## Rewrite single-block bin scan as 256-thread two-pass vector scan, add owned order stream

Replaces the 1024-thread LDS-chunked exclusive scan used by bin_scan and bin_ctx_scan with a 256-thread kernel. Each wave reduces a contiguous segment with uint4 loads, then rescans it with wave prefix sums, which removes the LDS staging and repeated block barriers. The change also adds an opt-in high-priority owned stream for the planned ordering phase (enabled by TATAJUBA_AMD_ORDER=aside), splits finalise and order timers, and stops using SPARE for BIG==2 staging. The two-pass scan reads the input twice and runs on only four waves, so latency may not fall for large bin counts.

```diff
diff --git a/include/tatajuba_amd.h b/include/tatajuba_amd.h
--- a/include/tatajuba_amd.h
+++ b/include/tatajuba_amd.h
@@ -154,6 +154,7 @@
 int    tjamd_counter_uses_log (const tjamd_counter *c);
 double tjamd_last_partition_ms (tjamd_counter *c);
 double tjamd_last_finalise_ms (tjamd_counter *c);
+double tjamd_last_order_ms (tjamd_counter *c);
 double tjamd_last_merge_ms (tjamd_counter *c);
 double tjamd_last_tract_stats_ms (tjamd_counter *c);
 double tjamd_last_union_tracts_ms (tjamd_counter *c);
diff --git a/tatajuba_amd/capi.py b/tatajuba_amd/capi.py
--- a/tatajuba_amd/capi.py
+++ b/tatajuba_amd/capi.py
@@ -114,7 +114,7 @@
     "tjamd_reference_create", "tjamd_reference_destroy", "tjamd_reference_entries", "tjamd_reference_contigs",
     "tjamd_reference_download", "tjamd_last_reference_ms", "tjamd_locate", "tjamd_last_locate_ms", "tjamd_located_tracts", "tjamd_last_located_tracts_ms",
     "tjamd_last_tract_variants_ms",
-    "tjamd_group_contexts", "tjamd_context_histograms", "tjamd_scan_windows", "tjamd_thread_cleanup", "tjamd_last_scan_ms", "tjamd_last_partition_ms", "tjamd_counter_uses_log", "tjamd_last_finalise_ms", "tjamd_last_scan_launches", "tjamd_plan_mismatches",
+    "tjamd_group_contexts", "tjamd_context_histograms", "tjamd_scan_windows", "tjamd_thread_cleanup", "tjamd_last_scan_ms", "tjamd_last_partition_ms", "tjamd_counter_uses_log", "tjamd_last_finalise_ms", "tjamd_last_order_ms", "tjamd_last_scan_launches", "tjamd_plan_mismatches",
     "tjamd_synth_stream", "tjamd_read_file_stream",
     "new_genomic_context_list", "del_genomic_context_list", "del_context_histogram",
     "distance_between_context_histogram_and_hopo_context", "indel_distance_between_context_histogram_and_hopo_context",
@@ -309,6 +309,7 @@
     L.hopo_counter_histogram_integral.argtypes = [P, C.c_int]
     L.tjamd_last_scan_ms.restype = C.c_double; L.tjamd_last_scan_ms.argtypes = [C.c_void_p]
     L.tjamd_last_finalise_ms.restype = C.c_double; L.tjamd_last_finalise_ms.argtypes = [C.c_void_p]
+    L.tjamd_last_order_ms.restype = C.c_double; L.tjamd_last_order_ms.argtypes = [C.c_void_p]
     L.tjamd_last_partition_ms.restype = C.c_double; L.tjamd_last_partition_ms.argtypes = [C.c_void_p]
     L.tjamd_last_scan_launches.restype = C.c_long; L.tjamd_last_scan_launches.argtypes = [C.c_void_p]
     L.tjamd_synth_stream.restype = C.c_long
@@ -827,6 +828,9 @@
     def last_finalise_ms(self):
         return lib().tjamd_last_finalise_ms(self._h)
 
+    def last_order_ms(self):
+        return lib().tjamd_last_order_ms(self._h)
+
 
 class HopoCounter:
 
diff --git a/tatajuba_amd/csrc/hopo_device.hip b/tatajuba_amd/csrc/hopo_device.hip
--- a/tatajuba_amd/csrc/hopo_device.hip
+++ b/tatajuba_amd/csrc/hopo_device.hip
@@ -743,7 +743,7 @@
   static constexpr int WS = (W == 4) ? 3 : W;
   static constexpr int WORDS = BIG == 2 ? 8192 : BIG ? TJ_STAGE_WORDS * 2 : (W == 1) ? TJ_STAGE_WORDS : 2688;
   static constexpr int S = WORDS / WS;
-  static constexpr int SPARE = BIG ? 64 : 0;
+  static constexpr int SPARE = BIG == 1 ? 64 : 0;
   u64 rec[WORDS + SPARE * WS];
   alignas (16) u64 gbase[TJ_P];
   u64 gbase2[TJ_P];
@@ -2644,42 +2644,73 @@
 }
 
 #define BS_MAXBINS (1 << BS_MAXBITS)
-#define WGS_CHUNK  16384
-
-#define WGS_PAD(i) ((i) + ((i) >> 5))
-struct WgScanLds { u32 a[WGS_CHUNK + WGS_CHUNK / 32 + 1]; u32 wsum[16]; u32 vmax; };
-
-__device__ __forceinline__ u32 wg_exclusive_scan (const u32 *__restrict__ in, int n_all, u32 *__restrict__ out, u32 *__restrict__ out2, WgScanLds &L, u32 &vmax)
-{
-  const int tid = threadIdx.x, lane = tid & 63, wave = tid >> 6;
-  if (tid == 0) L.vmax = 0;
-  u32 carry = 0;
-  for (int base = 0; base < n_all; base += WGS_CHUNK) {
-    const int n = min (WGS_CHUNK, n_all - base);
-    const int per = (n + 1023) / 1024;
-    for (int i = tid; i < n; i += 1024) L.a[WGS_PAD (i)] = in[base + i];
-    __syncthreads ();
-    u32 sum = 0, mx = 0;
-    for (int j = 0; j < per; j++) { const int b = tid * per + j; if (b < n) { const u32 v = L.a[WGS_PAD (b)]; sum += v; mx = max (mx, v); } }
-    const u32 incl = wave_inclusive_scan (sum);
-    if (lane == 63) L.wsum[wave] = incl;
-    for (int o = 32; o > 0; o >>= 1) mx = max (mx, (u32) __shfl_down ((int) mx, o));
-    if (lane == 0 && mx) atomicMax (&L.vmax, mx);
-    __syncthreads ();
-    u32 run = carry + incl - sum, total = 0;
-    for (int w = 0; w < 16; w++) { const u32 x = L.wsum[w]; if (w < wave) run += x; total += x; }
-    for (int j = 0; j < per; j++) { const int b = tid * per + j; if (b < n) { const u32 v = L.a[WGS_PAD (b)]; L.a[WGS_PAD (b)] = run; run += v; } }
-    __syncthreads ();
-    for (int i = tid; i < n; i += 1024) { const u32 v = L.a[WGS_PAD (i)]; out[base + i] = v; if (out2) out2[base + i] = v; }
-    carry += total;
-    __syncthreads ();
-  }
-  vmax = L.vmax;
-  return carry;
-}
-
-__global__ __launch_bounds__ (1024)
-void bin_scan_kernel (u32 *__restrict__ bins, int nbins, u32 *__restrict__ binstart, u32 rank_max, FinCounts *fin, const FinPlan *__restrict__ plan = nullptr)
+#define WGS_BLOCK  256
+#define WGS_AHEAD  4
+
+struct WgScanLds { u32 wsum[WGS_BLOCK / 64], wmax[WGS_BLOCK / 64]; };
+
+__device__ __forceinline__ u32 wg_exclusive_scan (const u32 *in, int n_all, u32 *out, u32 *out2, WgScanLds &L, u32 &vmax)
+{
+  const int tid = threadIdx.x, lane = tid & 63;
+  const int wave = __builtin_amdgcn_readfirstlane (tid >> 6);
+  const int seg = ((n_all + 4 * WGS_BLOCK - 1) / (4 * WGS_BLOCK)) * 256;
+  const int lo = min (wave * seg, n_all), hi = min (lo + seg, n_all);
+  const bool vec = ((((size_t) in) | ((size_t) out) | ((size_t) out2)) & 15) == 0;
+  auto load4 = [&] (int base) -> uint4 {
+    const int i = base + 4 * lane;
+    if (vec && base + 256 <= hi) return *reinterpret_cast<const uint4 *> (in + i);
+    uint4 v = make_uint4 (0, 0, 0, 0);
+    if (i < hi) v.x = in[i];
+    if (i + 1 < hi) v.y = in[i + 1];
+    if (i + 2 < hi) v.z = in[i + 2];
+    if (i + 3 < hi) v.w = in[i + 3];
+    return v;
+  };
+  auto store4 = [&] (u32 *dst, int base, const uint4 &v) {
+    const int i = base + 4 * lane;
+    if (vec && base + 256 <= hi) { *reinterpret_cast<uint4 *> (dst + i) = v; return; }
+    if (i < hi) dst[i] = v.x;
+    if (i + 1 < hi) dst[i + 1] = v.y;
+    if (i + 2 < hi) dst[i + 2] = v.z;
+    if (i + 3 < hi) dst[i + 3] = v.w;
+  };
+  u32 sum = 0, mx = 0;
+  for (int base = lo; base < hi; base += 256 * WGS_AHEAD) {
+    uint4 v[WGS_AHEAD];
+#pragma unroll
+    for (int j = 0; j < WGS_AHEAD; j++) v[j] = load4 (base + 256 * j);
+#pragma unroll
+    for (int j = 0; j < WGS_AHEAD; j++) { sum += v[j].x + v[j].y + v[j].z + v[j].w; mx = max (max (mx, max (v[j].x, v[j].y)), max (v[j].z, v[j].w)); }
+  }
+  const u32 wincl = wave_inclusive_scan (sum);
+  for (int o = 32; o > 0; o >>= 1) mx = max (mx, (u32) __shfl_down ((int) mx, o));
+  if (lane == 63) L.wsum[wave] = wincl;
+  if (lane == 0) L.wmax[wave] = mx;
+  __syncthreads ();
+  u32 carry = 0, total = 0;
+  vmax = 0;
+  for (int w = 0; w < WGS_BLOCK / 64; w++) { const u32 x = L.wsum[w]; if (w < wave) carry += x; total += x; vmax = max (vmax, L.wmax[w]); }
+  for (int base = lo; base < hi; base += 256 * WGS_AHEAD) {
+    uint4 v[WGS_AHEAD];
+#pragma unroll
+    for (int j = 0; j < WGS_AHEAD; j++) v[j] = load4 (base + 256 * j);
+#pragma unroll
+    for (int j = 0; j < WGS_AHEAD; j++) {
+      if (base + 256 * j >= hi) break;
+      const u32 s = v[j].x + v[j].y + v[j].z + v[j].w;
+      const u32 incl = wave_inclusive_scan (s);
+      const u32 e = carry + incl - s;
+      const uint4 o = make_uint4 (e, e + v[j].x, e + v[j].x + v[j].y, e + v[j].x + v[j].y + v[j].z);
+      store4 (out, base + 256 * j, o);
+      if (out2) store4 (out2, base + 256 * j, o);
+      carry += (u32) __shfl ((int) incl, 63);
+    }
+  }
+  return total;
+}
+
+__global__ __launch_bounds__ (WGS_BLOCK)
+void bin_scan_kernel (u32 *bins, int nbins, u32 *binstart, u32 rank_max, FinCounts *fin, const FinPlan *__restrict__ plan = nullptr)
 {
   __shared__ WgScanLds L;
   u32 vmax;
@@ -3064,8 +3095,8 @@
   }
 }
 
-__global__ __launch_bounds__ (1024)
-void bin_ctx_scan_kernel (const u32 *__restrict__ binctx, int nbins, u32 *__restrict__ binout, FinCounts *fin, const FinPlan *__restrict__ plan = nullptr)
+__global__ __launch_bounds__ (WGS_BLOCK)
+void bin_ctx_scan_kernel (const u32 *binctx, int nbins, u32 *binout, FinCounts *fin, const FinPlan *__restrict__ plan = nullptr)
 {
   __shared__ WgScanLds L;
   u32 vmax;
@@ -3298,7 +3329,7 @@
   { return timed && hipSetDevice (device) == hipSuccess && hipEventSynchronize (e1) == hipSuccess && hipEventElapsedTime (&ms, e0, e1) == hipSuccess; }
   double ms (int device) const { float f = 0.f; return elapsed (device, f) ? (double) f : -1.0; }
 };
-enum { T_SCAN, T_FIN, T_MERGE, T_TRACT, T_UNION, T_UNION_STATS, T_REF, T_LOCATE, T_LOCATED_TRACTS, T_VARIANTS, T_ANNOTATION, T_TRACT_FEATURES, T_SEED_ORDER, T_LOCATE_GAPPED, T_CODING, T_VARIANT_EFFECTS, T_MERGE_VARIANTS, TJ_N_TIMERS };
+enum { T_SCAN, T_FIN, T_ORDER, T_MERGE, T_TRACT, T_UNION, T_UNION_STATS, T_REF, T_LOCATE, T_LOCATED_TRACTS, T_VARIANTS, T_ANNOTATION, T_TRACT_FEATURES, T_SEED_ORDER, T_LOCATE_GAPPED, T_CODING, T_VARIANT_EFFECTS, T_MERGE_VARIANTS, TJ_N_TIMERS };
 
 struct tjamd_counter
 {
@@ -3340,8 +3371,9 @@
   bool bins_counted = false;
   long n_kept = 0; int n_idx = 0, coverage = 0, status = -1;
   hipEvent_t ev_done = nullptr;
-  hipEvent_t ev_agg = nullptr;
-  hipStream_t order_stream = nullptr;
+  hipStream_t order_stream = nullptr, order_own = nullptr;
+  bool order_owned = false;
+  bool order_aside = false;
   int fin_pending = 0;
   int fin_rb = 0, fin_mc = 0; bool fin_speculative = false, fin_plan_ahead = false; u64 fin_kept_cap = 0;
   hipEvent_t marks[8] = {nullptr, nullptr, nullptr, nullptr, nullptr, nullptr, nullptr, nullptr};
@@ -3451,7 +3483,8 @@
   for (StageTimer &t : c->timer) HIPCHK_NULL (t.create ());
   HIPCHK_NULL (hipEventCreate (&c->ev_p1));
   HIPCHK_NULL (hipEventCreateWithFlags (&c->ev_done, hipEventDisableTiming));
-  HIPCHK_NULL (hipEventCreateWithFlags (&c->ev_agg, hipEventDisableTiming));
+  const char *om = getenv ("TATAJUBA_AMD_ORDER");
+  if (om && !strcmp (om, "aside")) c->order_owned = true;
   HIPCHK_NULL (hipStreamSynchronize (c->stream));
   return c;
 }
@@ -3461,6 +3494,8 @@
   if (!c) return;
   (void) hipSetDevice (c->device);
   (void) hipStreamSynchronize (c->stream);
+  if (c->fin_pending == 1) (void) hipEventSynchronize (c->ev_done);
+  if (c->order_own) { (void) hipStreamSynchronize (c->order_own); (void) hipStreamDestroy (c->order_own); }
   DevBuf *all[] = {&c->log, &c->logmeta, &c->pool, &c->table, &c->stage, &c->fix, &c->loc, &c->prefix, &c->rawlist, &c->slow, &c->alt, &c->hist, &c->flags, &c->segid, &c->headpos,
                    &c->keep, &c->outpos, &c->scan_tmp, &c->kept, &c->idx_i, &c->idx_f, &c->cov, &c->bins, &c->binstart, &c->binctx, &c->ovf, &c->grp_jt, &c->grp_hist, &c->fine,
                    &c->ts_cov, &c->ts_aux, &c->ut_tot, &c->ut_lev, &c->ut_fb, &c->ut_slots, &c->lc_work};
@@ -3475,7 +3510,6 @@
   if (c->ev_p1) (void) hipEventDestroy (c->ev_p1);
   for (int i = 0; i < TJ_PIECE_EVENTS; i++) { if (c->ev_pa[i]) (void) hipEventDestroy (c->ev_pa[i]); if (c->ev_pb[i]) (void) hipEventDestroy (c->ev_pb[i]); }
   if (c->ev_done) (void) hipEventDestroy (c->ev_done);
-  if (c->ev_agg) (void) hipEventDestroy (c->ev_agg);
   if (c->own_stream) (void) hipStreamDestroy (c->own_stream);
   delete c;
 }
@@ -3487,6 +3521,7 @@
   if (!c) return set_err (TJAMD_ERR_ARG, "null counter");
   HIPCHK (hipSetDevice (c->device));
   HIPCHK (hipStreamSynchronize (c->stream));
+  if (c->order_own) HIPCHK (hipStreamSynchronize (c->order_own));
   c->stream = hip_stream ? (hipStream_t) hip_stream : c->own_stream;
   return TJAMD_OK;
 }
@@ -3497,6 +3532,7 @@
   HIPCHK (hipSetDevice (c->device));
   HIPCHK (hipStreamSynchronize (c->stream));
   if (c->order_stream) HIPCHK (hipStreamSynchronize (c->order_stream));
+  if (c->order_own) HIPCHK (hipStreamSynchronize (c->order_own));
   c->order_stream = (hipStream_t) hip_stream;
   return TJAMD_OK;
 }
@@ -4080,8 +4116,8 @@
   HIPCHK (hipGetLastError ());
   hipLaunchKernelGGL (cov_max_kernel, dim3 (std::min<unsigned> (grid_for (t), 256u)), dim3 (256), 0, c->stream, (const u64 *) ctab, t, &c->d_fin->coverage);
   HIPCHK (hipGetLastError ());
-  HIPCHK (c->timer[T_FIN].end (c->stream));
-  c->timer[T_FIN].timed = true;
+  HIPCHK (c->timer[T_ORDER].end (c->stream));
+  c->timer[T_ORDER].timed = true;
   HIPCHK (hipMemcpyAsync (c->h_fin, c->d_fin, sizeof (FinCounts), hipMemcpyDeviceToHost, c->stream));
   HIPCHK (hipStreamSynchronize (c->stream));
   return TJAMD_OK;
@@ -4090,8 +4126,17 @@
 static int finalise_binned (tjamd_counter *c, long n1, int min_coverage, long cap = 0, bool wait = true)
 {
   const bool planned = n1 == 0;
-  const bool aside = planned && !wait && c->order_stream != nullptr && c->order_stream != c->stream;
-  const hipStream_t st = aside ? c->order_stream : c->stream;
+  hipStream_t other = c->order_stream;
+  if (planned && !wait && !other && c->order_owned) {
+    if (!c->order_own) {
+      int least = 0, greatest = 0;
+      HIPCHK (hipDeviceGetStreamPriorityRange (&least, &greatest));
+      HIPCHK (hipStreamCreateWithPriority (&c->order_own, hipStreamNonBlocking, greatest));
+    }
+    other = c->order_own;
+  }
+  const bool aside = planned && !wait && other != nullptr && other != c->stream;
+  const hipStream_t st = aside ? other : c->stream;
   const FinPlan *plan = planned ? &c->d_state->plan : nullptr;
   if (planned) n1 = cap;
   const int nbits = bin_bits_for (n1, c->k);
@@ -4114,24 +4159,25 @@
   u32 *bins = (u32 *) c->bins.p, *binstart = (u32 *) c->binstart.p, *binctx = (u32 *) c->binctx.p, *binout = binctx + nbins;
   u32 *tstart = (u32 *) c->headpos.p, *tend = (u32 *) c->outpos.p;
   u64 *ctab = (u64 *) c->cov.p;
-  if (!fused && !c->bins_zeroed) HIPCHK (hipMemsetAsync (bins, 0, (size_t) BS_MAXBINS * 4, c->stream));
+  if (aside) { HIPCHK (hipStreamWaitEvent (st, c->timer[T_FIN].e1, 0)); HIPCHK (c->timer[T_ORDER].begin (st)); }
+  c->order_aside = aside;
+  if (!fused && !c->bins_zeroed) HIPCHK (hipMemsetAsync (bins, 0, (size_t) BS_MAXBINS * 4, st));
   c->bins_zeroed = false;
-  if (aside) { HIPCHK (hipEventRecord (c->ev_agg, c->stream)); HIPCHK (hipStreamWaitEvent (st, c->ev_agg, 0)); }
   const unsigned g1 = planned ? std::min<unsigned> (grid_for (n1), 2048u) : grid_for (n1);
   if (!fused) hipLaunchKernelGGL (bin_count_kernel, dim3 (g1), dim3 (256), 0, st, (const u64 *) c->kept.p, n1, c->k, nbits, bins,
                                   (uint4 *) c->cov.p, (long) (t / 2), 0, plan);
-  hipLaunchKernelGGL (bin_scan_kernel, dim3 (1), dim3 (1024), 0, st, bins, nbins, binstart, c->bin_rank_max, c->d_fin, plan);
+  hipLaunchKernelGGL (bin_scan_kernel, dim3 (1), dim3 (WGS_BLOCK), 0, st, bins, nbins, binstart, c->bin_rank_max, c->d_fin, plan);
   hipLaunchKernelGGL (bin_scatter_kernel, dim3 (g1), dim3 (256), 0, st, (const u64 *) c->kept.p, (u64 *) c->alt.p, n1, c->k, nbits, bins, plan,
                       fused ? (uint4 *) c->cov.p : (uint4 *) nullptr);
   hipLaunchKernelGGL (bin_sort_index_kernel, dim3 ((unsigned) std::min (nbins / BSI_WAVES + 1, 16384)), dim3 (64 * BSI_WAVES), 0, st,
                       (const u64 *) c->alt.p, (u64 *) c->kept.p, (const u32 *) binstart, nbins, (const FinCounts *) c->d_fin, min_coverage,
                       ctab, log2t, binctx, tstart, tend, plan, cov_direct);
-  hipLaunchKernelGGL (bin_ctx_scan_kernel, dim3 (1), dim3 (1024), 0, st, (const u32 *) binctx, nbins, binout, c->d_fin, plan);
+  hipLaunchKernelGGL (bin_ctx_scan_kernel, dim3 (1), dim3 (WGS_BLOCK), 0, st, (const u32 *) binctx, nbins, binout, c->d_fin, plan);
   hipLaunchKernelGGL (bin_ctx_write_kernel, dim3 (256), dim3 (256), 0, st, (const u32 *) binstart, (const u32 *) binctx, (const u32 *) binout, nbins,
                       (const u32 *) tstart, (const u32 *) tend, (int *) c->idx_i.p, (int *) c->idx_f.p, (const u64 *) ctab, t, c->d_fin, plan);
   HIPCHK (hipGetLastError ());
-  HIPCHK (c->timer[T_FIN].end (st));
-  c->timer[T_FIN].timed = true;
+  HIPCHK (c->timer[T_ORDER].end (st));
+  c->timer[T_ORDER].timed = true;
   if (planned) HIPCHK (hipMemcpyAsync (c->h_state, c->d_state, sizeof (DevState), hipMemcpyDeviceToHost, st));
   else HIPCHK (hipMemcpyAsync (c->h_fin, c->d_fin, sizeof (FinCounts), hipMemcpyDeviceToHost, c->stream));
   if (wait) HIPCHK (hipStreamSynchronize (c->stream));
@@ -4170,7 +4216,7 @@
   if (phase == 2) goto second_half;
   c->fin_pending = 0;
   {
-  c->n_kept = 0; c->n_idx = 0; c->coverage = 0; c->timer[T_FIN].timed = false;
+  c->n_kept = 0; c->n_idx = 0; c->coverage = 0; c->timer[T_FIN].timed = false; c->timer[T_ORDER].timed = false; c->order_aside = false;
   speculative = (c->raw_bound / 2 + 1) * 24 <= (8ull << 30);
   kept_cap = c->raw_bound / 2 + 1;
   if (!speculative) {
@@ -4210,6 +4256,8 @@
   rc = plan_ahead ? TJAMD_OK : queue_counter_copies (c);
   if (!rc) rc = clear_buckets (c, plan_ahead);
   if (rc) return rc;
+  HIPCHK (c->timer[T_FIN].end (c->stream));
+  c->timer[T_FIN].timed = true;
   c->fin_rb = remove_biased; c->fin_mc = min_coverage; c->fin_speculative = speculative; c->fin_plan_ahead = plan_ahead; c->fin_kept_cap = kept_cap;
   if (plan_ahead) { rc = finalise_binned (c, 0, min_coverage, plan_cap, phase != 1); if (rc) return rc; }
   else HIPCHK (hipStreamSynchronize (c->stream));
@@ -4238,7 +4286,7 @@
   if (plan_ahead ? c->h_state->plan.kept_overflow : c->h_fin->overflow) return set_err (TJAMD_ERR_CAPACITY, "kept list overflow");
   const long n1 = plan_ahead ? c->h_state->plan.n1 : (long) c->h_fin->n_kept;
   if (n1 == 0) {
-    HIPCHK (c->timer[T_FIN].end (c->stream)); c->timer[T_FIN].timed = true;
+    HIPCHK (c->timer[T_ORDER].end (c->stream)); c->timer[T_ORDER].timed = true;
     c->status = 2; if (status) *status = 2; return TJAMD_OK;
   }
 
@@ -4322,6 +4370,25 @@
 }
 
 extern "C" double tjamd_last_finalise_ms (tjamd_counter *c) { return c ? c->timer[T_FIN].ms (c->device) : -1.0; }
+
+extern "C" double tjamd_last_order_ms (tjamd_counter *c)
+{
+  if (!c || !c->timer[T_FIN].timed || !c->timer[T_ORDER].timed) return -1.0;
+  if (c->order_aside) return c->timer[T_ORDER].ms (c->device);
+  float ms = 0.f;
+  if (hipSetDevice (c->device) != hipSuccess || hipEventSynchronize (c->timer[T_ORDER].e1) != hipSuccess ||
+      hipEventElapsedTime (&ms, c->timer[T_FIN].e1, c->timer[T_ORDER].e1) != hipSuccess) return -1.0;
+  return (double) ms;
+}
+
+extern "C" double tjamd_debug_finalise_span_ms (tjamd_counter *c)
+{
+  float ms = 0.f;
+  if (!c || !c->timer[T_FIN].timed || !c->timer[T_ORDER].timed) return -1.0;
+  if (hipSetDevice (c->device) != hipSuccess || hipEventSynchronize (c->timer[T_ORDER].e1) != hipSuccess ||
+      hipEventElapsedTime (&ms, c->timer[T_FIN].e0, c->timer[T_ORDER].e1) != hipSuccess) return -1.0;
+  return (double) ms;
+}
 
 extern "C" long tjamd_last_scan_launches (tjamd_counter *c) { return c ? c->last_scan_launches : -1; }
 extern "C" long tjamd_plan_mismatches (tjamd_counter *c) { return c ? c->plan_mismatches : -1; }
@@ -5408,13 +5475,13 @@
   Stage st (c, T_MERGE);
   st.begin ();
   hipLaunchKernelGGL (bin_count_kernel, dim3 (grid_for (n)), dim3 (256), 0, c->stream, (const u64 *) d_records, n, c->k, nbits, bins, (uint4 *) nullptr, 0l, 1);
-  hipLaunchKernelGGL (bin_scan_kernel, dim3 (1), dim3 (1024), 0, c->stream, bins, nbins, binstart,
+  hipLaunchKernelGGL (bin_scan_kernel, dim3 (1), dim3 (WGS_BLOCK), 0, c->stream, bins, nbins, binstart,
                       c->bin_rank_max < (u32) BS_RANK_MAX ? c->bin_rank_max : (u32) MG_RANK_MAX, c->d_fin);
   hipLaunchKernelGGL (merge_scatter_kernel, dim3 (grid_for (n)), dim3 (256), 0, c->stream, (const u64 *) d_records, (u64 *) c->alt.p, n, c->k, nbits, bins,
                       (const long *) c->prefix.p, n_samples);
   hipLaunchKernelGGL (bin_merge_kernel, dim3 ((unsigned) std::min (nbins, 16384)), dim3 (64), 0, c->stream, (const u64 *) c->alt.p, (const u32 *) binstart, nbins,
                       (const FinCounts *) c->d_fin, binctx, tpos, ttot);
-  hipLaunchKernelGGL (bin_ctx_scan_kernel, dim3 (1), dim3 (1024), 0, c->stream, (const u32 *) binctx, nbins, binout, c->d_fin);
+  hipLaunchKernelGGL (bin_ctx_scan_kernel, dim3 (1), dim3 (WGS_BLOCK), 0, c->stream, (const u32 *) binctx, nbins, binout, c->d_fin);
   hipLaunchKernelGGL (bin_merge_write_kernel, dim3 ((unsigned) std::min (nbins / 4 + 1, 4096)), dim3 (256), 0, c->stream, (const u64 *) c->alt.p, (const u32 *) binstart,
                       (const u32 *) binout, nbins, (const FinCounts *) c->d_fin, (const u32 *) tpos, (const u32 *) ttot, n_samples,
                       (u64 *) d_out_keys, (int *) d_out_counts, capacity);
```

Measured after the change: 11.28 billion. About the same (-0.2%).
